# VKostoulas/Medical_Image_Generation

Measured on AMD Instinct MI355X. Metric: 3D DDPM U-Net train-step voxels/sec at 128^3 bf16, higher is better.
Workload: dtype bf16; 1 GPU; C4: DiffusionModelUNet num_channels=(32,64,128,256), attention at 16^3 (heads of 64), 128^3 x batch 1/GPU, eps-prediction, AdamW, clip 1.0; global_batch=1, parallelism=dp1, hipgraph=True

## Files before the change

### include/medimgen_hip.h

```cpp
#ifndef MEDIMGEN_HIP_H
#define MEDIMGEN_HIP_H

#include <hip/hip_runtime_api.h>
#include <stdint.h>

#ifdef __cplusplus
extern "C" {
#endif

#define MI_ERR_BAD_ARG 10001
#define MI_ERR_UNSUPPORTED 10002

int mi_abi_version(void);

int mi_ncdhw_f32_to_ndhwc_bf16(const float* src, void* dst, int N, int C, int64_t V, hipStream_t stream);
int mi_ndhwc_bf16_to_ncdhw_f32(const void* src, float* dst, int N, int C, int64_t V, hipStream_t stream);
int mi_cast_f32_to_bf16(const float* src, void* dst, int64_t n, hipStream_t stream);
int mi_cast_bf16_to_f32(const void* src, float* dst, int64_t n, int accumulate, hipStream_t stream);

int mi_add_bf16(const void* a, const void* b, void* out, int64_t n, hipStream_t stream);
int mi_copy_channels(const void* src, int Cs, int c0s, void* dst, int Cd, int c0d, int nC, int64_t nvox, hipStream_t stream);

int mi_upsample_nearest_fwd(const void* x, void* y, int N, int D, int H, int W, int C, int fd, int fh, int fw, hipStream_t stream);
int mi_upsample_nearest_bwd(const void* dy, void* dx, int N, int D, int H, int W, int C, int fd, int fh, int fw, hipStream_t stream);
int mi_space_to_depth(const void* in, int in_cstride, void* out, int N, int D, int H, int W, int C, int fd, int fh, int fw, hipStream_t stream);
int mi_depth_to_space(const void* in, void* out, int N, int D, int H, int W, int C, int fd, int fh, int fw, hipStream_t stream);

int64_t mi_gn_workspace_bytes(int N, int64_t V, int C);
int mi_gn_stats(const void* x, int x_cstride, int N, int64_t V, int C, int G, float eps, const float* gamma, const float* beta,
                float* scale_shift, float* mean_rstd, void* workspace, int64_t workspace_bytes, hipStream_t stream);
int mi_gn_stats_from_partial(const float* partial_a, int chunks_a, int Ca, const float* partial_b, int chunks_b, int Cb, int N, int64_t V,
                             int G, float eps, const float* gamma, const float* beta, float* scale_shift, float* mean_rstd,
                             hipStream_t stream);
int mi_gn_small_supported(int N, int64_t V, int C, int G);
int mi_gn_small_fwd(const void* x, int x_cstride, void* y, int y_cstride, int N, int64_t V, int C, int G, float eps, const float* gamma,
                    const float* beta, float* scale_shift, float* mean_rstd, int act, hipStream_t stream);
int mi_gn_apply(const void* x, int x_cstride, const float* scale_shift, void* y, int y_cstride, int N, int64_t V, int C, int silu,
                hipStream_t stream);
int mi_gn_bwd(const void* g, int g_cstride, const void* x, int x_cstride, int N, int64_t V, int C, int G, const float* gamma,
              const float* scale_shift, const float* mean_rstd, int silu, const void* add, int add_cstride, const void* add2, int add2_cstride,
              void* dx, int dx_cstride, float* dgamma, float* dbeta, float* coef, void* workspace, int64_t workspace_bytes, hipStream_t stream);

#define MI_GN_FUSED_REPLICAS 16
int mi_gn_bwd_fused(const void* g, int g_cstride, const void* x, int x_cstride, int N, int64_t V, int C, int G, const float* gamma,
                    const float* scale_shift, const float* mean_rstd, int silu, const void* add, int add_cstride, const void* add2,
                    int add2_cstride, void* dx, int dx_cstride, float* dgamma, float* dbeta, double* sums_zeroed, hipStream_t stream);

typedef struct mi_conv_plan mi_conv_plan;
int mi_conv_plan_create(mi_conv_plan** plan, int N, int Di, int Hi, int Wi, int Cin, int Cout, const int* kernel3, const int* stride3,
                        const int* padding3);
int mi_upconv_plan_create(mi_conv_plan** out, int N, int D, int H, int W, int Cin, int Cout);
int mi_conv_plan_destroy(mi_conv_plan* plan);
int mi_conv_plan_out_dims(const mi_conv_plan* plan, int* dims3);
int mi_conv_pack_weights(mi_conv_plan* plan, const float* weight, hipStream_t stream);
typedef struct mi_pack_batch mi_pack_batch;
int mi_conv_pack_batch_create(mi_pack_batch** out, mi_conv_plan* const* plans, const float* const* weights, int n);
int mi_conv_pack_batch_run(mi_pack_batch* batch, hipStream_t stream);
int mi_conv_pack_batch_destroy(mi_pack_batch* batch);

int mi_conv_fwd(mi_conv_plan* plan, const void* x, int x_cstride, const float* scale_shift, int silu, const float* addvec,
                int addvec_stride, const void* res, int res_cstride, void* y, int y_cstride, float* out_stats, hipStream_t stream);
int mi_conv_fwd_stats_chunks(const mi_conv_plan* plan);
int mi_conv_dgrad(mi_conv_plan* plan, const void* dy, int dy_cstride, void* dx, int dx_cstride, hipStream_t stream);
int mi_conv_wgrad(mi_conv_plan* plan, const void* x, int x_cstride, const float* scale_shift, int silu, const void* dy, int dy_cstride,
                  float* dweight, float* dy_colsum, int dy_colsum_stride, hipStream_t stream);
int mi_linear_wgrad_bf16(const void* x, int ldx, int in_features, const void* dy, int ldy, int out_features, int64_t rows, float* dw,
                         float* dbias, hipStream_t stream);

int mi_colsum_bf16(const void* x, float* out, int out_stride, int N, int64_t V, int C, int accumulate, hipStream_t stream);
int mi_add_f32_2d(const float* x, int ldx, float* y, int ldy, int rows, int cols, hipStream_t stream);
int mi_sum_rows_f32(const float* in, int ld, int rows, int cols, float* out, int accumulate, hipStream_t stream);
int mi_zero_f32_2d(float* x, int ld, int rows, int cols, hipStream_t stream);

int mi_gemm_nt_bf16(const void* A, int lda, int64_t sA1, int64_t sA2, const void* B, int ldb, int64_t sB1, int64_t sB2, void* C, int ldc,
                    int64_t sC1, int64_t sC2, const float* bias, const void* R, int ldr, int64_t sR1, int64_t sR2, int M, int N, int K,
                    int Z, int Z2, float alpha, int out_f32, int accumulate, hipStream_t stream);
int mi_transpose_bf16(const void* in, int ld_in, int64_t si1, int64_t si2, void* out, int ld_out, int64_t so1, int64_t so2, int R, int Cc,
                      int Z, int Z2, hipStream_t stream);
int mi_softmax_fwd(const float* scores, void* probs, int64_t rows, int cols, int ld_probs, hipStream_t stream);
int mi_softmax_bwd(const void* probs, const float* dprobs, void* dscores, int64_t rows, int cols, int ld_probs, float scale,
                   hipStream_t stream);

int mi_attn_supported(int C, int heads);
int64_t mi_attn_workspace_bytes(int C, int heads, int B, int S);
int mi_attn_fwd(const void* qkv, int ld, int C, int heads, int B, int S, float scale, const void* resid, void* y, float* lse, void* ws,
                int64_t ws_bytes, hipStream_t stream);
int mi_attn_bwd(const void* qkv, int ld, int C, int heads, int B, int S, float scale, const void* y, const void* resid, const void* dy,
                const float* lse, float* dsum, void* dqkv, void* ws, int64_t ws_bytes, hipStream_t stream);

int mi_timestep_embedding(const int64_t* timesteps, float* out, int B, int dim, float max_period, hipStream_t stream);
int mi_embedding_add(float* emb, const float* weight, const int64_t* labels, int B, int dim, hipStream_t stream);
int mi_embedding_bwd(const float* d_emb, const int64_t* labels, float* dweight, int B, int dim, hipStream_t stream);
int mi_silu_f32(const float* x, float* y, int64_t n, hipStream_t stream);
int mi_silu_bwd_f32(const float* x, const float* dy, float* dx, int64_t n, hipStream_t stream);

int mi_logvar_to_sigma_fwd(const void* logvar, void* sigma, int64_t n, hipStream_t stream);
int mi_logvar_to_sigma_bwd(const void* dsigma, const void* logvar, const void* sigma, void* dlogvar, int64_t n, hipStream_t stream);

int mi_layernorm_fwd(const void* x, int ldx, const float* gamma, const float* beta, void* y, int ldy, float* mean_rstd, int64_t M, int C,
                     float eps, hipStream_t stream);
int mi_layernorm_bwd(const void* dy, int lddy, const void* x, int ldx, const float* gamma, const float* mean_rstd, void* dx, int lddx,
                     float* dgamma, float* dbeta, int64_t M, int C, hipStream_t stream);
int mi_geglu_fwd(const void* h, void* y, int64_t M, int F, hipStream_t stream);
int mi_geglu_bwd(const void* h, const void* dy, void* dh, int64_t M, int F, hipStream_t stream);

int mi_avgpool_fwd(const void* x, void* y, int N, int D, int H, int W, int C, const int kernel[3], const int stride[3], hipStream_t stream);
int mi_avgpool_bwd(const void* dy, void* dx, int N, int D, int H, int W, int C, const int kernel[3], const int stride[3], hipStream_t stream);

int mi_crop_pad(const void* src, int src_is_f16, int C, int D, int H, int W, const int lo[3], float* out, int oD, int oH, int oW,
                float pad_value, int flip_mask, float scale, int clamp01, hipStream_t stream);

enum { MI_AUG_SCALE = 0, MI_AUG_CONTRAST = 1, MI_AUG_GAMMA = 2, MI_AUG_RESTORE_STATS = 3, MI_AUG_ADD_NOISE = 4, MI_AUG_CLAMP01 = 5 };
int64_t mi_aug_stats_workspace_bytes(void);
int mi_aug_plane_stats(const float* x, int64_t V, float* stats, float* workspace, hipStream_t stream);
int mi_aug_pointwise(float* x, int64_t V, int op, float p0, const float* stats_a, const float* stats_b, const float* aux, hipStream_t stream);
int mi_aug_blur_axis(const float* x, float* y, int D, int H, int W, int axis, const float* taps_host, int ntaps, hipStream_t stream);
int mi_aug_lowres(const float* x, float* y, int D, int H, int W, int lD, int lH, int lW, hipStream_t stream);
int mi_aug_affine_sample(const float* x, float* y, int D, int H, int W, int oD, int oH, int oW, const float* a_host, hipStream_t stream);

int mi_im2col3d(const void* x, int x_cstride, void* patches, int N, int D, int H, int W, int C, int k, int s, int p, hipStream_t stream);
int mi_col2im3d(const void* dpatches, void* dx, int dx_cstride, int N, int D, int H, int W, int C, int k, int s, int p, hipStream_t stream);
int mi_disc_pack_weights(const float* w, void* w2, void* w2t, int Cout, int Cout_padded, int Cin, int taps, hipStream_t stream);
int mi_disc_wgrad_unpack(const float* dw2, float* dw, int Cout, int Cin, int taps, hipStream_t stream);
int mi_leaky_relu_fwd(const void* x, void* y, int64_t n, float slope, hipStream_t stream);
int mi_leaky_relu_bwd(const void* x, const void* dy, void* dx, int64_t n, float slope, hipStream_t stream);
int mi_ls_gan_loss(const void* logits, int cs, int64_t nvox, float target, float act_slope, void* dlogits, float* loss, float weight,
                   hipStream_t stream);
int mi_bn_running_update(const float* mean_rstd, float* running_mean, float* running_var, int64_t* num_batches_tracked, int C, float eps,
                         float momentum, int64_t count, hipStream_t stream);

int mi_perc_gather(const void* x, int x_cstride, int C, int N, int D, int H, int W, int axis, const int* idx, int S, const float* shift,
                   const float* scale, void* out, hipStream_t stream);
int mi_perc_scatter_add(const void* dslices, int axis, const int* idx, int S, int N, int D, int H, int W, int C, const float* scale, void* dx,
                        int dx_cstride, hipStream_t stream);
int mi_pad_cin_f32(const float* w, float* out, int Cout, int Cin, int Cin_pad, int taps, hipStream_t stream);
int mi_relu_maxpool2_fwd(void* x, void* pooled, int N, int H, int W, int C, hipStream_t stream);
int mi_relu_maxpool2_bwd(const void* a, const void* dpooled, const void* dadd, void* dx, int N, int H, int W, int C, hipStream_t stream);
int mi_lpips_head(const void* f0, const void* f1, const float* w, int S, int64_t P, int C, float weight, float eps, float* loss, void* df0,
                  hipStream_t stream);

int mi_ssim_tiles(int D, int H, int W, int kD, int kH, int kW);
int mi_ssim_pairs(const float* x_base, const float* y_base, const int* pairs, int P, int C, int D, int H, int W, const float* taps, int kD,
                  int kH, int kW, float c1, float c2, double* partials, int part_stride, int part_off, hipStream_t stream);
int mi_ssim_pool2(const float* x, float* y, int64_t NC, int D, int H, int W, int pool_d, hipStream_t stream);
int mi_ssim_finalize(const double* partials, int P, int part_stride, int S, const int* host_tiles, const double* host_counts,
                     const double* host_weights, float* ms_out, float* ssim_out, hipStream_t stream);

int mi_qsample(const float* x0, const float* noise, const float* sqrt_alphas_cumprod, const float* sqrt_one_minus_alphas_cumprod,
               const int64_t* timesteps, const float* cond, int cond_channels, void* out, float* velocity, int N, int C, int64_t V,
               int num_train_timesteps, hipStream_t stream);
int mi_ddpm_step(float* x, const void* eps, const float* noise, const float* coef, const int64_t* t, void* x_cl, int x_cl_cs, int N,
                 int C, int64_t V, int clip, hipStream_t stream);
int mi_mse_fwd_bwd(const void* pred, const float* target, void* dpred, float* loss, int N, int C, int64_t V, float grad_scale,
                   hipStream_t stream);

int mi_l1_fwd_bwd(const void* pred, const float* target, void* dpred, float* loss, int N, int C, int64_t V, int accumulate, hipStream_t stream);
int mi_reparam_kl_fwd(const void* mu, const void* sigma, const float* eps, void* z, float* loss, int N, int C, int64_t V, float kl_weight,
                      hipStream_t stream);
int mi_reparam_kl_bwd(const void* mu, const void* sigma, const float* eps, const void* dz, void* dmu, void* dsigma, int N, int C, int64_t V,
                      float kl_weight, hipStream_t stream);

int mi_sumsq_f32(const float* x, int64_t n, float* out, int accumulate, hipStream_t stream);
int mi_clip_grad_by_norm(float* grad, int64_t n, const float* grad_sumsq, float max_norm, hipStream_t stream);
int mi_adam_step(float* param, const float* grad, float* exp_avg, float* exp_avg_sq, int64_t n, float lr, float beta1, float beta2,
                 float eps, float weight_decay, int decoupled_weight_decay, const float* grad_sumsq, float max_norm, float grad_scale,
                 float* step_counter, hipStream_t stream);
int mi_adam_step_dev(float* param, const float* grad, float* exp_avg, float* exp_avg_sq, int64_t n, const float* hparams,
                     int decoupled_weight_decay, const float* grad_sumsq, float grad_scale, float* step_counter, hipStream_t stream);
int mi_axpy_f32(float* y, const float* x, float alpha, int64_t n, hipStream_t stream);
int mi_scale_f32(float* x, float alpha, int64_t n, hipStream_t stream);

#define MI_METER_HEADER 4
#define MI_METER_PARTIALS 1024
int64_t mi_meter_bytes(void);
int mi_meter_reset(double* acc, hipStream_t stream);
int mi_mse_eval(const void* pred, const float* target, double* acc, int N, int C, int64_t V, hipStream_t stream);
int mi_l1_eval(const void* pred, const float* target, double* acc, int N, int C, int64_t V, hipStream_t stream);
int mi_kl_eval(const void* mu, const void* sigma, double* acc, int N, int C, int64_t V, hipStream_t stream);

#ifdef __cplusplus
}
#endif
#endif
```

### medical_image_generation_amd/_lib.py

```python
from __future__ import annotations

import ctypes as C
import os

import torch

_HERE = os.path.dirname(os.path.abspath(__file__))
LIB_PATH = os.environ.get("MI_LIB_PATH") or os.path.join(_HERE, "libmedimgen_hip.so")

_p, _i, _l, _f = C.c_void_p, C.c_int, C.c_int64, C.c_float

_SIGS = {
    "mi_abi_version": [],
    "mi_ncdhw_f32_to_ndhwc_bf16": [_p, _p, _i, _i, _l, _p],
    "mi_ndhwc_bf16_to_ncdhw_f32": [_p, _p, _i, _i, _l, _p],
    "mi_cast_f32_to_bf16": [_p, _p, _l, _p],
    "mi_cast_bf16_to_f32": [_p, _p, _l, _i, _p],
    "mi_add_bf16": [_p, _p, _p, _l, _p],
    "mi_copy_channels": [_p, _i, _i, _p, _i, _i, _i, _l, _p],
    "mi_upsample_nearest_fwd": [_p, _p, _i, _i, _i, _i, _i, _i, _i, _i, _p],
    "mi_upsample_nearest_bwd": [_p, _p, _i, _i, _i, _i, _i, _i, _i, _i, _p],
    "mi_space_to_depth": [_p, _i, _p, _i, _i, _i, _i, _i, _i, _i, _i, _p],
    "mi_depth_to_space": [_p, _p, _i, _i, _i, _i, _i, _i, _i, _i, _p],
    "mi_gn_workspace_bytes": [_i, _l, _i],
    "mi_gn_stats": [_p, _i, _i, _l, _i, _i, _f, _p, _p, _p, _p, _p, _l, _p],
    "mi_gn_stats_from_partial": [_p, _i, _i, _p, _i, _i, _i, _l, _i, _f, _p, _p, _p, _p, _p],
    "mi_gn_apply": [_p, _i, _p, _p, _i, _i, _l, _i, _i, _p],
    "mi_gn_bwd": [_p, _i, _p, _i, _i, _l, _i, _i, _p, _p, _p, _i, _p, _i, _p, _i, _p, _i, _p, _p, _p, _p, _l, _p],
    "mi_gn_bwd_fused": [_p, _i, _p, _i, _i, _l, _i, _i, _p, _p, _p, _i, _p, _i, _p, _i, _p, _i, _p, _p, _p, _p],
    "mi_conv_plan_create": [C.POINTER(_p), _i, _i, _i, _i, _i, _i, C.POINTER(_i), C.POINTER(_i), C.POINTER(_i)],
    "mi_upconv_plan_create": [C.POINTER(_p), _i, _i, _i, _i, _i, _i],
    "mi_conv_plan_destroy": [_p],
    "mi_conv_plan_out_dims": [_p, C.POINTER(_i)],
    "mi_conv_pack_weights": [_p, _p, _p],
    "mi_conv_pack_batch_create": [C.POINTER(_p), C.POINTER(_p), C.POINTER(_p), _i],
    "mi_conv_pack_batch_run": [_p, _p],
    "mi_conv_pack_batch_destroy": [_p],
    "mi_conv_fwd": [_p, _p, _i, _p, _i, _p, _i, _p, _i, _p, _i, _p, _p],
    "mi_conv_fwd_stats_chunks": [_p],
    "mi_conv_dgrad": [_p, _p, _i, _p, _i, _p],
    "mi_conv_wgrad": [_p, _p, _i, _p, _i, _p, _i, _p, _p, _i, _p],
    "mi_linear_wgrad_bf16": [_p, _i, _i, _p, _i, _i, _l, _p, _p, _p],
    "mi_colsum_bf16": [_p, _p, _i, _i, _l, _i, _i, _p],
    "mi_add_f32_2d": [_p, _i, _p, _i, _i, _i, _p],
    "mi_sum_rows_f32": [_p, _i, _i, _i, _p, _i, _p],
    "mi_zero_f32_2d": [_p, _i, _i, _i, _p],
    "mi_gemm_nt_bf16": [_p, _i, _l, _l, _p, _i, _l, _l, _p, _i, _l, _l, _p, _p, _i, _l, _l, _i, _i, _i, _i, _i, _f, _i, _i, _p],
    "mi_transpose_bf16": [_p, _i, _l, _l, _p, _i, _l, _l, _i, _i, _i, _i, _p],
    "mi_softmax_fwd": [_p, _p, _l, _i, _i, _p],
    "mi_softmax_bwd": [_p, _p, _p, _l, _i, _i, _f, _p],
    "mi_attn_supported": [_i, _i],
    "mi_attn_workspace_bytes": [_i, _i, _i, _i],
    "mi_attn_fwd": [_p, _i, _i, _i, _i, _i, _f, _p, _p, _p, _p, _l, _p],
    "mi_attn_bwd": [_p, _i, _i, _i, _i, _i, _f, _p, _p, _p, _p, _p, _p, _p, _l, _p],
    "mi_timestep_embedding": [_p, _p, _i, _i, _f, _p],
    "mi_silu_f32": [_p, _p, _l, _p],
    "mi_silu_bwd_f32": [_p, _p, _p, _l, _p],
    "mi_logvar_to_sigma_fwd": [_p, _p, _l, _p],
    "mi_logvar_to_sigma_bwd": [_p, _p, _p, _p, _l, _p],
    "mi_embedding_add": [_p, _p, _p, _i, _i, _p],
    "mi_embedding_bwd": [_p, _p, _p, _i, _i, _p],
    "mi_layernorm_fwd": [_p, _i, _p, _p, _p, _i, _p, _l, _i, _f, _p],
    "mi_layernorm_bwd": [_p, _i, _p, _i, _p, _p, _p, _i, _p, _p, _l, _i, _p],
    "mi_geglu_fwd": [_p, _p, _l, _i, _p],
    "mi_geglu_bwd": [_p, _p, _p, _l, _i, _p],
    "mi_avgpool_fwd": [_p, _p, _i, _i, _i, _i, _i, _p, _p, _p],
    "mi_avgpool_bwd": [_p, _p, _i, _i, _i, _i, _i, _p, _p, _p],
    "mi_crop_pad": [_p, _i, _i, _i, _i, _i, _p, _p, _i, _i, _i, _f, _i, _f, _i, _p],
    "mi_gn_small_supported": [_i, _l, _i, _i],
    "mi_gn_small_fwd": [_p, _i, _p, _i, _i, _l, _i, _i, _f, _p, _p, _p, _p, _i, _p],
    "mi_aug_stats_workspace_bytes": [],
    "mi_aug_plane_stats": [_p, _l, _p, _p, _p],
    "mi_aug_pointwise": [_p, _l, _i, _f, _p, _p, _p, _p],
    "mi_aug_blur_axis": [_p, _p, _i, _i, _i, _i, _p, _i, _p],
    "mi_aug_lowres": [_p, _p, _i, _i, _i, _i, _i, _i, _p],
    "mi_aug_affine_sample": [_p, _p, _i, _i, _i, _i, _i, _i, _p, _p],
    "mi_im2col3d": [_p, _i, _p, _i, _i, _i, _i, _i, _i, _i, _i, _p],
    "mi_col2im3d": [_p, _p, _i, _i, _i, _i, _i, _i, _i, _i, _i, _p],
    "mi_disc_pack_weights": [_p, _p, _p, _i, _i, _i, _i, _p],
    "mi_disc_wgrad_unpack": [_p, _p, _i, _i, _i, _p],
    "mi_perc_gather": [_p, _i, _i, _i, _i, _i, _i, _i, _p, _i, _p, _p, _p, _p],
    "mi_perc_scatter_add": [_p, _i, _p, _i, _i, _i, _i, _i, _i, _p, _p, _i, _p],
    "mi_pad_cin_f32": [_p, _p, _i, _i, _i, _i, _p],
    "mi_relu_maxpool2_fwd": [_p, _p, _i, _i, _i, _i, _p],
    "mi_relu_maxpool2_bwd": [_p, _p, _p, _p, _i, _i, _i, _i, _p],
    "mi_lpips_head": [_p, _p, _p, _i, _l, _i, _f, _f, _p, _p, _p],
    "mi_ssim_tiles": [_i, _i, _i, _i, _i, _i],
    "mi_ssim_pairs": [_p, _p, _p, _i, _i, _i, _i, _i, _p, _i, _i, _i, _f, _f, _p, _i, _i, _p],
    "mi_ssim_pool2": [_p, _p, _l, _i, _i, _i, _i, _p],
    "mi_ssim_finalize": [_p, _i, _i, _i, _p, _p, _p, _p, _p, _p],
    "mi_leaky_relu_fwd": [_p, _p, _l, _f, _p],
    "mi_leaky_relu_bwd": [_p, _p, _p, _l, _f, _p],
    "mi_ls_gan_loss": [_p, _i, _l, _f, _f, _p, _p, _f, _p],
    "mi_bn_running_update": [_p, _p, _p, _p, _i, _f, _f, _l, _p],
    "mi_qsample": [_p, _p, _p, _p, _p, _p, _i, _p, _p, _i, _i, _l, _i, _p],
    "mi_ddpm_step": [_p, _p, _p, _p, _p, _p, _i, _i, _i, _l, _i, _p],
    "mi_mse_fwd_bwd": [_p, _p, _p, _p, _i, _i, _l, _f, _p],
    "mi_l1_fwd_bwd": [_p, _p, _p, _p, _i, _i, _l, _i, _p],
    "mi_reparam_kl_fwd": [_p, _p, _p, _p, _p, _i, _i, _l, _f, _p],
    "mi_reparam_kl_bwd": [_p, _p, _p, _p, _p, _p, _i, _i, _l, _f, _p],
    "mi_sumsq_f32": [_p, _l, _p, _i, _p],
    "mi_clip_grad_by_norm": [_p, _l, _p, _f, _p],
    "mi_adam_step": [_p, _p, _p, _p, _l, _f, _f, _f, _f, _f, _i, _p, _f, _f, _p, _p],
    "mi_adam_step_dev": [_p, _p, _p, _p, _l, _p, _i, _p, _f, _p, _p],
    "mi_axpy_f32": [_p, _p, _f, _l, _p],
    "mi_scale_f32": [_p, _f, _l, _p],
    "mi_meter_bytes": [],
    "mi_meter_reset": [_p, _p],
    "mi_mse_eval": [_p, _p, _p, _i, _i, _l, _p],
    "mi_l1_eval": [_p, _p, _p, _i, _i, _l, _p],
    "mi_kl_eval": [_p, _p, _p, _i, _i, _l, _p],
}
_RET = {"mi_gn_workspace_bytes": _l, "mi_attn_workspace_bytes": _l, "mi_aug_stats_workspace_bytes": _l, "mi_meter_bytes": _l}
_NOCHECK = {"mi_abi_version", "mi_meter_bytes", "mi_ssim_tiles", "mi_gn_small_supported", "mi_gn_workspace_bytes", "mi_aug_stats_workspace_bytes", "mi_attn_supported", "mi_attn_workspace_bytes", "mi_conv_fwd_stats_chunks"}

_lib = None
ABI_VERSION = 12


def exported_symbols() -> list[str]:
    return sorted(_SIGS)


def load():
    global _lib
    if _lib is None:
        if not os.path.exists(LIB_PATH):
            raise RuntimeError(
                f"{LIB_PATH} is missing: build it with `python -c 'import __graft_entry__ as g; g.build()'` "
                "(there is no CPU / PyTorch fallback for the HIP path)")
        lib = C.CDLL(LIB_PATH)
        try:
            lib.mi_abi_version.restype = _i
            have = int(lib.mi_abi_version())
        except AttributeError:
            have = None
        if have != ABI_VERSION:
            raise RuntimeError(f"{LIB_PATH} is a stale library (C ABI {have}, this binding needs {ABI_VERSION}): rebuild it with "
                               "`python -c 'import __graft_entry__ as g; g.build()'`")
        for name, args in _SIGS.items():
            fn = getattr(lib, name)
            fn.argtypes = args
            fn.restype = _RET.get(name, _i)
        _lib = lib
    return _lib


def stream_ptr() -> int:
    return torch.cuda.current_stream().cuda_stream


class HipError(RuntimeError):
    pass


_ERRS = {10001: "MI_ERR_BAD_ARG (host-side shape/alignment check failed)", 10002: "MI_ERR_UNSUPPORTED"}


def ptr(t):
    if t is None:
        return None
    assert t.is_cuda, "medimgen HIP ops take device tensors only"
    return t.data_ptr()


_profile = None


class profile_calls:

    def __enter__(self):
        global _profile
        self.records = []
        _profile = self
        return self

    def __exit__(self, *exc):
        global _profile
        _profile = None
        return False

    def summary(self):
        torch.cuda.synchronize()
        out = {}
        for name, e0, e1 in self.records:
            out[name] = out.get(name, 0.0) + e0.elapsed_time(e1)
        return out


def call(name: str, *args):
    fn = getattr(load(), name)
    prof = _profile
    if prof is not None:
        st = torch.cuda.current_stream()
        e0, e1 = torch.cuda.Event(enable_timing=True), torch.cuda.Event(enable_timing=True)
        e0.record(st)
    rc = fn(*args, stream_ptr())
    if prof is not None:
        e1.record(st)
        prof.records.append((name, e0, e1))
    if rc != 0:
        raise HipError(f"{name} failed: {_ERRS.get(rc, f'hipError_t {rc}')}")


def call_raw(name: str, *args):
    fn = getattr(load(), name)
    rc = fn(*args)
    if name not in _NOCHECK and rc != 0:
        raise HipError(f"{name} failed: {_ERRS.get(rc, f'hipError_t {rc}')}")
    return rc
```

### medical_image_generation_amd/csrc/api.hip

```cpp
#include "common.h"
#include "medimgen_hip.h"
extern "C" int mi_abi_version(void) { return 12; }
```

### medical_image_generation_amd/csrc/conv.hip

```cpp
#include <stdlib.h>
#include <string.h>

#include <algorithm>
#include <unordered_map>
#include <vector>

#include "conv_common.h"
#include "medimgen_hip.h"

namespace {

template <int NP>
struct Stage {
  int pk[NP];
  u32x4 pre[NP];
  unsigned valid;
};

template <int NP, int NT = 256>
__device__ __forceinline__ void stage_init(Stage<NP>& s, const Geom& g) {
  const int HVOX = g.HD * g.HH * g.HW;
#pragma unroll
  for (int i = 0; i < NP; ++i) {
    int v = (threadIdx.x + NT * i) >> 2;
// ... 2046 lines not shown
  const int64_t xb = (int64_t)N * id * ih * iw * x_cs * 2, yb = (int64_t)N * od * oh * ow * y_cs * 2;
  if (xb >= (1ll << 32) || yb >= (1ll << 32) || (int64_t)ps.nfrags * 1024 >= (1ll << 32)) return MI_ERR_UNSUPPORTED;
  ConvArgs a;
  memset(&a, 0, sizeof(a));
  a.x = (const bf16*)x; a.x_cs = x_cs; a.N = N; a.Di = id; a.Hi = ih; a.Wi = iw; a.Cin = ps.Ki;
  a.y = (bf16*)y; a.y_cs = y_cs; a.Cout = ps.Ko; a.Do = od; a.Ho = oh; a.Wo = ow;
  a.ogpq = ps.ny; a.outc_q = ps.Ko;
  a.wpk = ps.d_w; a.wpk_bytes = (unsigned)ps.nfrags * 1024u; a.nchunks = ps.nchunks;
  a.addvec = addvec; a.addvec_stride = addvec_stride;
  a.x_bytes = (unsigned)xb; a.y_bytes = (unsigned)yb;
  a.perm16 = 1;
  a.g = ps.g;
  const int ntiles = N * a.g.tilesD * a.g.tilesH * a.g.tilesW;
  return mi_launch_convph(a, ps.ncb, ps.mode, ntiles, ps.ny, st);
}

int upconv_wgrad_tables(mi_conv_plan* P) {
  const int halo[3] = {1, 1, 1};
  P->g_wg = make_geom(2, P->Di, P->Hi, P->Wi, halo, P->N, 64);
  const Geom& g = P->g_wg;
  if (g.TD != 4 || g.TH != 8 || g.TW != 8 || g.row != WG3_XROW || g.slice != WG3_XSLICE) return MI_ERR_UNSUPPORTED;
  const int ny = (P->Cout + 31) / 32, nch = (P->Cin + 31) / 32;
  P->up_nch = nch;
  P->wg.ny = ny; P->wg.nchunks = nch;
  const int npairs = ny * nch * 2;
  P->wg_split_stride = (int64_t)ny * nch * 64 * 1024;
  const int ntiles = P->N * g.tilesD * g.tilesH * g.tilesW;
  int nsplit = 1;
  {
    int64_t best = -1;
    for (int ns = 1; ns <= 256 && ns <= ntiles; ++ns) {
      const int per_xcd = ns >= 8 ? npairs * ((ns + 7) / 8) : (npairs * ns + 7) / 8;
      const int64_t rounds = (per_xcd + 31) / 32, cost = rounds * ((ntiles + ns - 1) / ns + 2);
      if (best < 0 || cost < best) { best = cost; nsplit = ns; }
    }
  }
  static const int ns_env = env_int("MI_WGU_NSPLIT", 0);
  if (ns_env > 0 && ns_env <= ntiles) nsplit = ns_env;
  while (nsplit > 1 && (int64_t)nsplit * P->wg_split_stride * 4 > (256ll << 20)) nsplit /= 2;
  P->wg_nsplit = nsplit;
  if (hipMalloc((void**)&P->d_part, (size_t)nsplit * P->wg_split_stride * 4) != hipSuccess) return (int)hipErrorOutOfMemory;
  if (hipMalloc((void**)&P->d_cspart, (size_t)nsplit * 8 * P->N * P->Cout * 4) != hipSuccess) return (int)hipErrorOutOfMemory;
  return 0;
}

int upconv_wgrad(mi_conv_plan* P, const void* x, int x_cs, const void* dy, int dy_cs, float* dw, float* dy_colsum, int dy_colsum_stride, hipStream_t st) {
  if (dy_colsum && dy_colsum_stride != 0 && dy_colsum_stride < P->Cout) return MI_ERR_BAD_ARG;
  WgradArgs w;
  memset(&w, 0, sizeof(w));
  ConvArgs& a = w.c;
  a.x = (const bf16*)x; a.x_cs = x_cs; a.N = P->N; a.Di = P->Di; a.Hi = P->Hi; a.Wi = P->Wi; a.Cin = P->Cin;
  a.Cout = P->Cout; a.Do = P->Do; a.Ho = P->Ho; a.Wo = P->Wo;
  a.nchunks = P->up_nch;
  a.g = P->g_wg;
  const int64_t xb = (int64_t)P->N * P->Di * P->Hi * P->Wi * x_cs * 2, dyb = (int64_t)P->N * P->Do * P->Ho * P->Wo * dy_cs * 2;
  if (xb >= (1ll << 32) || dyb >= (1ll << 32)) return MI_ERR_UNSUPPORTED;
  a.x_bytes = (unsigned)xb;
  w.dy = (const bf16*)dy; w.dy_cs = dy_cs; w.dy_bytes = (unsigned)dyb;
  w.sx = 1; w.sy = 2; w.cs_chunks = 1;
  w.part = P->d_part; w.split_stride = P->wg_split_stride;
  w.ntiles = P->N * a.g.tilesD * a.g.tilesH * a.g.tilesW;
  w.nsplit = P->wg_nsplit;
  static const int contig_env = env_int("MI_WGRAD_CONTIG", 1);
  w.contig = contig_env && (w.ntiles % 8 == 0) && (w.nsplit % 8 == 0) && w.nsplit <= w.ntiles;
  w.colsum = dy_colsum; w.colsum_stride = dy_colsum_stride;
  w.cs_part = dy_colsum ? P->d_cspart : nullptr;
  w.npairs = P->wg.ny * P->up_nch * 2;
  const size_t lds = 2 * WGU_XSLOT + WGU_NBY * WGU_YSLOT + 64;
  static bool attr = false;
  if (!attr) {
    hipError_t e = hipFuncSetAttribute((const void*)k_wgrad_up, hipFuncAttributeMaxDynamicSharedMemorySize, 160 * 1024);
    if (e != hipSuccess) return (int)e;
    attr = true;
  }
  dim3 grid(w.nsplit >= 8 ? w.npairs * ((w.nsplit + 7) / 8) * 8 : w.npairs * w.nsplit);
  hipLaunchKernelGGL(k_wgrad_up, grid, dim3(768), lds, st, w);
  CsReduce cs{w.cs_part, P->wg_nsplit * 8, P->N, P->Cout, dy_colsum, dy_colsum_stride, 0};
  cs.nbx = (cs.Cout + 31) / 32;
  const int extra = cs.part ? cs.nbx * cs.N : 0, nmain = P->wg.ny * P->up_nch * 32;
  hipLaunchKernelGGL(k_wgrad_reduce_up, dim3(nmain + extra), dim3(256), 0, st, P->d_part, P->wg_split_stride, P->wg_nsplit, P->up_nch, dw, P->Cout,
                     P->Cin, cs, nmain);
  MI_CHECK_LAUNCH();
  return 0;
}

}

extern "C" {

int mi_conv_plan_create(mi_conv_plan** out, int N, int Di, int Hi, int Wi, int Cin, int Cout, const int* k, const int* s, const int* p) {
  if (!out || N <= 0 || Di <= 0 || Hi <= 0 || Wi <= 0 || Cin <= 0 || Cout <= 0) return MI_ERR_BAD_ARG;
  mi_conv_plan* P = new mi_conv_plan();
  P->N = N; P->Di = Di; P->Hi = Hi; P->Wi = Wi; P->Cin = Cin; P->Cout = Cout;
  std::vector<AxisCombo> cf[3], cdg[3];
  int dims[3] = {Di, Hi, Wi}, od[3], halo_f[3] = {0, 0, 0}, halo_d[3] = {0, 0, 0};
  for (int a = 0; a < 3; ++a) {
    P->k[a] = k[a]; P->s[a] = s[a]; P->p[a] = p[a];
    if (!axis_combos_fwd(k[a], s[a], p[a], cf[a], P->f[a]) || !axis_combos_dgrad(k[a], s[a], p[a], cdg[a])) {
      delete P;
      return MI_ERR_UNSUPPORTED;
    }
    od[a] = (dims[a] + 2 * p[a] - k[a]) / s[a] + 1;
    for (auto& c : cf[a]) if (c.delta != 0) halo_f[a] = 1;
    for (auto& c : cdg[a]) if (c.delta != 0) halo_d[a] = 1;
  }
  P->Do = od[0]; P->Ho = od[1]; P->Wo = od[2];
  P->Q = P->f[0] * P->f[1] * P->f[2];
  P->strided = P->Q > 1;
  P->Dp = (Di + P->f[0] - 1) / P->f[0]; P->Hp = (Hi + P->f[1] - 1) / P->f[1]; P->Wp = (Wi + P->f[2] - 1) / P->f[2];
  P->KT = k[0] * k[1] * k[2];
  P->full27 = true;
  for (int a = 0; a < 3; ++a) P->full27 = P->full27 && k[a] == 3 && s[a] == 1 && p[a] == 1;
  if (P->strided && (Cin % 8) != 0) { delete P; return MI_ERR_UNSUPPORTED; }
  P->ncb_fwd = Cout > 32 && Cout != 96 ? 2 : 1;
  {
    static const int ncb1_max = env_int("MI_NCB1_FWD_MAXC", 32);
    if (Cout <= ncb1_max && (Cout % 32) == 0) P->ncb_fwd = 1;
  }
  P->ncb_dg = Cin > 32 && Cin != 96 ? 2 : 1;
  {
    const int64_t tiles = (int64_t)N * ((od[0] + 3) / 4) * ((od[1] + 7) / 8) * ((od[2] + 7) / 8);
    if (od[0] > 1 && tiles * ((Cout + 63) / 64) <= 128) P->ncb_fwd = 1;
    if (od[0] > 1 && tiles * ((Cin + 63) / 64) <= 128) P->ncb_dg = 1;
  }
  P->g_fwd = make_geom(2, P->Do, P->Ho, P->Wo, halo_f, N);
  static const int use27 = env_int("MI_CONV27", 1);
  {
    static const int use_c1 = env_int("MI_CONV_C1", 1);
    auto c_ok = [](int c) { return c >= 8 && c <= 64 && (c & 7) == 0; };
    P->c1_in = use_c1 && P->full27 && Cin == 1 && c_ok(Cout);
    P->c1_out = use_c1 && P->full27 && Cout == 1 && c_ok(Cin);
    if (P->c1_in || P->c1_out) {
      const int C = P->c1_in ? Cout : Cin;
      if (hipMalloc((void**)&P->d_c1w, (size_t)27 * C * 4) != hipSuccess) { mi_conv_plan_destroy(P); return (int)hipErrorOutOfMemory; }
      if (hipMalloc((void**)&P->d_c1part, (size_t)mi_c1_wgrad_scratch_floats(C) * 4) != hipSuccess) { mi_conv_plan_destroy(P); return (int)hipErrorOutOfMemory; }
    }
  }
  const bool geo27 = P->full27 && P->g_fwd.TD == 4 && P->g_fwd.TH == 8 && P->g_fwd.TW == 8;
  P->v27_fwd = use27 && geo27 && (Cin % 8) == 0 && (Cout % 8) == 0;
  P->v27_dg = use27 && geo27 && (Cout % 8) == 0 && (Cin % 8) == 0;
  {
    static const int use11 = env_int("MI_CONV1X1", 1);
    const bool k1 = P->KT == 1 && !P->strided;
    auto chunks_ok = [](int c) { int n = (c + 31) / 32; return n == 1 || n == 2 || n == 3 || n == 4 || n == 6; };
    P->v11_fwd = use11 && k1 && (Cin % 8) == 0 && chunks_ok(Cin) && ((Cout + 31) / 32) * ((Cin + 31) / 32) * 2 <= 96;
    P->v11_dg = use11 && k1 && (Cout % 8) == 0 && chunks_ok(Cout) && ((Cout + 31) / 32) * ((Cin + 31) / 32) * 2 <= 96;
    static const int use_g11 = env_int("MI_CONV1X1_GEMM", 1);
    P->g11 = use_g11 && k1 && (!P->v11_fwd || !P->v11_dg) && (Cin % 8) == 0 && (Cout % 8) == 0;
    if (P->g11 && (hipMalloc((void**)&P->d_w11, (size_t)Cin * Cout * 2) != hipSuccess || hipMalloc((void**)&P->d_w11t, (size_t)Cin * Cout * 2) != hipSuccess)) {
      mi_conv_plan_destroy(P);
      return (int)hipErrorOutOfMemory;
    }
  }
  build_tables(P->fwd, P->g_fwd, P->ncb_fwd, cf, P->f, P->k, true, Cin, Cout, false, P->v27_fwd || P->v11_fwd);
  P->g_dg = make_geom(2, P->Dp, P->Hp, P->Wp, halo_d, N);
  build_tables(P->dg, P->g_dg, P->ncb_dg, cdg, P->f, P->k, false, Cout, Cin, true, P->v27_dg || P->v11_dg);
  P->g_wg = make_geom(2, P->Do, P->Ho, P->Wo, halo_f, N, 64);
  build_tables(P->wg, P->g_wg, 1, cf, P->f, P->k, true, Cin, Cout, false);
  int e;
  if ((e = upload_tables(P->fwd, true)) || (e = upload_tables(P->dg, true)) || (e = upload_tables(P->wg, false))) { mi_conv_plan_destroy(P); return e; }
  int npairs = P->wg.ny * P->wg.nchunks;
  int64_t off = 0;
  P->wg_pair_off.resize(npairs);
  for (int pr = 0; pr < npairs; ++pr) {
    P->wg_pair_off[pr] = (int)off;
    int nt = P->wg.hdr[(size_t)pr * 4 + 1];
    int frag0 = P->wg.hdr[(size_t)pr * 4 + 3];
    for (int t = 0; t < nt; ++t) {
      const int* it = &P->wg.frag_items[(size_t)(frag0 + t * 2) * 4];
      P->wg_uitems.push_back(it[0]); P->wg_uitems.push_back(it[1]); P->wg_uitems.push_back(it[2]); P->wg_uitems.push_back(0);
    }
    off += (int64_t)nt * 1024;
  }
  P->wg_split_stride = off;
  P->wg_nitems = (int)(off / 1024);
  int ntiles = N * P->g_wg.tilesD * P->g_wg.tilesH * P->g_wg.tilesW;
  int nsplit = 1;
  {
    int64_t best = -1;
    for (int ns = 1; ns <= 256 && ns <= ntiles; ++ns) {
      const int per_xcd = ns >= 8 ? npairs * ((ns + 7) / 8) : (npairs * ns + 7) / 8;
      static const int slab_cost = env_int("MI_WGRAD_SLAB_COST", 0);
      const int64_t rounds = (per_xcd + 31) / 32;
      const int64_t cost = 100 * rounds * ((ntiles + ns - 1) / ns + 6) + (int64_t)slab_cost * ns * (off * 4 / (1 << 20));
      if (best < 0 || cost < best) { best = cost; nsplit = ns; }
    }
  }
  static const int old_split = env_int("MI_WGRAD_SPLIT_OLD", 0);
  if (old_split) nsplit = (256 + npairs - 1) / npairs;
  static const int force_split = env_int("MI_WGRAD_NSPLIT", 0);
  if (force_split && ntiles <= 64) nsplit = force_split;
  if (nsplit > ntiles) nsplit = ntiles;
  while (nsplit > 1 && (int64_t)nsplit * off * 4 > (256ll << 20)) nsplit /= 2;
  if (nsplit < 1) nsplit = 1;
  P->wg_nsplit = nsplit;
  if ((e = upload(P->wg_pair_off, &P->d_pair_off)) || (e = upload(P->wg_uitems, &P->d_uitems))) { mi_conv_plan_destroy(P); return e; }
  if (hipMalloc((void**)&P->d_part, (size_t)nsplit * off * 4) != hipSuccess) { mi_conv_plan_destroy(P); return (int)hipErrorOutOfMemory; }
  if (hipMalloc((void**)&P->d_cspart, (size_t)nsplit * N * Cout * 4) != hipSuccess) { mi_conv_plan_destroy(P); return (int)hipErrorOutOfMemory; }
  {
    static const int use_ph = env_int("MI_CONVPH", 1);
    bool s2all = Di > 1;
    for (int a = 0; a < 3; ++a) s2all = s2all && k[a] == 3 && s[a] == 2 && p[a] == 1;
    if (use_ph && s2all && (Cin % 8) == 0 && (Cout % 8) == 0) {
      int e1 = phase_side_create(P->ph_fwd, S2_FWD, 2, 0, Cout, Cin, P->Do, P->Ho, P->Wo, N);
      int e2 = e1 ? e1 : phase_side_create(P->ph_dg, S2_DG, 1, 1, Cin, Cout, P->Do, P->Ho, P->Wo, N);
      if (e1 || e2) { phase_side_free(P->ph_fwd); phase_side_free(P->ph_dg); if ((e1 ? e1 : e2) != MI_ERR_UNSUPPORTED) { mi_conv_plan_destroy(P); return e1 ? e1 : e2; } }
      if (P->ph_fwd.mode && (Cin % 32) == 0) {
        std::vector<int> h2 = P->wg.hdr;
        const int cpq = Cin / 32;
        for (int pr = 0; pr < P->wg.ny * P->wg.nchunks; ++pr) {
          const int ch = pr % P->wg.nchunks, q = ch / cpq;
          h2[(size_t)pr * 4 + 2] = (ch % cpq) * 32;
          h2[(size_t)pr * 4 + 3] = q;
        }
        if ((e = upload(h2, &P->d_hdr2))) { mi_conv_plan_destroy(P); return e; }
        P->s2_wg_direct = true;
      }
    }
  }
  if (P->strided) {
    size_t nb = (size_t)N * P->Dp * P->Hp * P->Wp * P->Q * Cin * 2;
    if (hipMalloc((void**)&P->d_xs, nb) != hipSuccess || hipMalloc((void**)&P->d_dxs, nb) != hipSuccess) { mi_conv_plan_destroy(P); return (int)hipErrorOutOfMemory; }
  }
  *out = P;
  return 0;
}

int mi_conv_plan_destroy(mi_conv_plan* P) {
  if (!P) return 0;
  phase_side_free(P->ph_fwd); phase_side_free(P->ph_dg);
  if (P->d_hdr2) (void)hipFree(P->d_hdr2);
  if (P->up_inner) mi_conv_plan_destroy(P->up_inner);
  if (P->d_xup) (void)hipFree(P->d_xup);
  free_tables(P->fwd); free_tables(P->dg); free_tables(P->wg);
  if (P->d_pair_off) (void)hipFree(P->d_pair_off);
  if (P->d_uitems) (void)hipFree(P->d_uitems);
  if (P->d_part) (void)hipFree(P->d_part);
  if (P->d_cspart) (void)hipFree(P->d_cspart);
  if (P->d_c1w) (void)hipFree(P->d_c1w);
  if (P->d_w11) (void)hipFree(P->d_w11);
  if (P->d_w11t) (void)hipFree(P->d_w11t);
  if (P->d_g11job) (void)hipFree(P->d_g11job);
  if (P->d_c1part) (void)hipFree(P->d_c1part);
  if (P->d_xs) (void)hipFree(P->d_xs);
  if (P->d_dxs) (void)hipFree(P->d_dxs);
  delete P;
  return 0;
}

int mi_upconv_plan_create(mi_conv_plan** out, int N, int D, int H, int W, int Cin, int Cout) {
  if (!out || N <= 0 || D <= 0 || H <= 0 || W <= 0 || Cin <= 0 || Cout <= 0) return MI_ERR_BAD_ARG;
  if (D == 1) return MI_ERR_UNSUPPORTED;
  mi_conv_plan* P = new mi_conv_plan();
  P->up = true;
  P->N = N; P->Di = D; P->Hi = H; P->Wi = W; P->Cin = Cin; P->Cout = Cout;
  P->Do = 2 * D; P->Ho = 2 * H; P->Wo = 2 * W;
  for (int a = 0; a < 3; ++a) { P->k[a] = 3; P->s[a] = 1; P->p[a] = 1; P->f[a] = 1; }
  P->Q = 1; P->KT = 27; P->Dp = D; P->Hp = H; P->Wp = W;
  const int k3[3] = {3, 3, 3}, s1[3] = {1, 1, 1}, p1[3] = {1, 1, 1};
  int e = mi_conv_plan_create(&P->up_inner, N, 2 * D, 2 * H, 2 * W, Cin, Cout, k3, s1, p1);
  if (e) { P->up_inner = nullptr; mi_conv_plan_destroy(P); return e; }
  if (hipMalloc((void**)&P->d_xup, (size_t)N * 8 * D * H * W * Cin * 2) != hipSuccess) { mi_conv_plan_destroy(P); return (int)hipErrorOutOfMemory; }
  static const int use_ph = env_int("MI_CONVPH", 1);
  if (use_ph && (Cin % 8) == 0 && (Cout % 8) == 0) {
    int e1 = phase_side_create(P->ph_fwd, UC_FWD, 1, 0, Cout, Cin, D, H, W, N);
    int e2 = e1 ? e1 : phase_side_create(P->ph_dg, UC_DG, 2, 1, Cin, Cout, D, H, W, N);
    if (e1 || e2) { phase_side_free(P->ph_fwd); phase_side_free(P->ph_dg); if ((e1 ? e1 : e2) != MI_ERR_UNSUPPORTED) { mi_conv_plan_destroy(P); return e1 ? e1 : e2; } }
    if (P->ph_fwd.mode) {
      const int ew = upconv_wgrad_tables(P);
      if (ew && ew != MI_ERR_UNSUPPORTED) { mi_conv_plan_destroy(P); return ew; }
      P->up_wg = ew == 0;
    }
  }
  *out = P;
  return 0;
}

int mi_conv_plan_out_dims(const mi_conv_plan* P, int* dims3) {
  if (!P || !dims3) return MI_ERR_BAD_ARG;
  dims3[0] = P->Do; dims3[1] = P->Ho; dims3[2] = P->Wo;
  return 0;
}

}

struct G11Job { const float* w; bf16* o; bf16* ot; int Co, Ci, block0, bx; };
namespace {
__global__ void __launch_bounds__(256) k_pack_gemm11(const G11Job* __restrict__ jobs, int njobs) {
  __shared__ float t[32][33];
  int j = 0;
  while (j + 1 < njobs && (int)blockIdx.x >= jobs[j + 1].block0) ++j;
  const G11Job g = jobs[j];
  const int b = blockIdx.x - g.block0, bi = b % g.bx, bo = b / g.bx;
  const int tx = threadIdx.x & 31, ty = threadIdx.x >> 5;
  for (int r = ty; r < 32; r += 8) {
    const int co = bo * 32 + r, ci = bi * 32 + tx;
    const float v = (co < g.Co && ci < g.Ci) ? g.w[(int64_t)co * g.Ci + ci] : 0.f;
    t[r][tx] = v;
    if (co < g.Co && ci < g.Ci) g.o[(int64_t)co * g.Ci + ci] = f2bf(v);
  }
  __syncthreads();
  for (int r = ty; r < 32; r += 8) {
    const int ci = bi * 32 + r, co = bo * 32 + tx;
    if (co < g.Co && ci < g.Ci) g.ot[(int64_t)ci * g.Co + co] = f2bf(t[tx][r]);
  }
}
G11Job g11_job(const mi_conv_plan* P, const float* w, int block0) {
  G11Job g;
  g.w = w; g.o = P->d_w11; g.ot = P->d_w11t; g.Co = P->Cout; g.Ci = P->Cin; g.block0 = block0; g.bx = (P->Cin + 31) / 32;
  return g;
}
int g11_blocks(const mi_conv_plan* P) { return ((P->Cin + 31) / 32) * ((P->Cout + 31) / 32); }
}

extern "C" {

int mi_conv_pack_weights(mi_conv_plan* P, const float* w, hipStream_t st) {
  if (!P || !w) return MI_ERR_BAD_ARG;
  {
    int e = phase_side_pack(P->ph_fwd, w, P->Cout, P->Cin, st);
    if (!e) e = phase_side_pack(P->ph_dg, w, P->Cout, P->Cin, st);
    if (e) return e;
    if (P->up) return mi_conv_pack_weights(P->up_inner, w, st);
  }
  hipLaunchKernelGGL(k_pack_weights, dim3(((P->fwd.nfrags + P->dg.nfrags) * 64 + 255) / 256), dim3(256), 0, st, w, P->fwd.d_wpk,
                     P->fwd.d_items, P->fwd.nfrags, P->dg.d_wpk, P->dg.d_items, P->dg.nfrags, P->Cout, P->Cin, P->KT, P->d_c1w,
                     P->d_c1w ? 27 * P->Cin * P->Cout : 0);
  if (P->g11) {
    if (!P->d_g11job || P->g11job_w != w) {
      if (!P->d_g11job && hipMalloc(&P->d_g11job, sizeof(G11Job)) != hipSuccess) return (int)hipErrorOutOfMemory;
      const G11Job h = g11_job(P, w, 0);
      if (hipMemcpy(P->d_g11job, &h, sizeof(h), hipMemcpyHostToDevice) != hipSuccess) return (int)hipErrorUnknown;
      P->g11job_w = w;
    }
    hipLaunchKernelGGL(k_pack_gemm11, dim3(g11_blocks(P)), dim3(256), 0, st, (const G11Job*)P->d_g11job, 1);
  }
  P->c1_packed = true;
  MI_CHECK_LAUNCH();
  return 0;
}

struct mi_pack_batch {
  PackSuper* d_supers = nullptr;
  int nsupers = 0;
  size_t lds_super = 0;
  G11Job* d_g11 = nullptr;
  int ng11 = 0, g11_blocks = 0;
  PackGroup* d_groups = nullptr;
  int2* d_gtaps = nullptr;
  int ngroups = 0;
  size_t lds = 0;
  PhasePackJob* d_phase = nullptr;
  int nphase = 0, phase_blocks = 0;
};
namespace {
void add_groups(std::vector<PackGroup>& groups, std::vector<int2>& gtaps, const Tables& T, const float* w, const mi_conv_plan* P) {
  std::unordered_map<int64_t, int> index;
  const size_t g0 = groups.size();
  std::vector<std::vector<int2>> taps;
  for (int f = 0; f < T.nfrags; ++f) {
    const int* it = &T.frag_items[(size_t)f * 4];
    const int64_t key = ((int64_t)it[1] << 32) | (unsigned)it[2];
    auto found = index.find(key);
    int gi = found == index.end() ? -1 : found->second;
    if (gi < 0) {
      gi = (int)taps.size();
      index.emplace(key, gi);
      taps.emplace_back();
      PackGroup g;
      memset(&g, 0, sizeof(g));
      g.w = w; g.out = T.d_wpk;
      g.tr = it[3] & 1; g.perm = (it[3] >> 1) & 1;
      g.o0 = g.tr ? it[2] : it[1];
      g.i0 = g.tr ? it[1] : it[2];
      g.Co_t = P->Cout; g.Ci_t = P->Cin; g.KT = P->KT;
      groups.push_back(g);
    }
    taps[(size_t)gi].push_back(int2{it[0], f});
  }
  for (size_t k = 0; k < taps.size(); ++k) {
    groups[g0 + k].ntaps = (int)taps[k].size();
    groups[g0 + k].tap_off = (int)gtaps.size();
    gtaps.insert(gtaps.end(), taps[k].begin(), taps[k].end());
  }
}
}
int mi_conv_pack_batch_create(mi_pack_batch** out, mi_conv_plan* const* plans, const float* const* weights, int n) {
  if (!out || !plans || !weights || n <= 0) return MI_ERR_BAD_ARG;
  std::vector<PackGroup> groups;
  std::vector<int2> gtaps;
  size_t lds = 0;
  std::vector<PhasePackJob> phase;
  int phase_blocks = 0;
  std::vector<G11Job> g11;
  int g11_nblocks = 0;
  std::vector<PackSuper> supers;
  size_t lds_super = 0;
  static const int use_super = env_int("MI_PACK_SUPER", 1);
  bool super_ok = use_super != 0;
  for (int i = 0; i < n; ++i) {
    mi_conv_plan* P = plans[i];
    if (!P || !weights[i]) return MI_ERR_BAD_ARG;
    for (PhaseSide* ps : {&P->ph_fwd, &P->ph_dg})
      if (ps->mode) {
        phase.push_back(phase_job(*ps, weights[i], P->Cout, P->Cin, phase_blocks));
        phase_blocks += mi_pack_phase_blocks(ps->nfrags, ps->ncb, ps->nchunks);
      }
    if (P->g11) {
      g11.push_back(g11_job(P, weights[i], g11_nblocks));
      g11_nblocks += g11_blocks(P);
    }
    if (P->up) P = P->up_inner;
    P->c1_packed = true;
    const size_t g0 = groups.size();
    add_groups(groups, gtaps, P->fwd, weights[i], P);
    add_groups(groups, gtaps, P->dg, weights[i], P);
    if (P->d_c1w && groups.size() > g0) { groups[g0].c1w = P->d_c1w; groups[g0].c1n = 27 * P->Cin * P->Cout; }
    {
      std::unordered_map<int64_t, int> at;
      for (size_t gi = g0; gi < groups.size(); ++gi) {
        const PackGroup& g = groups[gi];
        const int O0 = g.o0 & ~31, I0 = g.i0 & ~31;
        const int64_t key = ((int64_t)O0 << 32) | (unsigned)I0;
        auto f = at.find(key);
        if (f == at.end()) {
          PackSuper su;
          memset(&su, 0, sizeof(su));
          su.w = weights[i]; su.O0 = O0; su.I0 = I0; su.Co_t = P->Cout; su.Ci_t = P->Cin; su.KT = P->KT;
          at.emplace(key, (int)supers.size());
          supers.push_back(su);
          f = at.find(key);
        }
        PackSuper& su = supers[(size_t)f->second];
        if (su.ng < 4) su.g[su.ng++] = (int)gi;
        else super_ok = false;
      }
      const size_t need_su = sizeof(unsigned short) * 32 * (size_t)(32 * P->KT + 4);
      if (need_su > lds_super) lds_super = need_su;
    }
    const size_t need = sizeof(float) * 32 * (size_t)(16 * P->KT + 1) > sizeof(float) * 16 * (size_t)(32 * P->KT + 1)
                            ? sizeof(float) * 32 * (size_t)(16 * P->KT + 1) : sizeof(float) * 16 * (size_t)(32 * P->KT + 1);
    if (need > lds) lds = need;
  }
  if (lds > 64 * 1024) return MI_ERR_UNSUPPORTED;
  mi_pack_batch* B = new mi_pack_batch();
  B->ngroups = (int)groups.size(); B->lds = lds;
  B->nphase = (int)phase.size(); B->phase_blocks = phase_blocks;
  B->ng11 = (int)g11.size(); B->g11_blocks = g11_nblocks;
  if (use_super > 1) fprintf(stderr, "[pack batch] %d plans, %zu groups, %zu super-groups, paired: %d, LDS %zu B\n", n, groups.size(), supers.size(), (int)super_ok, lds_super);
  if (super_ok && !supers.empty() && lds_super <= 150 * 1024) {
    if (hipMalloc((void**)&B->d_supers, sizeof(PackSuper) * supers.size()) != hipSuccess ||
        hipMemcpy(B->d_supers, supers.data(), sizeof(PackSuper) * supers.size(), hipMemcpyHostToDevice) != hipSuccess ||
        hipFuncSetAttribute((const void*)k_pack_super, hipFuncAttributeMaxDynamicSharedMemorySize, 160 * 1024) != hipSuccess) {
      mi_conv_pack_batch_destroy(B);
      return (int)hipErrorOutOfMemory;
    }
    B->nsupers = (int)supers.size(); B->lds_super = lds_super;
  }
  if (B->ng11) {
    if (hipMalloc((void**)&B->d_g11, sizeof(G11Job) * g11.size()) != hipSuccess ||
        hipMemcpy(B->d_g11, g11.data(), sizeof(G11Job) * g11.size(), hipMemcpyHostToDevice) != hipSuccess) {
      mi_conv_pack_batch_destroy(B);
      return (int)hipErrorOutOfMemory;
    }
  }
  if (B->nphase) {
    if (hipMalloc((void**)&B->d_phase, sizeof(PhasePackJob) * phase.size()) != hipSuccess ||
        hipMemcpy(B->d_phase, phase.data(), sizeof(PhasePackJob) * phase.size(), hipMemcpyHostToDevice) != hipSuccess) {
      mi_conv_pack_batch_destroy(B);
      return (int)hipErrorOutOfMemory;
    }
  }
  if (hipMalloc((void**)&B->d_groups, sizeof(PackGroup) * (groups.size() ? groups.size() : 1)) != hipSuccess ||
      hipMalloc((void**)&B->d_gtaps, sizeof(int2) * (gtaps.size() ? gtaps.size() : 1)) != hipSuccess) {
    mi_conv_pack_batch_destroy(B);
    return (int)hipErrorOutOfMemory;
  }
  hipError_t e = hipMemcpy(B->d_groups, groups.data(), sizeof(PackGroup) * groups.size(), hipMemcpyHostToDevice);
  if (e == hipSuccess) e = hipMemcpy(B->d_gtaps, gtaps.data(), sizeof(int2) * gtaps.size(), hipMemcpyHostToDevice);
  if (e != hipSuccess) { mi_conv_pack_batch_destroy(B); return (int)e; }
  *out = B;
  return 0;
}
int mi_conv_pack_batch_run(mi_pack_batch* B, hipStream_t st) {
  if (!B) return MI_ERR_BAD_ARG;
  if (B->nsupers) hipLaunchKernelGGL(k_pack_super, dim3(B->nsupers), dim3(kPackSuperT), B->lds_super, st, B->d_supers, B->d_groups, B->d_gtaps);
  else if (B->ngroups) hipLaunchKernelGGL(k_pack_groups, dim3(B->ngroups), dim3(256), B->lds, st, B->d_groups, B->d_gtaps);
  MI_CHECK_LAUNCH();
  if (B->ng11) hipLaunchKernelGGL(k_pack_gemm11, dim3(B->g11_blocks), dim3(256), 0, st, (const G11Job*)B->d_g11, B->ng11);
  MI_CHECK_LAUNCH();
  if (B->nphase) return mi_launch_pack_phase(B->d_phase, B->nphase, B->phase_blocks, st);
  return 0;
}
int mi_conv_pack_batch_destroy(mi_pack_batch* B) {
  if (!B) return 0;
  if (B->d_groups) (void)hipFree(B->d_groups);
  if (B->d_gtaps) (void)hipFree(B->d_gtaps);
  if (B->d_phase) (void)hipFree(B->d_phase);
  if (B->d_g11) (void)hipFree(B->d_g11);
  if (B->d_supers) (void)hipFree(B->d_supers);
  delete B;
  return 0;
}

int mi_conv_fwd_stats_chunks(const mi_conv_plan* P) {
  if (P && !P->up && P->c1_in) return mi_c1_expand_stats_chunks(P->N, P->Di, P->Hi, P->Wi, P->Cout);
  if (!P || P->up || !P->v27_fwd || P->N > 16 || P->ncb_fwd != 1) return 0;
  return 4 * mi_conv27_grid_x(P->N * P->g_fwd.tilesD * P->g_fwd.tilesH * P->g_fwd.tilesW, P->fwd.ny);
}

int mi_conv_fwd(mi_conv_plan* P, const void* x, int x_cs, const float* scale_shift, int silu, const float* addvec, int addvec_stride,
                const void* res, int res_cs, void* y, int y_cs, float* out_stats, hipStream_t st) {
  if (!P || !x || !y || x_cs < P->Cin || y_cs < P->Cout) return MI_ERR_BAD_ARG;
  if (out_stats && (!mi_conv_fwd_stats_chunks(P) || scale_shift || ((x_cs & 7) && !P->c1_in))) return MI_ERR_UNSUPPORTED;
  if (P->ph_fwd.mode && !scale_shift && !res) {
    const int e = phase_side_run(P->ph_fwd, x, x_cs, P->Di, P->Hi, P->Wi, y, y_cs, P->Do, P->Ho, P->Wo, P->N, addvec, addvec_stride, st);
    if (e != MI_ERR_UNSUPPORTED) return e;
  }
  if (P->up) {
    if (x_cs != P->Cin) return MI_ERR_UNSUPPORTED;
    int e = mi_upsample_nearest_fwd(x, P->d_xup, P->N, P->Di, P->Hi, P->Wi, P->Cin, 2, 2, 2, st);
    if (e) return e;
    return mi_conv_fwd(P->up_inner, P->d_xup, P->Cin, scale_shift, silu, addvec, addvec_stride, res, res_cs, y, y_cs, nullptr, st);
  }
  if ((P->c1_in || P->c1_out) && P->c1_packed && !scale_shift && !res) {
    if (out_stats && !P->c1_in) return MI_ERR_UNSUPPORTED;
    int e = P->c1_in ? mi_launch_c1_expand(x, x_cs, P->d_c1w, addvec, addvec_stride, y, y_cs, P->N, P->Di, P->Hi, P->Wi, P->Cout, 0, st, out_stats)
                     : mi_launch_c1_reduce(x, x_cs, P->d_c1w, addvec, addvec_stride, y, y_cs, P->N, P->Di, P->Hi, P->Wi, P->Cin, st);
    if (e != MI_ERR_UNSUPPORTED) return e;
  }
  if (out_stats && P->c1_in) return MI_ERR_UNSUPPORTED;
  ConvArgs a;
  memset(&a, 0, sizeof(a));
  const bf16* src = (const bf16*)x;
  int src_cs = x_cs;
  if (P->strided) {
    int e = mi_space_to_depth(x, x_cs, P->d_xs, P->N, P->Di, P->Hi, P->Wi, P->Cin, P->f[0], P->f[1], P->f[2], st);
    if (e) return e;
    src = P->d_xs;
    src_cs = P->Q * P->Cin;
  }
  a.x = src; a.x_cs = src_cs; a.N = P->N; a.Di = P->Dp; a.Hi = P->Hp; a.Wi = P->Wp; a.Cin = P->strided ? P->Q * P->Cin : P->Cin;
  if (!P->strided) { a.Di = P->Di; a.Hi = P->Hi; a.Wi = P->Wi; }
  a.y = (bf16*)y; a.y_cs = y_cs; a.Cout = P->Cout; a.Do = P->Do; a.Ho = P->Ho; a.Wo = P->Wo;
  a.ogpq = P->fwd.ny; a.outc_q = P->Cout;
  a.wpk = P->fwd.d_wpk; a.hdr = P->fwd.d_hdr; a.taps = P->fwd.d_taps; a.nchunks = P->fwd.nchunks;
  a.ss = scale_shift; a.ss_C = P->Cin; a.pro_silu = silu;
  a.addvec = addvec; a.addvec_stride = addvec_stride;
  a.res = (const bf16*)res; a.res_cs = res_cs;
  a.g = P->g_fwd;
  int ntiles = P->N * a.g.tilesD * a.g.tilesH * a.g.tilesW;
  a.wpk_bytes = (unsigned)P->fwd.nfrags * 1024u;
  {
    int64_t xb = (int64_t)a.N * a.Di * a.Hi * a.Wi * a.x_cs * 2;
    if (xb >= (1ll << 32)) return MI_ERR_UNSUPPORTED;
    a.x_bytes = (unsigned)xb;
  }
  a.perm16 = P->v27_fwd || P->v11_fwd;
  if (P->g11 && !P->v11_fwd && !scale_shift && !res && (x_cs & 7) == 0 && (y_cs & 7) == 0 && addvec_stride == 0 && !out_stats &&
      ((uintptr_t)x & 15) == 0 && (int64_t)P->N * P->Do * P->Ho * P->Wo < (1ll << 31))
    return mi_gemm_nt_bf16(x, x_cs, 0, 0, P->d_w11, P->Cin, 0, 0, y, y_cs, 0, 0, addvec, nullptr, 0, 0, 0, P->N * P->Do * P->Ho * P->Wo, P->Cout, P->Cin, 1, 1,
                           1.0f, 0, 0, st);
  if (P->v11_fwd && !scale_shift && !res && (x_cs & 7) == 0) {
    const int64_t yb = (int64_t)P->N * P->Do * P->Ho * P->Wo * y_cs * 2;
    a.y_bytes = yb < (1ll << 32) ? (unsigned)yb : 0u;
    return mi_launch_conv1x1(a, P->ncb_fwd, P->fwd.ny, st);
  }
  if (P->v27_fwd && !scale_shift) {
    if (x_cs & 7) return MI_ERR_UNSUPPORTED;
    const int64_t rb = res ? (int64_t)P->N * P->Do * P->Ho * P->Wo * res_cs * 2 : 0;
    a.res_bytes = rb < (1ll << 32) ? (unsigned)rb : 0u;
    const int64_t yb = (int64_t)P->N * P->Do * P->Ho * P->Wo * y_cs * 2;
    a.y_bytes = yb < (1ll << 32) ? (unsigned)yb : 0u;
    a.stats = out_stats; a.stats_chunks = out_stats ? mi_conv_fwd_stats_chunks(P) : 0;
    const int e27 = mi_launch_conv27(a, P->ncb_fwd, 0, ntiles, P->fwd.ny, st);
    if (e27 != MI_ERR_UNSUPPORTED || out_stats) return e27;
    a.stats = nullptr;
  }
  return launch_igemm_any(a, P->ncb_fwd, P->full27 ? 1 : 0, ntiles, P->fwd.ny, st);
}

int mi_conv_dgrad(mi_conv_plan* P, const void* dy, int dy_cs, void* dx, int dx_cs, hipStream_t st) {
  if (!P || !dy || !dx || dy_cs < P->Cout || dx_cs < P->Cin) return MI_ERR_BAD_ARG;
  if (P->ph_dg.mode) {
    const int e = phase_side_run(P->ph_dg, dy, dy_cs, P->Do, P->Ho, P->Wo, dx, dx_cs, P->Di, P->Hi, P->Wi, P->N, nullptr, 0, st);
    if (e != MI_ERR_UNSUPPORTED) return e;
  }
  if (P->up) {
    if (dx_cs != P->Cin) return MI_ERR_UNSUPPORTED;
    int e = mi_conv_dgrad(P->up_inner, dy, dy_cs, P->d_xup, P->Cin, st);
    if (e) return e;
    return mi_upsample_nearest_bwd(P->d_xup, dx, P->N, P->Di, P->Hi, P->Wi, P->Cin, 2, 2, 2, st);
  }
  if (P->c1_out && P->c1_packed) {
    int e = mi_launch_c1_expand(dy, dy_cs, P->d_c1w, nullptr, 0, dx, dx_cs, P->N, P->Di, P->Hi, P->Wi, P->Cin, 1, st);
    if (e != MI_ERR_UNSUPPORTED) return e;
  }
  ConvArgs a;
  memset(&a, 0, sizeof(a));
  a.x = (const bf16*)dy; a.x_cs = dy_cs; a.N = P->N; a.Di = P->Do; a.Hi = P->Ho; a.Wi = P->Wo; a.Cin = P->Cout;
  a.Do = P->Dp; a.Ho = P->Hp; a.Wo = P->Wp;
  a.Cout = P->Q * P->Cin;
  a.ogpq = P->dg.ny / P->Q; a.outc_q = P->Cin;
  if (P->strided) {
    if (dx_cs != P->Cin) return MI_ERR_UNSUPPORTED;
    a.y = P->d_dxs; a.y_cs = P->Q * P->Cin;
  } else {
    a.y = (bf16*)dx; a.y_cs = dx_cs;
  }
  a.wpk = P->dg.d_wpk; a.hdr = P->dg.d_hdr; a.taps = P->dg.d_taps; a.nchunks = P->dg.nchunks;
  a.g = P->g_dg;
  int ntiles = P->N * a.g.tilesD * a.g.tilesH * a.g.tilesW;
  a.wpk_bytes = (unsigned)P->dg.nfrags * 1024u;
  {
    int64_t xb = (int64_t)a.N * a.Di * a.Hi * a.Wi * a.x_cs * 2;
    if (xb >= (1ll << 32)) return MI_ERR_UNSUPPORTED;
    a.x_bytes = (unsigned)xb;
  }
  a.perm16 = P->v27_dg || P->v11_dg;
  if (P->g11 && !P->v11_dg && (dy_cs & 7) == 0 && (dx_cs & 7) == 0 && ((uintptr_t)dy & 15) == 0 &&
      (int64_t)P->N * P->Do * P->Ho * P->Wo < (1ll << 31))
    return mi_gemm_nt_bf16(dy, dy_cs, 0, 0, P->d_w11t, P->Cout, 0, 0, dx, dx_cs, 0, 0, nullptr, nullptr, 0, 0, 0, P->N * P->Do * P->Ho * P->Wo, P->Cin, P->Cout, 1,
                           1, 1.0f, 0, 0, st);
  if (P->v11_dg && (dy_cs & 7) == 0) {
    const int64_t yb = (int64_t)P->N * a.Do * a.Ho * a.Wo * a.y_cs * 2;
    a.y_bytes = yb < (1ll << 32) ? (unsigned)yb : 0u;
    return mi_launch_conv1x1(a, P->ncb_dg, P->dg.ny, st);
  }
  if (P->v27_dg) {
    if (dy_cs & 7) return MI_ERR_UNSUPPORTED;
    const int64_t yb = (int64_t)P->N * a.Do * a.Ho * a.Wo * a.y_cs * 2;
    a.y_bytes = yb < (1ll << 32) ? (unsigned)yb : 0u;
    const int e27 = mi_launch_conv27(a, P->ncb_dg, 1, ntiles, P->dg.ny, st);
    if (e27 != MI_ERR_UNSUPPORTED) return e27;
  }
  int e = launch_igemm_any(a, P->ncb_dg, P->full27 ? 2 : 0, ntiles, P->dg.ny, st);
  if (e) return e;
  if (P->strided) return mi_depth_to_space(P->d_dxs, dx, P->N, P->Di, P->Hi, P->Wi, P->Cin, P->f[0], P->f[1], P->f[2], st);
  return 0;
}

int mi_conv_wgrad(mi_conv_plan* P, const void* x, int x_cs, const float* scale_shift, int silu, const void* dy, int dy_cs, float* dw,
                  float* dy_colsum, int dy_colsum_stride, hipStream_t st) {
  if (!P || !x || !dy || !dw || x_cs < P->Cin || dy_cs < P->Cout) return MI_ERR_BAD_ARG;
  if (P->up && P->up_wg && !scale_shift && (x_cs & 7) == 0 && (dy_cs & 7) == 0) {
    const int e = upconv_wgrad(P, x, x_cs, dy, dy_cs, dw, dy_colsum, dy_colsum_stride, st);
    if (e != MI_ERR_UNSUPPORTED) return e;
  }
  if (P->up) {
    if (x_cs != P->Cin || scale_shift) return MI_ERR_UNSUPPORTED;
    int e = mi_upsample_nearest_fwd(x, P->d_xup, P->N, P->Di, P->Hi, P->Wi, P->Cin, 2, 2, 2, st);
    if (e) return e;
    return mi_conv_wgrad(P->up_inner, P->d_xup, P->Cin, nullptr, 0, dy, dy_cs, dw, dy_colsum, dy_colsum_stride, st);
  }
  static const int use_w11 = env_int("MI_WGRAD1X1", 1);
  if (use_w11 && P->KT == 1 && !P->strided && !scale_shift && !(dy_colsum && dy_colsum_stride != 0 && dy_colsum_stride < P->Cout)) {
    int e = mi_launch_wgrad1x1(x, x_cs, P->Cin, dy, dy_cs, P->Cout, P->N, (int64_t)P->Di * P->Hi * P->Wi, dw, dy_colsum, dy_colsum_stride, st);
    if (e != MI_ERR_UNSUPPORTED) return e;
  }
  static const int use_c1w = env_int("MI_C1_WGRAD", 1);
  if (use_c1w && (P->c1_in || P->c1_out) && P->d_c1part && !scale_shift && !(dy_colsum && dy_colsum_stride != 0)) {
    int e = P->c1_in ? mi_launch_c1_wgrad(dy, dy_cs, x, x_cs, dw, dy_colsum, nullptr, P->d_c1part, P->N, P->Di, P->Hi, P->Wi, P->Cout, 0, st)
                     : mi_launch_c1_wgrad(x, x_cs, dy, dy_cs, dw, nullptr, dy_colsum, P->d_c1part, P->N, P->Di, P->Hi, P->Wi, P->Cin, 1, st);
    if (e != MI_ERR_UNSUPPORTED) return e;
  }
  WgradArgs w;
  memset(&w, 0, sizeof(w));
  w.sx = w.sy = 1; w.cs_chunks = 1;
  ConvArgs& a = w.c;
  const bf16* src = (const bf16*)x;
  int src_cs = x_cs;
  static const int use_w2 = env_int("MI_WGRAD2", 1);
  bool direct = false;
  if (P->s2_wg_direct && use_w2 && !scale_shift && (x_cs & 7) == 0 && (dy_cs & 7) == 0 && (P->Cout & 7) == 0 && P->g_wg.vox == 64) {
    const int px = (P->g_wg.lds_bytes + 1023) / 1024, py = (P->g_wg.TD * P->g_wg.TH * P->g_wg.TW * 64 + 1023) / 1024;
    const int64_t dyb = (int64_t)P->N * P->Do * P->Ho * P->Wo * dy_cs * 2, xb = (int64_t)P->N * P->Di * P->Hi * P->Wi * x_cs * 2;
    direct = px <= 40 && py <= 16 && dyb < (1ll << 32) && xb < (1ll << 32);
  }
  if (P->strided && !direct) {
    int e = mi_space_to_depth(x, x_cs, P->d_xs, P->N, P->Di, P->Hi, P->Wi, P->Cin, P->f[0], P->f[1], P->f[2], st);
    if (e) return e;
    src = P->d_xs;
    src_cs = P->Q * P->Cin;
  }
  const bool s2d = P->strided && !direct;
  a.x = src; a.x_cs = src_cs; a.N = P->N;
  a.Di = s2d ? P->Dp : P->Di; a.Hi = s2d ? P->Hp : P->Hi; a.Wi = s2d ? P->Wp : P->Wi;
  a.Cin = s2d ? P->Q * P->Cin : P->Cin;
  a.Cout = P->Cout; a.Do = P->Do; a.Ho = P->Ho; a.Wo = P->Wo;
  a.hdr = direct ? P->d_hdr2 : P->wg.d_hdr; a.taps = P->wg.d_taps; a.nchunks = P->wg.nchunks;
  if (direct) w.sx = 2;
  a.ss = scale_shift; a.ss_C = P->Cin; a.pro_silu = silu;
  {
    int64_t xb = (int64_t)a.N * a.Di * a.Hi * a.Wi * a.x_cs * 2;
    if (xb >= (1ll << 32)) return MI_ERR_UNSUPPORTED;
    a.x_bytes = (unsigned)xb;
  }
  a.g = P->g_wg;
  w.dy = (const bf16*)dy; w.dy_cs = dy_cs;
  w.part = P->d_part; w.pair_off = P->d_pair_off; w.split_stride = P->wg_split_stride;
  w.ntiles = P->N * a.g.tilesD * a.g.tilesH * a.g.tilesW;
  w.nsplit = P->wg_nsplit;
  static const int contig_env = env_int("MI_WGRAD_CONTIG", 1);
  w.contig = contig_env && (w.ntiles % 8 == 0) && (w.nsplit % 8 == 0) && w.nsplit <= w.ntiles;
  static const int dbg = mi_diag_knob("MI_WGRAD_DBG");
  w.dbg = dbg;
  w.colsum = dy_colsum; w.colsum_stride = dy_colsum_stride;
  static const int cs_slab = env_int("MI_CS_SLAB", 1);
  bool cs_pairs_multi_tap = true;
  for (int yy = 0; yy < P->wg.ny; ++yy) cs_pairs_multi_tap = cs_pairs_multi_tap && P->wg.hdr[((size_t)yy * P->wg.nchunks) * 4 + 1] > 1;
  w.cs_part = (cs_slab && dy_colsum && cs_pairs_multi_tap) ? P->d_cspart : nullptr;  if (dy_colsum && dy_colsum_stride != 0 && dy_colsum_stride < P->Cout) return MI_ERR_BAD_ARG;
  const int hv = a.g.HD * a.g.HH * a.g.HW;
  const int np = (hv * 4 + 255) / 256;
  const int nvox = a.g.TD * a.g.TH * a.g.TW;
  const int npy = (nvox * 4 + 255) / 256;
  size_t lds = (size_t)a.g.lds_bytes + (size_t)nvox * a.g.vox;
  w.npairs = P->wg.ny * P->wg.nchunks;
  dim3 grid(w.nsplit >= 8 ? w.npairs * ((w.nsplit + 7) / 8) * 8 : w.npairs * w.nsplit), blk(512);
  if ((a.g.TD * (a.g.TH / 2) * (a.g.TW / 8)) % 2) return MI_ERR_BAD_ARG;
  if (npy > 4 || np > 16) return MI_ERR_BAD_ARG;
  int max_taps = 0;
  for (size_t i = 1; i < P->wg.hdr.size(); i += 4) max_taps = P->wg.hdr[i] > max_taps ? P->wg.hdr[i] : max_taps;
  if (max_taps >= 32) return MI_ERR_UNSUPPORTED;
#define MI_LAUNCH_WG(NPV) MI_LAUNCH_WG_G(NPV, false)
#define MI_LAUNCH_WG_G(NPV, G3)                                                                                    \
  do {                                                                                                             \
    auto kern = k_conv_wgrad<NPV, 2, G3>;                                                                          \
    static int lds_ok = 0;                                                                                         \
    if ((int)lds > lds_ok) {                                                                                       \
      hipError_t e = hipFuncSetAttribute((const void*)kern, hipFuncAttributeMaxDynamicSharedMemorySize, 160 * 1024); \
      if (e != hipSuccess) return (int)e;                                                                          \
      lds_ok = 160 * 1024;                                                                                         \
    }                                                                                                              \
    hipLaunchKernelGGL(kern, grid, blk, lds, st, w);                                                               \
  } while (0)
  {
    const int px = (a.g.lds_bytes + 1023) / 1024, py = (nvox * 64 + 1023) / 1024;
    const int64_t dyb = (int64_t)P->N * P->Do * P->Ho * P->Wo * dy_cs * 2;
    if (use_w2 && !scale_shift && a.g.vox == 64 && (a.x_cs & 7) == 0 && (a.Cin & 7) == 0 && (dy_cs & 7) == 0 && (P->Cout & 7) == 0 && px <= 40 &&
        py <= 16 && dyb < (1ll << 32)) {
      w.dy_bytes = (unsigned)dyb;
      w.nbuf = (P->KT == 1 && px == 16 && py == 16) ? 4 : 2;
      static const int use_flags = env_int("MI_WGRAD_FLAGS", 1);
      w.flags = use_flags;
      const size_t lds2 = (size_t)(w.nbuf * (px + py)) * 1024 + 64;
      const bool geo3 = P->full27 && a.g.row == WG3_XROW && a.g.slice == WG3_XSLICE && a.g.TD == 4 && a.g.TH == 8 && a.g.TW == 8;
      static bool attr3 = false, attrg = false;
      bool& done = geo3 ? attr3 : attrg;
      if (!done) {
        hipError_t e = geo3 ? hipFuncSetAttribute((const void*)k_conv_wgrad2<true>, hipFuncAttributeMaxDynamicSharedMemorySize, 160 * 1024)
                            : hipFuncSetAttribute((const void*)k_conv_wgrad2<false>, hipFuncAttributeMaxDynamicSharedMemorySize, 160 * 1024);
        if (e != hipSuccess) return (int)e;
        done = true;
      }
      static const int use_roll = env_int("MI_WGRAD_ROLL", 1);
      const bool roll = use_roll && geo3 && !direct && w.sx == 1 && w.sy == 1 && w.nbuf == 2 && w.flags && P->wg.hdr[1] == 27 && w.nsplit <= w.ntiles &&
                        a.g.tilesD >= 2 && (use_roll > 1 || (int64_t)w.ntiles <= 2ll * a.g.tilesD * w.nsplit);
      if (roll) {
        static bool attr_r = false;
        if (!attr_r) {
          hipError_t e = hipFuncSetAttribute((const void*)k_conv_wgrad3, hipFuncAttributeMaxDynamicSharedMemorySize, 160 * 1024);
          if (e != hipSuccess) return (int)e;
          attr_r = true;
        }
#ifdef MI_WG3_DIAG_CLK
        {
          unsigned long long h0[16] = {0, 0, 0, 0, 0, 0, 0, 0, 0, 0, 0, 0, 0, 0, ~0ull, 0};
          (void)hipDeviceSynchronize();
          (void)hipMemcpyToSymbol(HIP_SYMBOL(g_wg3_clk), h0, sizeof(h0));
          static unsigned long long z[6][1024];
          (void)hipMemcpyToSymbol(HIP_SYMBOL(g_wg3_span), z, sizeof(z));
        }
#endif
        hipLaunchKernelGGL(k_conv_wgrad3, grid, dim3(768), (size_t)WR_LDS, st, w);
#ifdef MI_WG3_DIAG_CLK
        {
          unsigned long long h[16];
          (void)hipDeviceSynchronize();
          (void)hipMemcpyFromSymbol(h, HIP_SYMBOL(g_wg3_clk), sizeof(h));
          auto us = [&](int a, int b) { return (double)((long long)h[b] - (long long)h[a]) / 100.0; };
          fprintf(stderr, "[wgrad3 %d->%d ntiles %d nsplit %d] all workgroups: first entry -> last exit %.2f us | workgroup 0 (from the first entry): entry %.2f, "
                  "compute wave 0: setup %.2f, prologue barrier %.2f, tiles %.2f, final barrier %.2f, stores issued %.2f, stores landed %.2f | loader wave: "
                  "descriptors %.2f, prologue issue %.2f, landed %.2f us\n", P->Cin, P->Cout, w.ntiles, w.nsplit, us(14, 15), us(14, 0), us(0, 1), us(1, 2), us(2, 3), us(3, 4),
                  us(4, 5), us(5, 6), us(8, 9), us(9, 10), us(10, 11));
// ... 55 lines not shown
```

### medical_image_generation_amd/engine.py

```python
from __future__ import annotations

import math
import weakref

import torch

from . import _lib
from . import hipops as ops
from ._lib import call, ptr

BF16, F32 = torch.bfloat16, torch.float32

import os as _os
FLASH_ATTENTION = _os.environ.get("MI_FLASH_ATTENTION", "1") == "1"
FUSE_GN_STATS = ops.FUSE_GN_STATS


class ParamArena:

    def __init__(self, entries, device, late=()):
        self.offsets, self.shapes = {}, {}
        late = set(late)
        off = 0
        self.n_late = 0
        for trainable_pass in (True, False):
            for name, shape, trainable in entries:
                if trainable != trainable_pass:
                    continue
                n = math.prod(shape)
                self.offsets[name], self.shapes[name] = off, tuple(shape)
                off += n
                if not trainable_pass or n % 4:
                    off = (off + 3) // 4 * 4
                if trainable_pass and name in late:
                    assert self.n_late == self.offsets[name], f"late tensors must form a prefix of the arena ({name})"
                    self.n_late = off
            if trainable_pass:
                off = (off + 3) // 4 * 4
                self.n_trainable = off
        self.numel = max(off, 4)
        self.data = torch.zeros(self.numel, dtype=F32, device=device)
        self.grad = torch.zeros(self.numel, dtype=F32, device=device)

    def view(self, name, flat=None):
        flat = self.data if flat is None else flat
        o, s = self.offsets[name], self.shapes[name]
        return flat[o:o + math.prod(s)].view(s)

    def gview(self, name):
        return self.view(name, self.grad)

    def span(self, names, flat=None):
        flat = self.data if flat is None else flat
        o = self.offsets[names[0]]
        end = o
        for nme in names:
            assert self.offsets[nme] == end, f"{nme} is not adjacent in the arena"
            end += math.prod(self.shapes[nme])
        return flat[o:end]


def CUT():
    """Tape marker (a no-op when called): recorded by a model at the forward position behind which -- in backward order: before
    which -- every gradient of the arena's early segment is final.  trainer._ArenaTrainer splits the backward there."""


class Tape:
    def __init__(self):
        self.fns = []
        self.grads = {}
        self.keep = []

    def record(self, fn):
        self.fns.append(fn)

    def take(self, t):
        g = self.grads.pop(id(t), None)
        return ops.add(g[0], g[1]) if isinstance(g, tuple) else g

    def take2(self, t):
        g = self.grads.pop(id(t), None)
        return g if isinstance(g, tuple) else (g, None)

    def put(self, t, g):
        cur = self.grads.get(id(t))
        if cur is None:
            self.grads[id(t)] = g
        elif isinstance(cur, tuple):
            self.grads[id(t)] = ops.add(ops.add(cur[0], cur[1]), g)
        else:
            self.grads[id(t)] = (cur, g)
        self.keep.append(t)

    def move(self, t, other: "Tape"):
        g = self.grads.pop(id(t), None)
        if g is not None:
            other.grads[id(t)] = g
            other.keep.append(t)

    def backward(self, out, dout):
        self.put(out, dout)
        for fn in reversed(self.fns):
            fn()
        self.fns.clear()


class Ctx:

    def __init__(self, arena: ParamArena, plans: dict, grad_enabled=True, prepacked=()):
        self.arena, self.plans = arena, plans
        self.tape = Tape() if grad_enabled else None
        self.packed = set(prepacked)
        self.flops_fwd = 0
        self.flops_bwd = 0
        self.sums = {}
        self.cat_parts = {}

    def sums_of(self, x):
        ent = self.sums.get(id(x))
        return ent[0] if ent is not None and ent[1]() is x else None

    def parts_of(self, x):
        ent = self.cat_parts.get(id(x))
        return ent[:2] if ent is not None and ent[2]() is x else None

    def count(self, fwd_flops, dgrad=True, wgrad=True):
        self.flops_fwd += fwd_flops
        if self.tape is not None:
            self.flops_bwd += fwd_flops * (int(dgrad) + int(wgrad))

    def p(self, name):
        return self.arena.view(name)

    def g(self, name):
        return self.arena.gview(name)


class PackBatch:

    def __init__(self, arena: ParamArena, plans: dict):
        import ctypes as C
        self.keys = tuple(plans)
        n = len(self.keys)
        plan_arr = (C.c_void_p * n)(*[plans[k].handle for k in self.keys])
        w_arr = (C.c_void_p * n)(*[arena.view(k[0] + ".weight").data_ptr() for k in self.keys])
        h = C.c_void_p()
        _lib.call_raw("mi_conv_pack_batch_create", C.byref(h), plan_arr, w_arr, n)
        self.handle = h

    def run(self):
        call("mi_conv_pack_batch_run", self.handle)
        return self.keys

    def __del__(self):
        try:
            if getattr(self, "handle", None):
                _lib.call_raw("mi_conv_pack_batch_destroy", self.handle)
                self.handle = None
        except Exception:
            pass


def gn(ctx: Ctx, x, name, groups, eps):
    gamma, beta = ctx.p(name + ".weight"), ctx.p(name + ".bias")
    st = None
    if FUSE_GN_STATS:
        n, v = x.shape[0], x.shape[1] * x.shape[2] * x.shape[3]
        ent, parts = ctx.sums_of(x), ctx.parts_of(x)
        if ent is not None:
            st = ops.gn_stats_from_sums(ent, None, n, v, groups, eps, gamma, beta)
        elif parts is not None:
            ea, eb = ctx.sums_of(parts[0]), ctx.sums_of(parts[1])
            if ea is not None and eb is not None:
                st = ops.gn_stats_from_sums(ea, eb, n, v, groups, eps, gamma, beta)
    if st is None:
        st = ops.gn_stats(x, groups, eps, gamma, beta)
    st.name = name
    return st


UPCONV = _os.environ.get("MI_UPCONV", "1") == "1"


def upsample_conv(ctx: Ctx, x, name, factors, kernel, padding, out=None):
    n, d, h, w, cin = x.shape
    fused = UPCONV and tuple(factors) == (2, 2, 2) and tuple(kernel) == (3, 3, 3) and tuple(padding) == (1, 1, 1) and d > 1 and \
        cin % 8 == 0 and ctx.p(name + ".weight").shape[0] % 8 == 0 and x.is_contiguous()
    if not fused:
        return conv(ctx, upsample(ctx, x, factors), name, kernel, (1, 1, 1), padding, out=out)
    return conv(ctx, x, name, kernel, (1, 1, 1), padding, out=out, upconv=True)


def conv_transpose(ctx: Ctx, x, name, kernel, stride, padding):
    n, d, h, w, cin = x.shape
    wt = ctx.p(name + ".weight")
    cout = wt.shape[1]
    k, s_, p_ = tuple(kernel), tuple(stride), tuple(padding)
    if d <= 1 or k != (3, 3, 3) or p_ != (1, 1, 1) or s_ not in ((1, 1, 1), (2, 2, 2)) or cin % 8 or cout % 8:
        raise NotImplementedError(f"use_convtranspose: kernel {k} stride {s_} padding {p_} ({cin}->{cout}) is not on the HIP path "
                                  "(3-D, kernel 3, padding 1, stride 1 or 2 on all axes, channels in multiples of 8)")
    fine = tuple(v * s_[0] for v in (d, h, w))
    key = (name, n, d, h, w)
    plan = ctx.plans.get(key)
    if plan is None:
        plan = ctx.plans[key] = ops.ConvPlan(n, fine, cout, cin, k, s_, p_)
    if key not in ctx.packed:
        plan.pack(wt)
        ctx.packed.add(key)
    y0 = plan.dgrad(x)
    bias = ctx.p(name + ".bias")
    ss = torch.stack([torch.ones_like(bias), bias], dim=1).unsqueeze(0).expand(n, cout, 2).contiguous()
    y = ops.gn_apply(y0, ops.GNStats(ss, None, 1), False)
    del y0
    ctx.count(2 * y.numel() * cin * 27 // (s_[0] ** 3), dgrad=True)
    if ctx.tape is not None:
        tape = ctx.tape

        def bwd():
            dy = tape.take(y)
            if dy is None:
                return
            plan.wgrad(dy, x, ctx.g(name + ".weight"))
            ops.colsum(dy.contiguous(), out=ctx.g(name + ".bias"), accumulate=True, merge_batch=True)
            tape.put(x, plan.fwd(dy))

        tape.record(bwd)
    return y


def conv(ctx: Ctx, x, name, kernel, stride, padding, norm=None, silu=False, addvec=None, res=None, d_addvec=None,
         need_dx=True, bias_grad_like=None, out=None, upconv=False):
    n, d, h, w, cin = x.shape
    wt = ctx.p(name + ".weight")
    cout = wt.shape[0]
    key = (name, n, d, h, w)
    plan = ctx.plans.get(key)
    if plan is None:
        plan = ctx.plans[key] = ops.UpConvPlan(n, (d, h, w), cin, cout) if upconv else ops.ConvPlan(n, (d, h, w), cin, cout, kernel, stride, padding)
    if key not in ctx.packed:
        plan.pack(wt)
        ctx.packed.add(key)
    av = addvec if addvec is not None else ctx.p(name + ".bias")
    xin = ops.gn_apply(x, norm, silu) if norm is not None else x
    y, sums = plan.fwd(xin, addvec=av, res=res, out=out, want_sums=True)
    if sums is not None:
        ctx.sums[id(y)] = (sums, weakref.ref(y))
    ctx.count(2 * y.numel() * cin * math.prod(kernel), dgrad=need_dx)
    if ctx.tape is not None:
        tape = ctx.tape

        def bwd():
            dy = tape.take(y)
            if dy is None:
                return
            gw = ctx.g(name + ".weight")
            if bias_grad_like is not None:
                plan.wgrad(xin, dy, gw)
                ops.add_f32_(ctx.g(name + ".bias"), ctx.g(bias_grad_like + ".bias"))
            else:
                plan.wgrad(xin, dy, gw, colsum=d_addvec if d_addvec is not None else ctx.g(name + ".bias"))
            if res is not None:
                tape.put(res, dy)
            if need_dx:
                g = plan.dgrad(dy)
                if norm is not None:
                    other, other2 = tape.take2(x)
                    dx = ops.gn_bwd(g, x, norm, ctx.p(norm.name + ".weight"), silu, ctx.g(norm.name + ".weight"),
                                    ctx.g(norm.name + ".bias"), add=other, add2=other2)
                    tape.grads[id(x)] = dx
                    tape.keep.append(x)
                else:
                    tape.put(x, g)

        tape.record(bwd)
    return y


def upsample(ctx: Ctx, x, factors):
    y = ops.upsample_nearest(x, factors)
    if ctx.tape is not None:
        tape = ctx.tape

        def bwd():
            dy = tape.take(y)
            if dy is not None:
                tape.put(x, ops.upsample_nearest_bwd(ops.dense(dy), factors))

        tape.record(bwd)
    return y


def checkpoint(ctx: Ctx, fn, x):
    if ctx.tape is None:
        return fn(ctx, x)
    sub = Ctx(ctx.arena, ctx.plans, grad_enabled=False)
    sub.packed, sub.sums, sub.cat_parts = ctx.packed, ctx.sums, ctx.cat_parts
    y = fn(sub, x)
    ctx.flops_fwd += sub.flops_fwd
    ctx.flops_bwd += 2 * sub.flops_fwd
    tape = ctx.tape

    def bwd():
        dy = tape.take(y)
        if dy is None:
            return
        inner = Ctx(ctx.arena, ctx.plans, grad_enabled=True)
        inner.packed, inner.sums, inner.cat_parts = ctx.packed, ctx.sums, ctx.cat_parts
        y2 = fn(inner, x)
        it = inner.tape
        tape.move(x, it)
        it.backward(y2, dy)
        g = it.take(x)
        if g is not None:
            tape.grads[id(x)] = g
            tape.keep.append(x)
        it.grads.clear(), it.keep.clear()

    tape.record(bwd)
    return y


def avg_pool(ctx: Ctx, x, kernel, stride):
    y = ops.avg_pool(x, kernel, stride)
    if ctx.tape is not None:
        tape = ctx.tape
        dims = tuple(x.shape[1:4])

        def bwd():
            dy = tape.take(y)
            if dy is not None:
                tape.put(x, ops.avg_pool_bwd(ops.dense(dy), dims, kernel, stride))

        tape.record(bwd)
    return y


def gn_act(ctx: Ctx, x, st, silu):
    y = ops.gn_apply(x, st, silu)
    if ctx.tape is not None:
        tape = ctx.tape

        def bwd():
            g = tape.take(y)
            if g is None:
                return
            other, other2 = tape.take2(x)
            dx = ops.gn_bwd(g, x, st, ctx.p(st.name + ".weight"), silu, ctx.g(st.name + ".weight"), ctx.g(st.name + ".bias"),
                            add=other, add2=other2)
            tape.grads[id(x)] = dx
            tape.keep.append(x)

        tape.record(bwd)
    return y


def add(ctx: Ctx, a, b, b_needs_grad=True):
    y = ops.add(a, b)
    if ctx.tape is not None:
        tape = ctx.tape

        def bwd():
            dy = tape.take(y)
            if dy is not None:
                tape.put(a, dy)
                if b_needs_grad:
                    tape.put(b, dy)

        tape.record(bwd)
    return y


def resnet(ctx: Ctx, x, name, sd, groups, eps, addvec, d_addvec, mode=None, stride=None, kernel=None, out=None):
    k3, s1, p1 = (1,) * (3 - sd) + (3,) * sd, (1, 1, 1), (0,) * (3 - sd) + (1,) * sd
    name = name + "." if name else ""
    n1 = gn(ctx, x, name + "norm1", groups, eps)
    if mode is None:
        h = conv(ctx, x, name + "conv1.conv", k3, s1, p1, norm=n1, silu=True, addvec=addvec, d_addvec=d_addvec)
    else:
        h = gn_act(ctx, x, n1, True)
        if mode == "up":
            x, h = upsample(ctx, x, stride), upsample(ctx, h, stride)
        else:
            x, h = avg_pool(ctx, x, kernel, stride), avg_pool(ctx, h, kernel, stride)
        h = conv(ctx, h, name + "conv1.conv", k3, s1, p1, addvec=addvec, d_addvec=d_addvec)
    n2 = gn(ctx, h, name + "norm2", groups, eps)
    if name + "skip_connection.conv.weight" in ctx.arena.offsets:
        xs = conv(ctx, x, name + "skip_connection.conv", (1, 1, 1), s1, (0, 0, 0), bias_grad_like=name + "conv2.conv")
    else:
        xs = x
    return conv(ctx, h, name + "conv2.conv", k3, s1, p1, norm=n2, silu=True, res=xs, out=out)


def concat_buffer(a_shape, ca, cb, device):
    buf = torch.empty(tuple(a_shape[:-1]) + (ca + cb,), dtype=BF16, device=device)
    return buf, buf[..., :ca]


def concat(ctx: Ctx, a, b, buf=None):
    ca, cb = a.shape[-1], b.shape[-1]
    a_in = buf is not None and a.data_ptr() == buf.data_ptr() and ops._cs(a) == ca + cb
    b_in = buf is not None and b.data_ptr() == buf.data_ptr() + 2 * ca and ops._cs(b) == ca + cb
    if a_in or b_in:
        n, v = a.shape[0], a.shape[1] * a.shape[2] * a.shape[3]
        if not a_in:
            call("mi_copy_channels", ptr(a), ops._cs(a), 0, ptr(buf), ca + cb, 0, ca, n * v)
        if not b_in:
            call("mi_copy_channels", ptr(b), ops._cs(b), 0, ptr(buf), ca + cb, ca, cb, n * v)
        y = buf
    else:
        y = ops.concat_channels(a, b)
    ctx.cat_parts[id(y)] = (a, b, weakref.ref(y))
    if ctx.tape is not None:
        tape = ctx.tape

        def bwd():
            dy = tape.take(y)
            if dy is None:
                return
            for t, lo, n_c, in_place in ((a, 0, ca, a_in), (b, ca, cb, b_in)):
                if in_place and id(t) not in tape.grads:
                    tape.grads[id(t)] = dy[..., lo:lo + n_c]
                    tape.keep.append(t)
                    tape.keep.append(dy)
                else:
                    tape.put(t, ops.slice_channels(dy, lo, n_c))

        tape.record(bwd)
    return y


def _gemm(a, lda, sa1, sa2, b, ldb, sb1, sb2, c, ldc, sc1, sc2, m, n, k, z, z2, alpha=1.0, bias=None, res=None, ldr=0, sr1=0,
          sr2=0, accumulate=False):

    def addr(t):
        if t is None:
            return None
        if isinstance(t, tuple):
            return t[0].data_ptr() + t[1] * t[0].element_size()
        return t.data_ptr()

    ct = c[0] if isinstance(c, tuple) else c
    call("mi_gemm_nt_bf16", addr(a), lda, sa1, sa2, addr(b), ldb, sb1, sb2, addr(c), ldc, sc1, sc2, ptr(bias), addr(res), ldr, sr1, sr2,
         m, n, k, z, z2, float(alpha), int(ct.dtype == F32), int(accumulate))


def _transpose(src, ld_in, si1, si2, rows, cols, z, z2, device):
    out = torch.empty((z, cols, rows), dtype=BF16, device=device)
    a = src[0].data_ptr() + src[1] * 2 if isinstance(src, tuple) else src.data_ptr()
    call("mi_transpose_bf16", a, ld_in, si1, si2, ptr(out), rows, z2 * cols * rows, cols * rows, rows, cols, z, z2)
    return out


def _attention_flash(ctx, x, name, st, xn, wqkv, qkv, b, s, c, heads, scale):
    dev = x.device
    d_, h_, w_ = x.shape[1:4]
    y = torch.empty_like(x)
    lse = torch.empty((b * heads, s), dtype=F32, device=dev)
    nws = _lib.call_raw("mi_attn_workspace_bytes", c, heads, b, s)
    ws = torch.empty(max(nws, 16), dtype=torch.uint8, device=dev)
    call("mi_attn_fwd", ptr(qkv), 3 * c, c, heads, b, s, float(scale), ptr(x), ptr(y), ptr(lse), ptr(ws), nws)
    del ws
    ctx.count(2 * b * s * c * 3 * c)
    ctx.count(4 * b * s * s * c)
    if ctx.tape is not None:
        tape = ctx.tape

        def bwd():
            dy = tape.take(y)
            if dy is None:
                return
            dqkv = torch.empty((b * s, 3 * c), dtype=BF16, device=dev)
            dsum = torch.empty((b * heads, s), dtype=F32, device=dev)
            ws = torch.empty(max(nws, 16), dtype=torch.uint8, device=dev)
            call("mi_attn_bwd", ptr(qkv), 3 * c, c, heads, b, s, float(scale), ptr(y), ptr(x), ptr(dy), ptr(lse), ptr(dsum), ptr(dqkv),
                 ptr(ws), nws)
            _attention_param_and_input_grads(ctx, tape, x, name, st, xn, wqkv, dqkv, dy, b, s, c)

        tape.record(bwd)
    return y


def _attention_param_and_input_grads(ctx, tape, x, name, st, xn, wqkv, dqkv, dy, b, s, c):
    dev = x.device
    pre = name + "." if name else ""
    gw = ctx.arena.span([f"{pre}to_{t}.weight" for t in "qkv"], ctx.arena.grad)
    gb = ctx.arena.span([f"{pre}to_{t}.bias" for t in "qkv"], ctx.arena.grad)
    call("mi_linear_wgrad_bf16", ptr(xn), c, c, ptr(dqkv), 3 * c, 3 * c, b * s, ptr(gw), ptr(gb))
    wqkv_t = _transpose(wqkv, c, 0, 0, 3 * c, c, 1, 1, dev)[0]
    dxn = torch.empty(x.shape, dtype=BF16, device=dev)
    _gemm(dqkv, 3 * c, 0, 0, wqkv_t, 3 * c, 0, 0, dxn, c, 0, 0, b * s, c, 3 * c, 1, 1)
    other = tape.take(x)
    dx = ops.gn_bwd(dxn, x, st, ctx.p(pre + "norm.weight"), False, ctx.g(pre + "norm.weight"), ctx.g(pre + "norm.bias"), add=dy, add2=other)
    tape.grads[id(x)] = dx
    tape.keep.append(x)


def attention(ctx: Ctx, x, name, groups, eps, heads):
    b, d_, h_, w_, c = x.shape
    s = d_ * h_ * w_
    hd = c // heads
    scale = 1.0 / math.sqrt(c / heads)
    dev = x.device
    pre = name + "." if name else ""
    st = gn(ctx, x, pre + "norm", groups, eps)
    xn = ops.gn_apply(x, st, False)
    wqkv = ops.cast_bf16(ctx.arena.span([f"{pre}to_{t}.weight" for t in "qkv"]).view(3 * c, c))
    bqkv = ctx.arena.span([f"{pre}to_{t}.bias" for t in "qkv"])
    qkv = torch.empty((b * s, 3 * c), dtype=BF16, device=dev)
    _gemm(xn, c, 0, 0, wqkv, c, 0, 0, qkv, 3 * c, 0, 0, b * s, 3 * c, c, 1, 1, bias=bqkv)
    z = b * heads
    sq = s * 3 * c
    if FLASH_ATTENTION and _lib.call_raw("mi_attn_supported", c, heads):
        return _attention_flash(ctx, x, name, st, xn, wqkv, qkv, b, s, c, heads, scale)
    sp = (s + 7) // 8 * 8
    scores = torch.empty((z, s, s), dtype=F32, device=dev)
    _gemm((qkv, 0), 3 * c, sq, hd, (qkv, c), 3 * c, sq, hd, scores, s, heads * s * s, s * s, s, s, hd, z, heads, alpha=scale)
    probs = ops.softmax_fwd(scores, pad8=True)
    del scores

    def tr_tokens(src, ld_in, si1, si2, cols):
        out = torch.empty((z, cols, sp), dtype=BF16, device=dev)
        a = src[0].data_ptr() + src[1] * 2 if isinstance(src, tuple) else src.data_ptr()
        call("mi_transpose_bf16", a, ld_in, si1, si2, ptr(out), sp, heads * cols * sp, cols * sp, s, cols, z, heads)
        return out

    vt = tr_tokens((qkv, 2 * c), 3 * c, sq, hd, hd)
    y = torch.empty_like(x)
    _gemm(probs, sp, heads * s * sp, s * sp, vt, sp, heads * hd * sp, hd * sp, (y, 0), c, s * c, hd, s, hd, sp, z, heads,
          res=(x, 0), ldr=c, sr1=s * c, sr2=hd)
    ctx.count(2 * b * s * c * 3 * c)
    ctx.count(4 * b * s * s * c)
    if ctx.tape is not None:
        tape = ctx.tape

        def bwd():
            dy = tape.take(y)
            if dy is None:
                return
            dp = torch.empty((z, s, s), dtype=F32, device=dev)
            _gemm((dy, 0), c, s * c, hd, (qkv, 2 * c), 3 * c, sq, hd, dp, s, heads * s * s, s * s, s, s, hd, z, heads)
            ds = ops.softmax_bwd(probs, dp, scale)
            del dp
            dqkv = torch.empty((b * s, 3 * c), dtype=BF16, device=dev)
            kt = tr_tokens((qkv, c), 3 * c, sq, hd, hd)
            _gemm(ds, sp, heads * s * sp, s * sp, kt, sp, heads * hd * sp, hd * sp, (dqkv, 0), 3 * c, sq, hd, s, hd, sp, z, heads)
            qt = tr_tokens((qkv, 0), 3 * c, sq, hd, hd)
            dst = tr_tokens(ds, sp, heads * s * sp, s * sp, s)
            _gemm(dst, sp, heads * s * sp, s * sp, qt, sp, heads * hd * sp, hd * sp, (dqkv, c), 3 * c, sq, hd, s, hd, sp, z, heads)
            del dst, ds
            pt = tr_tokens(probs, sp, heads * s * sp, s * sp, s)
            dot = tr_tokens((dy, 0), c, s * c, hd, hd)
            _gemm(pt, sp, heads * s * sp, s * sp, dot, sp, heads * hd * sp, hd * sp, (dqkv, 2 * c), 3 * c, sq, hd, s, hd, sp, z, heads)
            del pt
            _attention_param_and_input_grads(ctx, tape, x, name, st, xn, wqkv, dqkv, dy, b, s, c)

        tape.record(bwd)
    return y


def linear_f32(x_f32, w, b, gw, gb):
    out_f, in_f = w.shape
    xb, wb = ops.cast_bf16(x_f32), ops.cast_bf16(w)
    m = x_f32.shape[0]
    y = torch.empty((m, out_f), dtype=F32, device=x_f32.device)
    _gemm(xb, in_f, 0, 0, wb, in_f, 0, 0, y, out_f, 0, 0, m, out_f, in_f, 1, 1, bias=b)

    def bwd(dy_f32, need_dx=True):
        dyb = ops.cast_bf16(dy_f32)
        ops.sum_rows_f32(dy_f32, gb, accumulate=True)
        mp = (m + 7) // 8 * 8
        dy_t = torch.empty((out_f, mp), dtype=BF16, device=dy_f32.device)
        x_t = torch.empty((in_f, mp), dtype=BF16, device=dy_f32.device)
        call("mi_transpose_bf16", ptr(dyb), out_f, 0, 0, ptr(dy_t), mp, 0, 0, m, out_f, 1, 1)
        call("mi_transpose_bf16", ptr(xb), in_f, 0, 0, ptr(x_t), mp, 0, 0, m, in_f, 1, 1)
        _gemm(dy_t, mp, 0, 0, x_t, mp, 0, 0, gw, in_f, 0, 0, out_f, in_f, mp, 1, 1, accumulate=True)
        if not need_dx:
            return None
        w_t = _transpose(wb, in_f, 0, 0, out_f, in_f, 1, 1, dy_f32.device)[0]
        dx = torch.empty((m, in_f), dtype=F32, device=dy_f32.device)
        _gemm(dyb, out_f, 0, 0, w_t, out_f, 0, 0, dx, in_f, 0, 0, m, in_f, out_f, 1, 1)
        return dx

    return y, bwd


def _reshape(ctx: Ctx, x, shape):
    y = x.view(shape)
    if ctx.tape is not None:
        tape = ctx.tape

        def bwd():
            g = tape.take(y)
            if g is not None:
                tape.put(x, ops.dense(g).view(x.shape))

        tape.record(bwd)
    return y


def layernorm(ctx: Ctx, x, name, eps=1e-5):
    m, c = x.shape
    gamma, beta = ctx.p(name + ".weight"), ctx.p(name + ".bias")
    y = torch.empty_like(x)
    mr = torch.empty((m, 2), dtype=F32, device=x.device)
    call("mi_layernorm_fwd", ptr(x), c, ptr(gamma), ptr(beta), ptr(y), c, ptr(mr), m, c, float(eps))
    if ctx.tape is not None:
        tape = ctx.tape

        def bwd():
            dy = tape.take(y)
            if dy is None:
                return
            dx = torch.empty_like(x)
            call("mi_layernorm_bwd", ptr(dy), c, ptr(x), c, ptr(gamma), ptr(mr), ptr(dx), c, ptr(ctx.g(name + ".weight")),
                 ptr(ctx.g(name + ".bias")), m, c)
            tape.put(x, dx)

        tape.record(bwd)
    return y


def linear(ctx: Ctx, x, name, bias=True, res=None, need_dx=True):
    m, k = x.shape
    w = ctx.p(name + ".weight")
    n = w.shape[0]
    if k % 8 or n % 8:
        raise ValueError(f"{name}: feature counts must be multiples of 8 on the HIP path (got {k} -> {n})")
    wb = ops.cast_bf16(w)
    y = torch.empty((m, n), dtype=BF16, device=x.device)
    _gemm(x, k, 0, 0, wb, k, 0, 0, y, n, 0, 0, m, n, k, 1, 1, bias=ctx.p(name + ".bias") if bias else None, res=res, ldr=n)
    ctx.count(2 * m * n * k, dgrad=need_dx)
    if ctx.tape is not None:
        tape = ctx.tape

        def bwd():
            dy = tape.take(y)
            if dy is None:
                return
            call("mi_linear_wgrad_bf16", ptr(x), k, k, ptr(dy), n, n, m, ptr(ctx.g(name + ".weight")), ptr(ctx.g(name + ".bias")) if bias else None)
            if res is not None:
                tape.put(res, dy)
            if need_dx:
                wt = _transpose(wb, k, 0, 0, n, k, 1, 1, x.device)[0]
                dx = torch.empty((m, k), dtype=BF16, device=x.device)
                _gemm(dy, n, 0, 0, wt, n, 0, 0, dx, k, 0, 0, m, k, n, 1, 1)
                tape.put(x, dx)

        tape.record(bwd)
    return y


def geglu(ctx: Ctx, h):
    m, f2 = h.shape
    f = f2 // 2
    y = torch.empty((m, f), dtype=BF16, device=h.device)
    call("mi_geglu_fwd", ptr(h), ptr(y), m, f)
    if ctx.tape is not None:
        tape = ctx.tape

        def bwd():
            dy = tape.take(y)
            if dy is not None:
                dh = torch.empty_like(h)
                call("mi_geglu_bwd", ptr(h), ptr(dy), ptr(dh), m, f)
                tape.put(h, dh)

        tape.record(bwd)
    return y


def mha(ctx: Ctx, q, k, v, b, sq, skv, heads):
    c = q.shape[1]
    hd = c // heads
    if hd % 8:
        raise ValueError("head width must be a multiple of 8 on the HIP path")
    scale = 1.0 / math.sqrt(hd)
    z, dev = b * heads, q.device
    kp, qp = (skv + 7) // 8 * 8, (sq + 7) // 8 * 8

    def tr(src, rows, pad):
        out = torch.empty((z, hd, pad), dtype=BF16, device=dev)
        call("mi_transpose_bf16", ptr(src), c, rows * c, hd, ptr(out), pad, heads * hd * pad, hd * pad, rows, hd, z, heads)
        return out

    scores = torch.empty((z, sq, skv), dtype=F32, device=dev)
    _gemm(q, c, sq * c, hd, k, c, skv * c, hd, scores, skv, heads * sq * skv, sq * skv, sq, skv, hd, z, heads, alpha=scale)
    probs = ops.softmax_fwd(scores, pad8=True)
    del scores
    vt = tr(v, skv, kp)
    o = torch.empty((b * sq, c), dtype=BF16, device=dev)
    _gemm(probs, kp, heads * sq * kp, sq * kp, vt, kp, heads * hd * kp, hd * kp, o, c, sq * c, hd, sq, hd, kp, z, heads)
    ctx.count(4 * b * sq * skv * c)
    if ctx.tape is not None:
        tape = ctx.tape

        def bwd():
            do = tape.take(o)
            if do is None:
                return
            dp = torch.empty((z, sq, skv), dtype=F32, device=dev)
            _gemm(do, c, sq * c, hd, v, c, skv * c, hd, dp, skv, heads * sq * skv, sq * skv, sq, skv, hd, z, heads)
            ds = ops.softmax_bwd(probs, dp, scale)
            del dp
            kt = tr(k, skv, kp)
            dq = torch.empty((b * sq, c), dtype=BF16, device=dev)
            _gemm(ds, kp, heads * sq * kp, sq * kp, kt, kp, heads * hd * kp, hd * kp, dq, c, sq * c, hd, sq, hd, kp, z, heads)
            tape.put(q, dq)

            def tr_ss(src):
                out = torch.empty((z, skv, qp), dtype=BF16, device=dev)
                call("mi_transpose_bf16", ptr(src), kp, heads * sq * kp, sq * kp, ptr(out), qp, heads * skv * qp, skv * qp, sq, skv, z, heads)
                return out

            dst, qt = tr_ss(ds), tr(q, sq, qp)
            dk = torch.empty((b * skv, c), dtype=BF16, device=dev)
            _gemm(dst, qp, heads * skv * qp, skv * qp, qt, qp, heads * hd * qp, hd * qp, dk, c, skv * c, hd, skv, hd, qp, z, heads)
            pt, dot = tr_ss(probs), tr(do, sq, qp)
            dv = torch.empty((b * skv, c), dtype=BF16, device=dev)
            _gemm(pt, qp, heads * skv * qp, skv * qp, dot, qp, heads * hd * qp, hd * qp, dv, c, skv * c, hd, skv, hd, qp, z, heads)
            tape.put(k, dk), tape.put(v, dv)

        tape.record(bwd)
    return o


def spatial_transformer(ctx: Ctx, x, name, context, groups, eps, heads, layers):
    b, d_, h_, w_, c = x.shape
    s = d_ * h_ * w_
    pre = name + "." if name else ""
    st = gn(ctx, x, pre + "norm", groups, eps)
    xn = gn_act(ctx, x, st, False)
    one, zero = (1, 1, 1), (0, 0, 0)
    t = _reshape(ctx, conv(ctx, xn, pre + "proj_in.conv", one, one, zero), (b * s, c))
    sc = context.shape[0] // b if context is not None else s
    for li in range(layers):
        blk = f"{pre}transformer_blocks.{li}"
        n1 = layernorm(ctx, t, blk + ".norm1")
        a1 = blk + ".attn1"
        o = mha(ctx, linear(ctx, n1, a1 + ".to_q", bias=False), linear(ctx, n1, a1 + ".to_k", bias=False),
                linear(ctx, n1, a1 + ".to_v", bias=False), b, s, s, heads)
        t = linear(ctx, o, a1 + ".to_out.0", res=t)
        n2 = layernorm(ctx, t, blk + ".norm2")
        a2 = blk + ".attn2"
        kv_src, kv_grad = (context, False) if context is not None else (n2, True)
        o = mha(ctx, linear(ctx, n2, a2 + ".to_q", bias=False), linear(ctx, kv_src, a2 + ".to_k", bias=False, need_dx=kv_grad),
                linear(ctx, kv_src, a2 + ".to_v", bias=False, need_dx=kv_grad), b, s, sc, heads)
        t = linear(ctx, o, a2 + ".to_out.0", res=t)
        n3 = layernorm(ctx, t, blk + ".norm3")
        t = linear(ctx, geglu(ctx, linear(ctx, n3, blk + ".ff.linear1")), blk + ".ff.linear2", res=t)
    return conv(ctx, _reshape(ctx, t, (b, d_, h_, w_, c)), pre + "proj_out.conv", one, one, zero, res=x)
```

### medical_image_generation_amd/hipops.py

```python
from __future__ import annotations

import ctypes as C
import os

import torch

from . import _lib
from ._lib import call, ptr

BF16, F32 = torch.bfloat16, torch.float32
import os as _os
FUSE_GN_STATS = _os.environ.get("MI_FUSE_GN_STATS", "1") == "1"


def _vox(t):
    n, d, h, w, c = t.shape
    return n, d * h * w, c


def _cs(t):
    assert t.dim() == 5
    if t.is_contiguous():
        return t.shape[-1]
    assert t.stride(-1) == 1
# ... 59 lines not shown

def upsample_nearest_bwd(dy, f):
    n, d, h, w, c = dy.shape
    out = torch.empty((n, d // f[0], h // f[1], w // f[2], c), dtype=BF16, device=dy.device)
    call("mi_upsample_nearest_bwd", ptr(dy), ptr(out), n, d // f[0], h // f[1], w // f[2], c, f[0], f[1], f[2])
    return out


def _pool_out(dims, kernel, stride):
    return tuple((d - k) // s + 1 for d, k, s in zip(dims, kernel, stride))


def avg_pool(x, kernel, stride):
    x = dense(x)
    n, d, h, w, c = x.shape
    od, oh, ow = _pool_out((d, h, w), kernel, stride)
    out = torch.empty((n, od, oh, ow, c), dtype=BF16, device=x.device)
    arr = lambda v: (C.c_int * 3)(*v)
    call("mi_avgpool_fwd", ptr(x), ptr(out), n, d, h, w, c, arr(kernel), arr(stride))
    return out


def avg_pool_bwd(dy, in_dims, kernel, stride):
    n, c = dy.shape[0], dy.shape[-1]
    assert dy.is_contiguous() and tuple(dy.shape[1:4]) == _pool_out(in_dims, kernel, stride)
    dx = torch.empty((n,) + tuple(in_dims) + (c,), dtype=BF16, device=dy.device)
    arr = lambda v: (C.c_int * 3)(*v)
    call("mi_avgpool_bwd", ptr(dy), ptr(dx), n, in_dims[0], in_dims[1], in_dims[2], c, arr(kernel), arr(stride))
    return dx


_ws_cache: dict = {}


def _workspace(nbytes, device):
    key = (device.index, "gn")
    ws = _ws_cache.get(key)
    if ws is None or ws.numel() < nbytes:
        ws = torch.empty(max(nbytes, 1 << 20), dtype=torch.uint8, device=device)
        _ws_cache[key] = ws
    return ws


class GNStats:
    __slots__ = ("_ss", "_mr", "groups", "name", "_pending")

    def __init__(self, scale_shift, mean_rstd, groups, pending=None):
        self._ss, self._mr, self.groups, self._pending = scale_shift, mean_rstd, groups, pending

    def _force(self):
        if self._pending is not None:
            x, eps, gamma, beta = self._pending
            self._pending = None
            st = gn_stats(x, self.groups, eps, gamma, beta, allow_small=False)
            self._ss, self._mr = st._ss, st._mr

    @property
    def scale_shift(self):
        self._force()
        return self._ss

    @property
    def mean_rstd(self):
        self._force()
        return self._mr


GN_SMALL = os.environ.get("MI_GN_SMALL", "0") == "1"


def gn_stats(x, groups, eps, gamma, beta, allow_small=True) -> GNStats:
    n, v, c = _vox(x)
    if allow_small and GN_SMALL and c % groups == 0 and _lib.call_raw("mi_gn_small_supported", n, v, c, groups):
        return GNStats(None, None, groups, pending=(x, float(eps), gamma, beta))
    ss = torch.empty((n, c, 2), dtype=F32, device=x.device)
    mr = torch.empty((n, groups, 2), dtype=F32, device=x.device)
    nb = _lib.call_raw("mi_gn_workspace_bytes", n, v, c)
    ws = _workspace(nb, x.device)
    call("mi_gn_stats", ptr(x), _cs(x), n, v, c, groups, float(eps), ptr(gamma), ptr(beta), ptr(ss), ptr(mr), ptr(ws), ws.numel())
    return GNStats(ss, mr, groups)


class ChannelSums:
    __slots__ = ("partial", "chunks", "channels")

    def __init__(self, partial, chunks, channels):
        self.partial, self.chunks, self.channels = partial, chunks, channels


def gn_stats_from_sums(a: ChannelSums, b: ChannelSums | None, n, v, groups, eps, gamma, beta) -> GNStats | None:
    c = a.channels + (b.channels if b is not None else 0)
    dev = a.partial.device
    ss = torch.empty((n, c, 2), dtype=F32, device=dev)
    mr = torch.empty((n, groups, 2), dtype=F32, device=dev)
    call("mi_gn_stats_from_partial", ptr(a.partial), a.chunks, a.channels, ptr(b.partial) if b is not None else None,
         b.chunks if b is not None else 0, b.channels if b is not None else 0, n, v, groups, float(eps), ptr(gamma), ptr(beta), ptr(ss), ptr(mr))
    return GNStats(ss, mr, groups)


def gn_apply(x, st: GNStats, silu: bool):
    n, v, c = _vox(x)
    y = torch.empty(x.shape, dtype=BF16, device=x.device)
    if st._pending is not None and st._pending[0] is x:
        _, eps, gamma, beta = st._pending
        st._pending = None
        st._ss = torch.empty((n, c, 2), dtype=F32, device=x.device)
        st._mr = torch.empty((n, st.groups, 2), dtype=F32, device=x.device)
        call("mi_gn_small_fwd", ptr(x), _cs(x), ptr(y), c, n, v, c, st.groups, eps, ptr(gamma), ptr(beta), ptr(st._ss), ptr(st._mr), int(silu))
        return y
    call("mi_gn_apply", ptr(x), _cs(x), ptr(st.scale_shift), ptr(y), c, n, v, c, int(silu))
    return y


GN_FUSED_REPLICAS = 16


def gn_bwd(g, x, st: GNStats, gamma, silu: bool, dgamma, dbeta, add=None, add2=None, sums=None):
    if add is None and add2 is not None:
        add, add2 = add2, None
    n, v, c = _vox(x)
    dx = torch.empty(x.shape, dtype=BF16, device=x.device)
    if sums is not None:
        assert sums.dtype == torch.float64 and sums.numel() >= GN_FUSED_REPLICAS * n * c * 2
        call("mi_gn_bwd_fused", ptr(g), _cs(g), ptr(x), _cs(x), n, v, c, st.groups, ptr(gamma), ptr(st.scale_shift), ptr(st.mean_rstd),
             int(silu), ptr(add), _cs(add) if add is not None else 0, ptr(add2), _cs(add2) if add2 is not None else 0, ptr(dx), c,
             ptr(dgamma), ptr(dbeta), ptr(sums))
        return dx
    coef = torch.empty((n, c, 3), dtype=F32, device=x.device)
    nb = _lib.call_raw("mi_gn_workspace_bytes", n, v, c)
    ws = _workspace(nb, x.device)
    call("mi_gn_bwd", ptr(g), _cs(g), ptr(x), _cs(x), n, v, c, st.groups, ptr(gamma), ptr(st.scale_shift), ptr(st.mean_rstd),
         int(silu), ptr(add), _cs(add) if add is not None else 0, ptr(add2), _cs(add2) if add2 is not None else 0, ptr(dx), c, ptr(dgamma),
         ptr(dbeta), ptr(coef), ptr(ws), ws.numel())
    return dx


class ConvPlan:

    def __init__(self, n, dims, cin, cout, kernel, stride, padding):
        self.n, self.dims, self.cin, self.cout = n, tuple(dims), cin, cout
        self.kernel, self.stride, self.padding = tuple(kernel), tuple(stride), tuple(padding)
        h = C.c_void_p()
        arr = lambda v: (C.c_int * 3)(*v)
        _lib.call_raw("mi_conv_plan_create", C.byref(h), n, dims[0], dims[1], dims[2], cin, cout, arr(kernel), arr(stride), arr(padding))
        self.handle = h
        od = (C.c_int * 3)()
        _lib.call_raw("mi_conv_plan_out_dims", self.handle, od)
        self.out_dims = tuple(od)
        self.stats_chunks = int(_lib.call_raw("mi_conv_fwd_stats_chunks", self.handle))

    def __del__(self):
        try:
            if getattr(self, "handle", None):
                _lib.call_raw("mi_conv_plan_destroy", self.handle)
                self.handle = None
        except Exception:
            pass

    def pack(self, weight_f32):
        assert weight_f32.dtype == F32 and weight_f32.is_contiguous()
        call("mi_conv_pack_weights", self.handle, ptr(weight_f32))

    def fwd(self, x, st: GNStats | None = None, silu=False, addvec=None, res=None, out=None, want_sums=False):
        n, d, h, w, c = x.shape
        assert (n, (d, h, w), c) == (self.n, self.dims, self.cin), f"plan/input mismatch {x.shape} vs {self.n, self.dims, self.cin}"
        if out is None:
            y = torch.empty((n,) + self.out_dims + (self.cout,), dtype=BF16, device=x.device)
        else:
            assert out.shape == (n,) + self.out_dims + (self.cout,) and out.dtype == BF16
            y = out
        av_stride = 0
        if addvec is not None and addvec.dim() == 2:
            assert addvec.shape == (n, self.cout) and addvec.stride(1) == 1
            av_stride = addvec.stride(0)
        sums = None
        if want_sums and FUSE_GN_STATS and st is None and self.stats_chunks > 0 and (_cs(x) % 8 == 0 or (self.cin == 1 and res is None)):
            sums = ChannelSums(torch.empty((n, self.cout, self.stats_chunks, 2), dtype=F32, device=x.device), self.stats_chunks, self.cout)
        call("mi_conv_fwd", self.handle, ptr(x), _cs(x), ptr(st.scale_shift) if st is not None else None, int(silu), ptr(addvec), av_stride,
             ptr(res), _cs(res) if res is not None else 0, ptr(y), _cs(y), ptr(sums.partial) if sums is not None else None)
        return (y, sums) if want_sums else y

    def dgrad(self, dy):
        assert dy.shape == (self.n,) + self.out_dims + (self.cout,)
        dx = torch.empty((self.n,) + self.dims + (self.cin,), dtype=BF16, device=dy.device)
        call("mi_conv_dgrad", self.handle, ptr(dy), _cs(dy), ptr(dx), self.cin)
        return dx

    def wgrad(self, x, dy, dweight_f32, st: GNStats | None = None, silu=False, colsum=None):
        assert dweight_f32.dtype == F32 and dweight_f32.is_contiguous()
        cs_stride = 0
        if colsum is not None:
            assert colsum.dtype == F32 and colsum.stride(-1) == 1
            if colsum.dim() == 2:
                assert colsum.shape == (self.n, self.cout)
                cs_stride = colsum.stride(0)
            else:
                assert colsum.shape == (self.cout,)
        call("mi_conv_wgrad", self.handle, ptr(x), _cs(x), ptr(st.scale_shift) if st is not None else None, int(silu), ptr(dy), _cs(dy),
             ptr(dweight_f32), ptr(colsum), cs_stride)


class UpConvPlan(ConvPlan):

    def __init__(self, n, dims, cin, cout):
        self.n, self.dims, self.cin, self.cout = n, tuple(dims), cin, cout
        self.kernel, self.stride, self.padding = (3, 3, 3), (1, 1, 1), (1, 1, 1)
        h = C.c_void_p()
        _lib.call_raw("mi_upconv_plan_create", C.byref(h), n, dims[0], dims[1], dims[2], cin, cout)
        self.handle = h
        self.out_dims = tuple(2 * d for d in dims)
        self.stats_chunks = 0


def colsum(x, out=None, accumulate=False, merge_batch=False):
    n, v, c = _vox(x)
    assert x.is_contiguous()
    if merge_batch:
        n, v = 1, n * v
    if out is None:
        out = torch.empty((n, c), dtype=F32, device=x.device)
    stride = out.stride(0) if out.dim() == 2 else c
    call("mi_colsum_bf16", ptr(x), ptr(out), stride, n, v, c, int(accumulate))
    return out


def add_f32_(y, x):
    y2 = y if y.dim() == 2 else y.unsqueeze(0)
    if x.dim() == 1:
        assert x.shape[0] == y2.shape[1] and x.stride(0) == 1
        ldx, xp = 0, x
    else:
        assert x.shape == y2.shape and x.stride(1) == 1
        ldx, xp = x.stride(0), x
    assert y2.stride(1) == 1
    call("mi_add_f32_2d", ptr(xp), ldx, ptr(y2), y2.stride(0), y2.shape[0], y2.shape[1])
    return y


def zero_f32_2d_(x):
    assert x.dim() == 2 and x.stride(1) == 1
    call("mi_zero_f32_2d", ptr(x), x.stride(0), x.shape[0], x.shape[1])
    return x


def sum_rows_f32(x, out, accumulate=True):
    assert x.dim() == 2 and x.stride(1) == 1 and out.is_contiguous()
    call("mi_sum_rows_f32", ptr(x), x.stride(0), x.shape[0], x.shape[1], ptr(out), int(accumulate))
    return out


def gemm_nt(a, b, *, bias=None, res=None, alpha=1.0, out=None, out_f32=False, accumulate=False):
    a3, b3 = (a if a.dim() == 3 else a.unsqueeze(0)), (b if b.dim() == 3 else b.unsqueeze(0))
    z, m, k = a3.shape
    n = b3.shape[1]
    assert b3.shape[2] == k and a3.stride(2) == 1 and b3.stride(2) == 1
    zb = b3.shape[0]
    assert zb in (1, z)
    if out is None:
        out = torch.empty((z, m, n), dtype=F32 if out_f32 else BF16, device=a.device)
        out_v = out
    else:
        out_v = out if out.dim() == 3 else out.unsqueeze(0)
    r3 = None
    if res is not None:
        r3 = res if res.dim() == 3 else res.unsqueeze(0)
        assert r3.stride(2) == 1
    call("mi_gemm_nt_bf16", ptr(a3), a3.stride(1), a3.stride(0), 0, ptr(b3), b3.stride(1), b3.stride(0) if zb == z else 0, 0,
         ptr(out_v), out_v.stride(1), out_v.stride(0), 0, ptr(bias), ptr(r3), r3.stride(1) if r3 is not None else 0,
         r3.stride(0) if r3 is not None else 0, 0, m, n, k, z, 1, float(alpha), int(out_v.dtype == F32), int(accumulate))
    return out if a.dim() == 3 or out.dim() == 2 else out[0]


def transpose(x):
    x3 = x if x.dim() == 3 else x.unsqueeze(0)
    z, r, c = x3.shape
    out = torch.empty((z, c, r), dtype=BF16, device=x.device)
    call("mi_transpose_bf16", ptr(x3), x3.stride(1), x3.stride(0), 0, ptr(out), r, c * r, 0, r, c, z, 1)
    return out if x.dim() == 3 else out[0]


def softmax_fwd(scores_f32, pad8=False):
    s = scores_f32.contiguous()
    cols = s.shape[-1]
    ld = (cols + 7) // 8 * 8 if pad8 else cols
    out = torch.empty(s.shape[:-1] + (ld,), dtype=BF16, device=s.device)
    call("mi_softmax_fwd", ptr(s), ptr(out), s.numel() // cols, cols, ld)
    return out[..., :cols]


def softmax_bwd(probs, dprobs_f32, scale):
    cols, ld = probs.shape[-1], probs.stride(-2)
    assert probs.stride(-1) == 1 and dprobs_f32.is_contiguous()
    out = torch.empty(probs.shape[:-1] + (ld,), dtype=BF16, device=probs.device)
    call("mi_softmax_bwd", ptr(probs), ptr(dprobs_f32), ptr(out), probs.numel() // cols, cols, ld, float(scale))
    return out[..., :cols]


def timestep_embedding(t_i64, dim, max_period=10000.0):
    out = torch.empty((t_i64.shape[0], dim), dtype=F32, device=t_i64.device)
    call("mi_timestep_embedding", ptr(t_i64), ptr(out), t_i64.shape[0], dim, float(max_period))
    return out


def silu_f32(x):
    y = torch.empty_like(x)
    call("mi_silu_f32", ptr(x), ptr(y), x.numel())
    return y


def silu_bwd_f32(x, dy):
    dx = torch.empty_like(x)
    call("mi_silu_bwd_f32", ptr(x), ptr(dy), ptr(dx), x.numel())
    return dx


def cast_bf16(x_f32):
    assert x_f32.is_contiguous() and x_f32.dtype == F32
    out = torch.empty(x_f32.shape, dtype=BF16, device=x_f32.device)
    call("mi_cast_f32_to_bf16", ptr(x_f32), ptr(out), x_f32.numel())
    return out


def cast_f32(x_bf16, out=None, accumulate=False):
    if out is None:
        out = torch.empty(x_bf16.shape, dtype=F32, device=x_bf16.device)
    call("mi_cast_bf16_to_f32", ptr(x_bf16), ptr(out), x_bf16.numel(), int(accumulate))
    return out
```

### medical_image_generation_amd/unet.py

```python
from __future__ import annotations

import math
from typing import Sequence

import torch
from torch import nn

from . import engine as E
from . import hipops as ops
from ._lib import call, ptr

F32 = torch.float32
import os as _os
SKIP_SLOTS = _os.environ.get("MI_SKIP_SLOTS", "1") == "1"


class _Tree(nn.Module):
    """Anonymous container: gives parameters the reference's dotted state_dict names."""


def _attach(root, dotted, tensor):
    mod = root
    parts = dotted.split(".")
    for part in parts[:-1]:
        if part not in mod._modules:
            mod.add_module(part, _Tree())
        mod = mod._modules[part]
    mod.register_parameter(parts[-1], nn.Parameter(tensor))


def _tuple_rep(v, n):
    if isinstance(v, (list, tuple)):
        if len(v) != n:
            raise ValueError(f"Sequence must have length {n}, got {len(v)}.")
        return tuple(v)
    return (v,) * n


def _axis3(v, sd, fill):
    t = _tuple_rep(v, sd)
    return (fill,) * (3 - sd) + tuple(int(a) for a in t)


class ParamSpec:

    def __init__(self, root, sd):
        self.root, self.sd = root, sd
        self.order = []

    def _add(self, name, t, trainable=True):
        _attach(self.root, name, t)
        self.order.append((name, tuple(t.shape), trainable))

    def conv(self, name, cin, cout, k, zero=False):
        k = _tuple_rep(k, self.sd)
        w, b = torch.empty(cout, cin, *k), torch.empty(cout)
        if zero:
            w.zero_(), b.zero_()
        else:
            nn.init.kaiming_uniform_(w, a=math.sqrt(5))
            bound = 1 / math.sqrt(cin * math.prod(k))
            nn.init.uniform_(b, -bound, bound)
        self._add(name + ".weight", w)
        self._add(name + ".bias", b)

    def linear(self, name, cin, cout, trainable=True, bias=True):
        w = torch.empty(cout, cin)
        nn.init.kaiming_uniform_(w, a=math.sqrt(5))
        bound = 1 / math.sqrt(cin)
        self._add(name + ".weight", w, trainable)
        if bias:
            self._add(name + ".bias", torch.empty(cout).uniform_(-bound, bound), trainable)

    def transformer(self, name, c, cdim, layers):
        name = name + "." if name else ""
        self.norm(name + "norm", c)
        self.conv(name + "proj_in.conv", c, c, 1)
        for k in range(layers):
            blk = f"{name}transformer_blocks.{k}"
            for attn, kv in (("attn1", c), ("attn2", cdim)):
                self.linear(f"{blk}.{attn}.to_q", c, c, bias=False)
                self.linear(f"{blk}.{attn}.to_k", kv, c, bias=False)
                self.linear(f"{blk}.{attn}.to_v", kv, c, bias=False)
                self.linear(f"{blk}.{attn}.to_out.0", c, c)
            self.linear(f"{blk}.ff.linear1", c, 8 * c)
            self.linear(f"{blk}.ff.linear2", 4 * c, c)
            for n in ("norm1", "norm2", "norm3"):
                self.norm(f"{blk}.{n}", c)
        self.conv(name + "proj_out.conv", c, c, 1, zero=True)

    def norm(self, name, c):
        self._add(name + ".weight", torch.ones(c))
        self._add(name + ".bias", torch.zeros(c))

    def attention(self, name, c):
        pre = name + "." if name else ""
        self.norm(pre + "norm", c)
        for n in ("to_q", "to_k", "to_v"):
            self.linear(pre + n, c, c)
        self.linear(pre + "proj_attn", c, c, trainable=False)


def arena_order(entries, groups, late=()):
    grouped = {n for g in groups for n in g}
    by_name = {e[0]: e for e in entries}
    out = []
    for g in groups:
        out.extend(by_name[n] for n in g)
    out.extend(e for e in entries if e[0] not in grouped)
    late = set(late)
    for g in groups:
        assert len({n in late for n in g}) <= 1, f"group straddles the late / early split: {g[0]} ..."
    return [e for e in out if e[0] in late and e[2]] + [e for e in out if not (e[0] in late and e[2])]


class HipModule(nn.Module):

    def _init_plumbing(self, spec: ParamSpec, groups, late=()):
        self._late = tuple(n for n in late)
        self._entries = arena_order(spec.order, groups, self._late)
        self._arena = None
        self._plans = {}
        self._packb = None

    def arena(self, device) -> E.ParamArena:
        device = torch.device(device)
        if device.type == "cuda" and device.index is None:
            device = torch.device("cuda", torch.cuda.current_device())
        params = dict(self.named_parameters())
        a = self._arena
        first = self._entries[0][0]
        if a is None or a.data.device != device or params[first].data_ptr() != a.view(first).data_ptr():
            a = E.ParamArena(self._entries, device, late=self._late)
            for name, _, _ in self._entries:
                v = a.view(name)
                v.copy_(params[name].data)
                params[name].data = v
            self._arena = a
            self._plans = {}
            self._packb = None
        return a

    def pack_all(self):
        if not self._plans or self._arena is None:
            return ()
        pb = getattr(self, "_packb", None)
        if pb is None or len(pb.keys) != len(self._plans):
            if torch.cuda.is_current_stream_capturing():
                return () if pb is None else pb.run()
            pb = self._packb = E.PackBatch(self._arena, self._plans)
        return pb.run()

    def _apply(self, fn, *args, **kwargs):
        self._arena = None
        self._packb = None
        return super()._apply(fn, *args, **kwargs)


class _NetFn(torch.autograd.Function):

    @staticmethod
    def forward(ctx, module, runner, nouts, grad_enabled, x, emb, *params):
        dev = x.device
        ctx.set_materialize_grads(False)
        arena = module.arena(dev)
        c = E.Ctx(arena, module._plans, grad_enabled=grad_enabled, prepacked=module.pack_all())
        need_dx = bool(grad_enabled and ctx.needs_input_grad[4])
        outs_cl, extra = runner(c, x, need_dx) if emb is None else runner(c, x, need_dx, emb)
        ctx.c, ctx.module, ctx.outs_cl, ctx.need_dx, ctx.extra = c, module, outs_cl, need_dx, extra
        ctx.need_demb = bool(emb is not None and grad_enabled and ctx.needs_input_grad[5])
        ctx.sd = module.spatial_dims
        ctx.names = [n for n, _ in module.named_parameters()]
        outs = tuple(ops.to_channels_first(o, ctx.sd) for o in outs_cl)
        return outs if nouts > 1 else outs[0]

    @staticmethod
    def backward(ctx, *douts):
        c = ctx.c
        arena = c.arena
        arena.grad.zero_()
        tape = c.tape
        for o, do in zip(ctx.outs_cl, douts):
            if do is not None:
                tape.put(o, ops.to_channels_last(do.contiguous().float()))
        for fn in reversed(tape.fns):
            fn()
        tape.fns.clear()
        dx = None
        if ctx.need_dx:
            g = tape.take(ctx.extra["x_cl"])
            dx = ops.to_channels_first(ops.dense(g), ctx.sd) if g is not None else None
        demb = ctx.extra["d_emb"]() if ctx.need_demb else None
        trainable = {n for n, _, t in ctx.module._entries if t}
        grads = tuple(arena.gview(n).clone() if n in trainable else None for n in ctx.names)
        tape.grads.clear(), tape.keep.clear()
        return (None, None, None, None, dx, demb) + grads


class DiffusionModelUNet(HipModule):
    def __init__(
        self,
        spatial_dims: int,
        in_channels: int,
        out_channels: int,
        num_res_blocks: Sequence[int] | int = (2, 2, 2, 2),
        num_channels: Sequence[int] = (32, 64, 64, 64),
        attention_levels: Sequence[bool] = (False, False, True, True),
        norm_num_groups: int = 32,
        norm_eps: float = 1e-6,
        resblock_updown: bool = False,
        num_head_channels: int | Sequence[int] = 8,
        with_conditioning: bool = False,
        transformer_num_layers: int = 1,
        cross_attention_dim: int | None = None,
        num_class_embeds: int | None = None,
        upcast_attention: bool = False,
        use_flash_attention: bool = False,
        dropout_cattn: float = 0.0,
        strides=((2, 2, 2), (2, 2, 2), (2, 2, 2)),
        kernel_sizes=((4, 4, 4), (4, 4, 4), (4, 4, 4)),
        paddings=(1, 1, 1),
    ) -> None:
        super().__init__()
        if with_conditioning is True and cross_attention_dim is None:
            raise ValueError("DiffusionModelUNet expects dimension of the cross-attention conditioning (cross_attention_dim) "
                             "when using with_conditioning.")
        if cross_attention_dim is not None and with_conditioning is False:
            raise ValueError("DiffusionModelUNet expects with_conditioning=True when specifying the cross_attention_dim.")
        if dropout_cattn > 1.0 or dropout_cattn < 0.0:
            raise ValueError("Dropout cannot be negative or >1.0!")
        if any((c % norm_num_groups) != 0 for c in num_channels):
            raise ValueError("DiffusionModelUNet expects all num_channels being multiple of norm_num_groups")
        if len(num_channels) != len(attention_levels):
            raise ValueError("DiffusionModelUNet expects num_channels being same size of attention_levels")
        if isinstance(num_head_channels, int):
            num_head_channels = _tuple_rep(num_head_channels, len(attention_levels))
        if len(num_head_channels) != len(attention_levels):
            raise ValueError("num_head_channels should have the same length as attention_levels.")
        if isinstance(num_res_blocks, int):
            num_res_blocks = _tuple_rep(num_res_blocks, len(num_channels))
        if len(num_res_blocks) != len(num_channels):
            raise ValueError("`num_res_blocks` should be a single integer or a tuple of integers with the same length as "
                             "`num_channels`.")
        if use_flash_attention:
            raise ValueError("use_flash_attention is True but xformers is not installed.")
        if with_conditioning and dropout_cattn > 0.0:
            raise NotImplementedError("dropout_cattn > 0 is not on the HIP path (the reference's default is 0.0)")
        if with_conditioning and (cross_attention_dim % 8 or any(a and n % 8 for a, n in zip(attention_levels, num_head_channels))):
            raise ValueError("cross_attention_dim and num_head_channels must be multiples of 8 on the HIP path")
        if spatial_dims not in (2, 3):
            raise ValueError("spatial_dims must be 2 or 3")

        sd = self.spatial_dims = spatial_dims
        self.in_channels, self.out_channels = in_channels, out_channels
        self.block_out_channels = ch = tuple(num_channels)
        self.num_res_blocks = nrb = tuple(num_res_blocks)
        self.attention_levels = att = tuple(attention_levels)
        self.num_head_channels = nhc = tuple(num_head_channels)
        self.with_conditioning = bool(with_conditioning)
        self.cross_attention_dim, self.transformer_num_layers = cross_attention_dim, transformer_num_layers
        self.num_class_embeds = num_class_embeds
        self.resblock_updown = bool(resblock_updown)
        self.use_checkpointing = False
        self.groups, self.eps = norm_num_groups, norm_eps
        L = len(ch)
        self._k = [_axis3(kernel_sizes[i], sd, 1) for i in range(L)]
        self._s = [_axis3(strides[i], sd, 1) for i in range(L)]
        self._p = [_axis3(paddings[i], sd, 0) for i in range(L)]
        temb = self.temb_dim = ch[0] * 4

        spec = ParamSpec(self, sd)
        self._resnets: list[tuple[str, int, int]] = []
        self._attns: list[str] = []

        def resnet(name, cin, cout):
            spec.norm(name + ".norm1", cin)
            spec.conv(name + ".conv1.conv", cin, cout, 3)
            spec.linear(name + ".time_emb_proj", temb, cout)
            spec.norm(name + ".norm2", cout)
            spec.conv(name + ".conv2.conv", cout, cout, 3, zero=True)
            if cin != cout:
                spec.conv(name + ".skip_connection.conv", cin, cout, 1)
            self._resnets.append((name, cin, cout))

        def attn(name, c):
            if with_conditioning:
                spec.transformer(name, c, cross_attention_dim, transformer_num_layers)
            else:
                spec.attention(name, c)
                self._attns.append(name)

        spec.conv("conv_in.conv", in_channels, ch[0], kernel_sizes[0])
        spec.linear("time_embed.0", ch[0], temb)
        spec.linear("time_embed.2", temb, temb)
        out_c = ch[0]
        for i in range(L):
            in_c, out_c = out_c, ch[i]
            for j in range(nrb[i]):
                resnet(f"down_blocks.{i}.resnets.{j}", in_c if j == 0 else out_c, out_c)
                if att[i]:
                    attn(f"down_blocks.{i}.attentions.{j}", out_c)
            if i != L - 1:
                if resblock_updown:
                    resnet(f"down_blocks.{i}.downsampler", out_c, out_c)
                else:
                    spec.conv(f"down_blocks.{i}.downsampler.op.conv", out_c, out_c, kernel_sizes[i + 1])
        resnet("middle_block.resnet_1", ch[-1], ch[-1])
        attn("middle_block.attention", ch[-1])
        resnet("middle_block.resnet_2", ch[-1], ch[-1])
        rch, rnrb, ratt = list(reversed(ch)), list(reversed(nrb)), list(reversed(att))
        out_c = rch[0]
        for i in range(L):
            prev, out_c = out_c, rch[i]
            in_c = rch[min(i + 1, L - 1)]
            n = rnrb[i] + 1
            for j in range(n):
                skip_c = in_c if j == n - 1 else out_c
                resnet(f"up_blocks.{i}.resnets.{j}", (prev if j == 0 else out_c) + skip_c, out_c)
                if ratt[i]:
                    attn(f"up_blocks.{i}.attentions.{j}", out_c)
            if i != L - 1:
                if resblock_updown:
                    resnet(f"up_blocks.{i}.upsampler", out_c, out_c)
                else:
                    spec.conv(f"up_blocks.{i}.upsampler.conv.conv", out_c, out_c, 3)
        spec.norm("out.0", ch[0])
        spec.conv("out.2.conv", ch[0], out_channels, 3, zero=True)
        if num_class_embeds is not None:
            spec._add("class_embedding.weight", torch.randn(num_class_embeds, temb))

        groups = [[r[0] + ".time_emb_proj.weight" for r in self._resnets], [r[0] + ".time_emb_proj.bias" for r in self._resnets],
                  [r[0] + ".conv1.conv.bias" for r in self._resnets]]
        for a in self._attns:
            groups.append([f"{a}.to_{t}.weight" for t in "qkv"])
            groups.append([f"{a}.to_{t}.bias" for t in "qkv"])
        self._cut_level = max(0, L // 2 - 1)
        late_pre = tuple(f"down_blocks.{i}." for i in range(self._cut_level + 1)) + ("conv_in.", "time_embed.", "class_embedding.")
        late = [n for n, _, _ in spec.order if n.startswith(late_pre) or ".time_emb_proj." in n or n.endswith(".conv1.conv.bias")]
        self._init_plumbing(spec, groups, late)
        rch_, rnrb_ = list(reversed(ch)), list(reversed(nrb))
        pops = []
        for i in range(L):
            for j in range(rnrb_[i] + 1):
                pops.append((rch_[i - 1] if i > 0 else rch_[0]) if j == 0 else rch_[i])
        self._skip_ca = list(reversed(pops))
        self._temb_off = {}
        off = 0
        for name, _, cout in self._resnets:
            self._temb_off[name] = off
            off += cout
        self._temb_total = off

    def _resnet(self, c, x, name, temb_all, d_temb_all, out=None, mode=None, stride=None, kernel=None):
        cout = c.p(name + ".conv1.conv.weight").shape[0]
        off = self._temb_off[name]

        def run(cc, xx):
            return E.resnet(cc, xx, name, self.spatial_dims, self.groups, self.eps, temb_all[:, off:off + cout],
                            d_temb_all[:, off:off + cout] if d_temb_all is not None else None, mode=mode, stride=stride, kernel=kernel,
                            out=out if cc is c or cc.tape is None else None)

        return E.checkpoint(c, run, x) if self.use_checkpointing else run(c, x)

    def _attention(self, c, x, name, heads):
        if self.with_conditioning:
            run = lambda cc, xx: E.spatial_transformer(cc, xx, name, self._context, self.groups, self.eps, heads, self.transformer_num_layers)
        else:
            run = lambda cc, xx: E.attention(cc, xx, name, self.groups, self.eps, heads)
        return E.checkpoint(c, run, x) if self.use_checkpointing else run(c, x)

    def _heads(self, ch, nhc):
        return ch // nhc if nhc is not None else 1

    def _run(self, c: E.Ctx, x_cl, timesteps, need_dx, class_labels=None, down_res=None, mid_res=None, context=None):
        ch, L, sd = self.block_out_channels, len(self.block_out_channels), self.spatial_dims
        self._context = context
        a = c.arena
        dev = x_cl.device
        grad = c.tape is not None
        t0 = ops.timestep_embedding(timesteps, ch[0])
        e1, bwd1 = E.linear_f32(t0, c.p("time_embed.0.weight"), c.p("time_embed.0.bias"), c.g("time_embed.0.weight"), c.g("time_embed.0.bias"))
        s1v = ops.silu_f32(e1)
        emb, bwd2 = E.linear_f32(s1v, c.p("time_embed.2.weight"), c.p("time_embed.2.bias"), c.g("time_embed.2.weight"), c.g("time_embed.2.bias"))
        if self.num_class_embeds is not None:
            call("mi_embedding_add", ptr(emb), ptr(c.p("class_embedding.weight")), ptr(class_labels), emb.shape[0], emb.shape[1])
        se = ops.silu_f32(emb)
        wn = [r[0] + ".time_emb_proj.weight" for r in self._resnets]
        bn = [r[0] + ".time_emb_proj.bias" for r in self._resnets]
        T = self._temb_total
        temb_all, bwd3 = E.linear_f32(se, a.span(wn).view(T, self.temb_dim), a.span(bn), a.span(wn, a.grad).view(T, self.temb_dim),
                                      a.span(bn, a.grad))
        ops.add_f32_(temb_all, a.span([r[0] + ".conv1.conv.bias" for r in self._resnets]))
        d_temb_all = ops.zero_f32_2d_(torch.empty_like(temb_all)) if grad else None
        if grad:
            def bwd_emb():
                ops.sum_rows_f32(d_temb_all, a.span([r[0] + ".conv1.conv.bias" for r in self._resnets], a.grad), accumulate=True)
                d_se = bwd3(d_temb_all)
                d_emb = ops.silu_bwd_f32(emb, d_se)
                if self.num_class_embeds is not None:
                    call("mi_embedding_bwd", ptr(d_emb), ptr(class_labels), ptr(c.g("class_embedding.weight")), d_emb.shape[0], d_emb.shape[1])
                d_s1 = bwd2(d_emb)
                bwd1(ops.silu_bwd_f32(e1, d_s1), need_dx=False)

            c.tape.record(bwd_emb)

        k3 = (1,) * (3 - sd) + (3,) * sd
        slots = down_res is None and SKIP_SLOTS
        skips = []

        def slot(dims, cb):
            if not slots:
                return None, None
            ca = self._skip_ca[len(skips)]
            buf = torch.empty((x_cl.shape[0],) + tuple(dims) + (ca + cb,), dtype=torch.bfloat16, device=dev)
            return buf, buf[..., ca:]

        def conv_dims(dims, k, s, p):
            return tuple((d + 2 * pp - kk) // ss + 1 for d, kk, ss, pp in zip(dims, k, s, p))

        buf, view = slot(conv_dims(x_cl.shape[1:4], self._k[0], self._s[0], self._p[0]), ch[0])
        h = E.conv(c, x_cl, "conv_in.conv", self._k[0], self._s[0], self._p[0], need_dx=need_dx, out=view)
        skips.append((h, buf))
        for i in range(L):
            for j in range(self.num_res_blocks[i]):
                att = self.attention_levels[i]
                buf, view = (None, None) if att else slot(h.shape[1:4], ch[i])
                h = self._resnet(c, h, f"down_blocks.{i}.resnets.{j}", temb_all, d_temb_all, out=view)
                if att:
                    h = self._attention(c, h, f"down_blocks.{i}.attentions.{j}", self._heads(ch[i], self.num_head_channels[i]))
                skips.append((h, buf))
            if i != L - 1:
                if self.resblock_updown:
                    h = self._resnet(c, h, f"down_blocks.{i}.downsampler", temb_all, d_temb_all, mode="down", stride=self._s[i + 1],
                                     kernel=self._k[i + 1])
                    skips.append((h, None))
                else:
                    buf, view = slot(conv_dims(h.shape[1:4], self._k[i + 1], self._s[i + 1], self._p[i + 1]), ch[i])
                    h = E.conv(c, h, f"down_blocks.{i}.downsampler.op.conv", self._k[i + 1], self._s[i + 1], self._p[i + 1], out=view)
                    skips.append((h, buf))
            if i == self._cut_level and grad:
                c.tape.record(E.CUT)
        if down_res is not None:
            if len(down_res) != len(skips):
                raise ValueError(f"down_block_additional_residuals must hold {len(skips)} tensors, got {len(down_res)}")
            skips = [(E.add(c, sk, r, b_needs_grad=False), None) for (sk, _), r in zip(skips, down_res)]
        h = self._resnet(c, h, "middle_block.resnet_1", temb_all, d_temb_all)
        h = self._attention(c, h, "middle_block.attention", self._heads(ch[-1], self.num_head_channels[-1]))

        def cat_buffer(ca):
            sk, sbuf = skips[-1]
            if sbuf is not None and sbuf.shape[-1] == ca + sk.shape[-1]:
                return sbuf, sbuf[..., :ca]
            return E.concat_buffer(sk.shape, ca, sk.shape[-1], dev)

        pending, view = cat_buffer(ch[-1])
        h = self._resnet(c, h, "middle_block.resnet_2", temb_all, d_temb_all, out=None if mid_res is not None else view)
        if mid_res is not None:
            h = E.add(c, h, mid_res, b_needs_grad=False)
        rch, rnrb = list(reversed(ch)), list(reversed(self.num_res_blocks))
        ratt, rnhc = list(reversed(self.attention_levels)), list(reversed(self.num_head_channels))
        rs, rp = list(reversed(self._s)), list(reversed(self._p))
        for i in range(L):
            n_res = rnrb[i] + 1
            for j in range(n_res):
                sk, sbuf = skips.pop()
                if pending is None or (sbuf is not None and pending is not sbuf):
                    pending = sbuf if sbuf is not None and sbuf.shape[-1] == h.shape[-1] + sk.shape[-1] else pending
                h = E.concat(c, h, sk, buf=pending)
                pending, view = (None, None)
                if j < n_res - 1 and not ratt[i]:
                    pending, view = cat_buffer(rch[i])
                h = self._resnet(c, h, f"up_blocks.{i}.resnets.{j}", temb_all, d_temb_all, out=view)
                if ratt[i]:
                    h = self._attention(c, h, f"up_blocks.{i}.attentions.{j}", self._heads(rch[i], rnhc[i]))
            if i != L - 1 and self.resblock_updown:
                pending, view = cat_buffer(rch[i])
                h = self._resnet(c, h, f"up_blocks.{i}.upsampler", temb_all, d_temb_all, out=view, mode="up", stride=rs[i])
            elif i != L - 1:
                pending, view = cat_buffer(rch[i])
                h = E.upsample_conv(c, h, f"up_blocks.{i}.upsampler.conv.conv", rs[i], k3, rp[i], out=view)
        no = E.gn(c, h, "out.0", self.groups, self.eps)
        p1 = (0,) * (3 - sd) + (1,) * sd
        return E.conv(c, h, "out.2.conv", k3, (1, 1, 1), p1, norm=no, silu=True)

    def forward(self, x, timesteps, context=None, class_labels=None, down_block_additional_residuals=None,
                mid_block_additional_residual=None):
        if context is not None and not self.with_conditioning:
            raise ValueError("model should have with_conditioning = True if context is provided")
        if timesteps.ndim != 1:
            raise ValueError("Timesteps should be a 1d-array")
        if x.shape[1] != self.in_channels:
            raise ValueError(f"Input number of channels ({x.shape[1]}) is not equal to expected number of channels ({self.in_channels})")
        if not x.is_cuda:
            raise RuntimeError("medical_image_generation_amd runs on MI355X only: move the module and inputs to 'cuda' "
                               "(there is no CPU fallback; the CPU restatement lives in oracle/ for tests)")
        timesteps = timesteps.to(device=x.device, dtype=torch.int64)
        if self.num_class_embeds is not None:
            if class_labels is None:
                raise ValueError("class_labels should be provided when num_class_embeds > 0")
            class_labels = class_labels.to(device=x.device, dtype=torch.int64).contiguous()
            if class_labels.shape != timesteps.shape or int(class_labels.min()) < 0 or int(class_labels.max()) >= self.num_class_embeds:
                raise IndexError("class_labels must hold one index in [0, num_class_embeds) per sample")

        to_cl = lambda r: ops.to_channels_last(r.detach().to(x.device).contiguous().float())
        down_res = [to_cl(r) for r in down_block_additional_residuals] if down_block_additional_residuals is not None else None
        mid_res = to_cl(mid_block_additional_residual) if mid_block_additional_residual is not None else None

        ctx_tokens = None
        if context is not None:
            if context.dim() != 3 or context.shape[0] != x.shape[0] or context.shape[2] != self.cross_attention_dim:
                raise ValueError(f"context must be [batch, tokens, {self.cross_attention_dim}], got {tuple(context.shape)}")
            ctx_tokens = ops.cast_bf16(context.detach().to(x.device).contiguous().float().reshape(-1, context.shape[2]))

        def runner(c, xin, need_dx):
            x_cl = ops.to_channels_last(xin.contiguous().float())
            y = self._run(c, x_cl, timesteps, need_dx, class_labels, down_res, mid_res, ctx_tokens)
            return (y,), {"x_cl": x_cl}

        grad_enabled = torch.is_grad_enabled() and (x.requires_grad or any(p.requires_grad for p in self.parameters()))
        return _NetFn.apply(self, runner, 1, grad_enabled, x, None, *self.parameters())
```

Baseline: 98.95 million voxels/s.

## Fuse timestep-embedding MLP into custom kernels and prepack attention QKV weights

Replaces the chain of small timestep-embedding ops (sinusoid, two linears, SiLU, projection to all resnet biases, zeroing of the gradient buffer) with two fused forward kernels and a fused backward kernel. It also extends the weight-pack batch to produce the bf16 QKV weights and their transposes once per step, so attention no longer casts and transposes them on every call. The goal is fewer tiny launches and less per-op overhead in a launch-bound graph. In exchange it adds a lot of new kernel code, and the bf16 rounding and accumulation order differ from the previous path.

```diff
diff --git a/include/medimgen_hip.h b/include/medimgen_hip.h
--- a/include/medimgen_hip.h
+++ b/include/medimgen_hip.h
@@ -55,6 +55,8 @@
 int mi_conv_pack_weights(mi_conv_plan* plan, const float* weight, hipStream_t stream);
 typedef struct mi_pack_batch mi_pack_batch;
 int mi_conv_pack_batch_create(mi_pack_batch** out, mi_conv_plan* const* plans, const float* const* weights, int n);
+int mi_conv_pack_batch_add_params(mi_pack_batch* batch, const float* const* weights, void* const* copies, void* const* transposes,
+                                  const int* rows, const int* cols, int n);
 int mi_conv_pack_batch_run(mi_pack_batch* batch, hipStream_t stream);
 int mi_conv_pack_batch_destroy(mi_pack_batch* batch);
 
@@ -92,6 +94,15 @@
 int mi_embedding_add(float* emb, const float* weight, const int64_t* labels, int B, int dim, hipStream_t stream);
 int mi_embedding_bwd(const float* d_emb, const int64_t* labels, float* dweight, int B, int dim, hipStream_t stream);
 int mi_silu_f32(const float* x, float* y, int64_t n, hipStream_t stream);
+int mi_embed_mlp_fwd(const int64_t* timesteps, int N, int C, int E, int T, float max_period, const float* w0, const float* b0,
+                     const float* w2, const float* b2, const float* class_weight, const int64_t* labels, const float* w_proj,
+                     const float* b_proj, const float* b_conv1, float* t0, float* e1, float* emb, float* temb_all, float* d_temb_all,
+                     hipStream_t stream);
+int64_t mi_embed_mlp_ws_floats(int N, int C, int E, int T);
+int mi_embed_mlp_bwd(const float* d_temb_all, int N, int C, int E, int T, const float* t0, const float* e1, const float* emb,
+                     const float* w0, const float* w2, const float* w_proj, float* gw0, float* gb0, float* gw2, float* gb2, float* gw_proj,
+                     float* gb_proj, float* gb_conv1, const int64_t* labels, float* g_class, float* ws, int64_t ws_floats,
+                     hipStream_t stream);
 int mi_silu_bwd_f32(const float* x, const float* dy, float* dx, int64_t n, hipStream_t stream);
 
 int mi_logvar_to_sigma_fwd(const void* logvar, void* sigma, int64_t n, hipStream_t stream);
diff --git a/medical_image_generation_amd/_lib.py b/medical_image_generation_amd/_lib.py
--- a/medical_image_generation_amd/_lib.py
+++ b/medical_image_generation_amd/_lib.py
@@ -34,6 +34,7 @@
     "mi_conv_plan_out_dims": [_p, C.POINTER(_i)],
     "mi_conv_pack_weights": [_p, _p, _p],
     "mi_conv_pack_batch_create": [C.POINTER(_p), C.POINTER(_p), C.POINTER(_p), _i],
+    "mi_conv_pack_batch_add_params": [_p, C.POINTER(_p), C.POINTER(_p), C.POINTER(_p), C.POINTER(_i), C.POINTER(_i), _i],
     "mi_conv_pack_batch_run": [_p, _p],
     "mi_conv_pack_batch_destroy": [_p],
     "mi_conv_fwd": [_p, _p, _i, _p, _i, _p, _i, _p, _i, _p, _i, _p, _p],
@@ -55,6 +56,9 @@
     "mi_attn_bwd": [_p, _i, _i, _i, _i, _i, _f, _p, _p, _p, _p, _p, _p, _p, _l, _p],
     "mi_timestep_embedding": [_p, _p, _i, _i, _f, _p],
     "mi_silu_f32": [_p, _p, _l, _p],
+    "mi_embed_mlp_fwd": [_p, _i, _i, _i, _i, _f] + [_p] * 15,
+    "mi_embed_mlp_ws_floats": [_i, _i, _i, _i],
+    "mi_embed_mlp_bwd": [_p, _i, _i, _i, _i] + [_p] * 16 + [_l, _p],
     "mi_silu_bwd_f32": [_p, _p, _p, _l, _p],
     "mi_logvar_to_sigma_fwd": [_p, _p, _l, _p],
     "mi_logvar_to_sigma_bwd": [_p, _p, _p, _p, _l, _p],
@@ -111,11 +115,11 @@
     "mi_l1_eval": [_p, _p, _p, _i, _i, _l, _p],
     "mi_kl_eval": [_p, _p, _p, _i, _i, _l, _p],
 }
-_RET = {"mi_gn_workspace_bytes": _l, "mi_attn_workspace_bytes": _l, "mi_aug_stats_workspace_bytes": _l, "mi_meter_bytes": _l}
-_NOCHECK = {"mi_abi_version", "mi_meter_bytes", "mi_ssim_tiles", "mi_gn_small_supported", "mi_gn_workspace_bytes", "mi_aug_stats_workspace_bytes", "mi_attn_supported", "mi_attn_workspace_bytes", "mi_conv_fwd_stats_chunks"}
+_RET = {"mi_gn_workspace_bytes": _l, "mi_attn_workspace_bytes": _l, "mi_aug_stats_workspace_bytes": _l, "mi_meter_bytes": _l, "mi_embed_mlp_ws_floats": _l}
+_NOCHECK = {"mi_abi_version", "mi_embed_mlp_ws_floats", "mi_meter_bytes", "mi_ssim_tiles", "mi_gn_small_supported", "mi_gn_workspace_bytes", "mi_aug_stats_workspace_bytes", "mi_attn_supported", "mi_attn_workspace_bytes", "mi_conv_fwd_stats_chunks"}
 
 _lib = None
-ABI_VERSION = 12
+ABI_VERSION = 13
 
 
 def exported_symbols() -> list[str]:
diff --git a/medical_image_generation_amd/csrc/api.hip b/medical_image_generation_amd/csrc/api.hip
--- a/medical_image_generation_amd/csrc/api.hip
+++ b/medical_image_generation_amd/csrc/api.hip
@@ -1,3 +1,3 @@
 #include "common.h"
 #include "medimgen_hip.h"
-extern "C" int mi_abi_version(void) { return 12; }
+extern "C" int mi_abi_version(void) { return 13; }
diff --git a/medical_image_generation_amd/csrc/conv.hip b/medical_image_generation_amd/csrc/conv.hip
--- a/medical_image_generation_amd/csrc/conv.hip
+++ b/medical_image_generation_amd/csrc/conv.hip
@@ -2372,7 +2372,7 @@
   __syncthreads();
   for (int r = ty; r < 32; r += 8) {
     const int ci = bi * 32 + r, co = bo * 32 + tx;
-    if (co < g.Co && ci < g.Ci) g.ot[(int64_t)ci * g.Co + co] = f2bf(t[tx][r]);
+    if (g.ot && co < g.Co && ci < g.Ci) g.ot[(int64_t)ci * g.Co + co] = f2bf(t[tx][r]);
   }
 }
 G11Job g11_job(const mi_conv_plan* P, const float* w, int block0) {
@@ -2416,6 +2416,7 @@
   size_t lds_super = 0;
   G11Job* d_g11 = nullptr;
   int ng11 = 0, g11_blocks = 0;
+  std::vector<G11Job> h_g11;
   PackGroup* d_groups = nullptr;
   int2* d_gtaps = nullptr;
   int ngroups = 0;
@@ -2528,6 +2529,7 @@
     B->nsupers = (int)supers.size(); B->lds_super = lds_super;
   }
   if (B->ng11) {
+    B->h_g11 = g11;
     if (hipMalloc((void**)&B->d_g11, sizeof(G11Job) * g11.size()) != hipSuccess ||
         hipMemcpy(B->d_g11, g11.data(), sizeof(G11Job) * g11.size(), hipMemcpyHostToDevice) != hipSuccess) {
       mi_conv_pack_batch_destroy(B);
@@ -2550,6 +2552,26 @@
   if (e == hipSuccess) e = hipMemcpy(B->d_gtaps, gtaps.data(), sizeof(int2) * gtaps.size(), hipMemcpyHostToDevice);
   if (e != hipSuccess) { mi_conv_pack_batch_destroy(B); return (int)e; }
   *out = B;
+  return 0;
+}
+int mi_conv_pack_batch_add_params(mi_pack_batch* B, const float* const* weights, void* const* copies, void* const* transposes,
+                                  const int* rows, const int* cols, int n) {
+  if (!B || !weights || !copies || !transposes || !rows || !cols || n <= 0) return MI_ERR_BAD_ARG;
+  std::vector<G11Job> jobs = B->h_g11;
+  int blocks = B->g11_blocks;
+  for (int i = 0; i < n; ++i) {
+    if (!weights[i] || !copies[i] || rows[i] <= 0 || cols[i] <= 0) return MI_ERR_BAD_ARG;
+    G11Job g;
+    g.w = weights[i]; g.o = (bf16*)copies[i]; g.ot = (bf16*)transposes[i]; g.Co = rows[i]; g.Ci = cols[i]; g.block0 = blocks;
+    g.bx = (cols[i] + 31) / 32;
+    blocks += g.bx * ((rows[i] + 31) / 32);
+    jobs.push_back(g);
+  }
+  G11Job* d = nullptr;
+  if (hipMalloc((void**)&d, sizeof(G11Job) * jobs.size()) != hipSuccess) return (int)hipErrorOutOfMemory;
+  if (hipMemcpy(d, jobs.data(), sizeof(G11Job) * jobs.size(), hipMemcpyHostToDevice) != hipSuccess) { (void)hipFree(d); return (int)hipErrorUnknown; }
+  if (B->d_g11) (void)hipFree(B->d_g11);
+  B->d_g11 = d; B->h_g11.swap(jobs); B->ng11 = (int)B->h_g11.size(); B->g11_blocks = blocks;
   return 0;
 }
 int mi_conv_pack_batch_run(mi_pack_batch* B, hipStream_t st) {
diff --git a/medical_image_generation_amd/csrc/embed.hip b/medical_image_generation_amd/csrc/embed.hip
--- /dev/null
+++ b/medical_image_generation_amd/csrc/embed.hip
@@ -0,0 +1,272 @@
+#include "common.h"
+#include "medimgen_hip.h"
+
+namespace {
+
+constexpr int kThreads = 256;
+constexpr int kWaves = kThreads / MI_WAVE;
+constexpr int kNB = 8;
+constexpr int kRows = 32;
+
+__device__ __forceinline__ float rbf(float v) { return bf2f(f2bf(v)); }
+
+__device__ __forceinline__ void row_dots(const float* __restrict__ wrow, int K, const float* xs, int nn, float acc[kNB]) {
+  const int lane = threadIdx.x & (MI_WAVE - 1);
+#pragma unroll
+  for (int i = 0; i < kNB; ++i) acc[i] = 0.f;
+  for (int k = lane * 4; k < K; k += MI_WAVE * 4) {
+    const float4 w = *reinterpret_cast<const float4*>(wrow + k);
+    const float w0 = rbf(w.x), w1 = rbf(w.y), w2 = rbf(w.z), w3 = rbf(w.w);
+#pragma unroll
+    for (int i = 0; i < kNB; ++i)
+      if (i < nn) {
+        const float4 x = *reinterpret_cast<const float4*>(xs + (size_t)i * K + k);
+        acc[i] = fmaf(w3, x.w, fmaf(w2, x.z, fmaf(w1, x.y, fmaf(w0, x.x, acc[i]))));
+      }
+  }
+#pragma unroll
+  for (int i = 0; i < kNB; ++i)
+    if (i < nn) acc[i] = wave_sum(acc[i]);
+}
+
+__device__ __forceinline__ float sinusoid(int64_t t, int j, int dim, float neg_log_period) {
+  const int half = dim / 2;
+  if (j >= 2 * half) return 0.f;
+  const int k = j < half ? j : j - half;
+  const float freq = (float)exp((double)(neg_log_period * (float)k) / (double)half);
+  const float arg = (float)t * freq;
+  return j < half ? cosf(arg) : sinf(arg);
+}
+
+__global__ void __launch_bounds__(kThreads) k_embed_mlp(const int64_t* __restrict__ t, int N, int C, int E, float neg_log_period,
+                                                        const float* __restrict__ w0, const float* __restrict__ b0,
+                                                        const float* __restrict__ w2, const float* __restrict__ b2,
+                                                        const float* __restrict__ cls, const int64_t* __restrict__ labels,
+                                                        float* __restrict__ t0, float* __restrict__ e1, float* __restrict__ emb) {
+  extern __shared__ float4 smem4[];
+  float* x0 = reinterpret_cast<float*>(smem4);
+  float* s1 = x0 + (size_t)kNB * C;
+  const int wave = threadIdx.x >> 6, lane = threadIdx.x & 63;
+  const int r0 = blockIdx.x * kRows;
+  float acc[kNB];
+  for (int n0 = 0; n0 < N; n0 += kNB) {
+    const int nn = min(kNB, N - n0);
+    for (int i = threadIdx.x; i < nn * C; i += kThreads) {
+      const int n = n0 + i / C, j = i % C;
+      const float v = sinusoid(t[n], j, C, neg_log_period);
+      if (blockIdx.x == 0) t0[(size_t)n * C + j] = v;
+      x0[i] = rbf(v);
+    }
+    __syncthreads();
+    for (int j = wave; j < E; j += kWaves) {
+      row_dots(w0 + (size_t)j * C, C, x0, nn, acc);
+      const float bj = b0[j];
+#pragma unroll
+      for (int i = 0; i < kNB; ++i)
+        if (i < nn && lane == i) {
+          const float h = acc[i] + bj;
+          if (blockIdx.x == 0) e1[(size_t)(n0 + i) * E + j] = h;
+          s1[(size_t)i * E + j] = rbf(silu_f(h));
+        }
+    }
+    __syncthreads();
+    for (int rr = wave; rr < kRows && r0 + rr < E; rr += kWaves) {
+      const int r = r0 + rr;
+      row_dots(w2 + (size_t)r * E, E, s1, nn, acc);
+      const float br = b2[r];
+#pragma unroll
+      for (int i = 0; i < kNB; ++i)
+        if (i < nn && lane == i) {
+          float v = acc[i] + br;
+          if (cls) v += cls[labels[n0 + i] * (int64_t)E + r];
+          emb[(size_t)(n0 + i) * E + r] = v;
+        }
+    }
+    __syncthreads();
+  }
+}
+
+__global__ void __launch_bounds__(kThreads) k_embed_proj(const float* __restrict__ emb, int N, int E, int T, const float* __restrict__ wp,
+                                                         const float* __restrict__ bp, const float* __restrict__ bc,
+                                                         float* __restrict__ temb, float* __restrict__ dtemb) {
+  extern __shared__ float4 smem4[];
+  float* se = reinterpret_cast<float*>(smem4);
+  const int wave = threadIdx.x >> 6, lane = threadIdx.x & 63;
+  const int r0 = blockIdx.x * kRows;
+  float acc[kNB];
+  for (int n0 = 0; n0 < N; n0 += kNB) {
+    const int nn = min(kNB, N - n0);
+    for (int i = threadIdx.x; i < nn * E; i += kThreads) se[i] = rbf(silu_f(emb[(size_t)n0 * E + i]));
+    __syncthreads();
+    for (int rr = wave; rr < kRows && r0 + rr < T; rr += kWaves) {
+      const int r = r0 + rr;
+      row_dots(wp + (size_t)r * E, E, se, nn, acc);
+      const float b1 = bp[r], b2 = bc[r];
+#pragma unroll
+      for (int i = 0; i < kNB; ++i)
+        if (i < nn && lane == i) {
+          temb[(size_t)(n0 + i) * T + r] = (acc[i] + b1) + b2;
+          if (dtemb) dtemb[(size_t)(n0 + i) * T + r] = 0.f;
+        }
+    }
+    __syncthreads();
+  }
+}
+
+struct LinBwd {
+  const float* dy_in;
+  const float* parts;
+  int nparts;
+  const float* pre_y;
+  const float* x_in;
+  int x_silu;
+  const float* w;
+  float *gw, *gb, *gb2;
+  const int64_t* labels;
+  float* gcls;
+  float* part_out;
+  int N, R, K;
+};
+__global__ void __launch_bounds__(kThreads) k_embed_lin_bwd(const LinBwd p) {
+  extern __shared__ float4 smem4[];
+  const int K = p.K, R = p.R, N = p.N;
+  const int KQ = K / 4, RS = kThreads / KQ;
+  float* xs = reinterpret_cast<float*>(smem4);
+  float* dys = xs + (size_t)kNB * K;
+  float* red = dys + kNB * kRows;
+  const int r0 = blockIdx.x * kRows;
+  const int k4 = threadIdx.x % KQ, rsub = threadIdx.x / KQ;
+  for (int n0 = 0; n0 < N; n0 += kNB) {
+    const int nn = min(kNB, N - n0);
+    for (int i = threadIdx.x; i < nn * K; i += kThreads) {
+      const float v = p.x_in[(size_t)n0 * K + i];
+      xs[i] = rbf(p.x_silu ? silu_f(v) : v);
+    }
+    for (int i = threadIdx.x; i < nn * kRows; i += kThreads) {
+      const int n = n0 + i / kRows, rr = i % kRows, r = r0 + rr;
+      float v = 0.f;
+      if (r < R) {
+        if (p.parts) {
+          for (int q = 0; q < p.nparts; ++q) v += p.parts[((size_t)q * N + n) * R + r];
+          v *= silu_grad_f(p.pre_y[(size_t)n * R + r]);
+        } else {
+          v = p.dy_in[(size_t)n * R + r];
+        }
+      }
+      dys[i] = v;
+    }
+    __syncthreads();
+    if (threadIdx.x < kRows && r0 + (int)threadIdx.x < R) {
+      const int rr = threadIdx.x, r = r0 + rr;
+      float s = p.gb[r];
+      for (int i = 0; i < nn; ++i) s += dys[i * kRows + rr];
+      p.gb[r] = s;
+      if (p.gb2) {
+        float s2 = p.gb2[r];
+        for (int i = 0; i < nn; ++i) s2 += dys[i * kRows + rr];
+        p.gb2[r] = s2;
+      }
+      if (p.gcls)
+        for (int i = 0; i < nn; ++i) p.gcls[p.labels[n0 + i] * (int64_t)R + r] += dys[i * kRows + rr];
+    }
+    float4 acc[kNB];
+#pragma unroll
+    for (int i = 0; i < kNB; ++i) acc[i] = make_float4(0.f, 0.f, 0.f, 0.f);
+    if (rsub < RS) {
+      for (int rr = rsub; rr < kRows && r0 + rr < R; rr += RS) {
+        const size_t at = (size_t)(r0 + rr) * K + (size_t)k4 * 4;
+        const float4 wv = *reinterpret_cast<const float4*>(p.w + at);
+        const float w0 = rbf(wv.x), w1 = rbf(wv.y), w2 = rbf(wv.z), w3 = rbf(wv.w);
+        float4 g = make_float4(0.f, 0.f, 0.f, 0.f);
+#pragma unroll
+        for (int i = 0; i < kNB; ++i)
+          if (i < nn) {
+            const float d = rbf(dys[i * kRows + rr]);
+            const float4 x = *reinterpret_cast<const float4*>(xs + (size_t)i * K + k4 * 4);
+            g.x = fmaf(d, x.x, g.x); g.y = fmaf(d, x.y, g.y); g.z = fmaf(d, x.z, g.z); g.w = fmaf(d, x.w, g.w);
+            acc[i].x = fmaf(d, w0, acc[i].x); acc[i].y = fmaf(d, w1, acc[i].y);
+            acc[i].z = fmaf(d, w2, acc[i].z); acc[i].w = fmaf(d, w3, acc[i].w);
+          }
+        float4 cur = *reinterpret_cast<const float4*>(p.gw + at);
+        cur.x += g.x; cur.y += g.y; cur.z += g.z; cur.w += g.w;
+        *reinterpret_cast<float4*>(p.gw + at) = cur;
+      }
+    }
+    if (p.part_out) {
+      if (rsub < RS) {
+#pragma unroll
+        for (int i = 0; i < kNB; ++i)
+          if (i < nn) *reinterpret_cast<float4*>(red + ((size_t)rsub * kNB + i) * K + k4 * 4) = acc[i];
+      }
+      __syncthreads();
+      for (int i = threadIdx.x; i < nn * K; i += kThreads) {
+        const int n = i / K, k = i % K;
+        float s = 0.f;
+        for (int q = 0; q < RS; ++q) s += red[((size_t)q * kNB + n) * K + k];
+        p.part_out[((size_t)blockIdx.x * N + n0 + n) * K + k] = s;
+      }
+    }
+    __syncthreads();
+  }
+}
+
+inline bool aligned16(const void* q) { return (reinterpret_cast<uintptr_t>(q) & 15) == 0; }
+inline bool dims_ok(int N, int C, int E, int T) { return N > 0 && T > 0 && C > 0 && E > 0 && C % 4 == 0 && E % 4 == 0 && C <= 1024 && E <= 1024; }
+inline size_t bwd_lds(int K) { return sizeof(float) * ((size_t)kNB * K + kNB * kRows + (size_t)(kThreads / (K / 4)) * kNB * K); }
+
+}
+
+extern "C" {
+
+int64_t mi_embed_mlp_ws_floats(int N, int C, int E, int T) {
+  if (!dims_ok(N, C, E, T)) return 0;
+  return ((int64_t)ceil_div(T, kRows) + ceil_div(E, kRows)) * N * E;
+}
+
+int mi_embed_mlp_fwd(const int64_t* timesteps, int N, int C, int E, int T, float max_period, const float* w0, const float* b0,
+                     const float* w2, const float* b2, const float* class_weight, const int64_t* labels, const float* w_proj,
+                     const float* b_proj, const float* b_conv1, float* t0, float* e1, float* emb, float* temb_all, float* d_temb_all,
+                     hipStream_t st) {
+  if (!timesteps || !w0 || !b0 || !w2 || !b2 || !w_proj || !b_proj || !b_conv1 || !t0 || !e1 || !emb || !temb_all) return MI_ERR_BAD_ARG;
+  if (!dims_ok(N, C, E, T) || (class_weight && !labels)) return MI_ERR_BAD_ARG;
+  if (!aligned16(w0) || !aligned16(w2) || !aligned16(w_proj)) return MI_ERR_BAD_ARG;
+  const size_t lds1 = sizeof(float) * (size_t)kNB * (C + E), lds2 = sizeof(float) * (size_t)kNB * E;
+  hipLaunchKernelGGL(k_embed_mlp, dim3(ceil_div(E, kRows)), dim3(kThreads), lds1, st, timesteps, N, C, E, -logf(max_period), w0, b0, w2,
+                     b2, class_weight, labels, t0, e1, emb);
+  MI_CHECK_LAUNCH();
+  hipLaunchKernelGGL(k_embed_proj, dim3(ceil_div(T, kRows)), dim3(kThreads), lds2, st, (const float*)emb, N, E, T, w_proj, b_proj, b_conv1,
+                     temb_all, d_temb_all);
+  MI_CHECK_LAUNCH();
+  return 0;
+}
+
+int mi_embed_mlp_bwd(const float* d_temb_all, int N, int C, int E, int T, const float* t0, const float* e1, const float* emb,
+                     const float* w0, const float* w2, const float* w_proj, float* gw0, float* gb0, float* gw2, float* gb2, float* gw_proj,
+                     float* gb_proj, float* gb_conv1, const int64_t* labels, float* g_class, float* ws, int64_t ws_floats, hipStream_t st) {
+  if (!d_temb_all || !t0 || !e1 || !emb || !w0 || !w2 || !w_proj || !gw0 || !gb0 || !gw2 || !gb2 || !gw_proj || !gb_proj || !gb_conv1 || !ws)
+    return MI_ERR_BAD_ARG;
+  if (!dims_ok(N, C, E, T) || (g_class && !labels) || ws_floats < mi_embed_mlp_ws_floats(N, C, E, T)) return MI_ERR_BAD_ARG;
+  for (const void* q : {(const void*)w0, (const void*)w2, (const void*)w_proj, (const void*)gw0, (const void*)gw2, (const void*)gw_proj, (const void*)ws})
+    if (!aligned16(q)) return MI_ERR_BAD_ARG;
+  static const hipError_t attr = hipFuncSetAttribute((const void*)k_embed_lin_bwd, hipFuncAttributeMaxDynamicSharedMemorySize, 96 * 1024);
+  if (attr != hipSuccess) return (int)attr;
+  const int bT = ceil_div(T, kRows), bE = ceil_div(E, kRows);
+  float* part_proj = ws;
+  float* part_2 = ws + (size_t)bT * N * E;
+  LinBwd p;
+  p.dy_in = d_temb_all; p.parts = nullptr; p.nparts = 0; p.pre_y = nullptr; p.x_in = emb; p.x_silu = 1; p.w = w_proj;
+  p.gw = gw_proj; p.gb = gb_proj; p.gb2 = gb_conv1; p.labels = nullptr; p.gcls = nullptr; p.part_out = part_proj; p.N = N; p.R = T; p.K = E;
+  hipLaunchKernelGGL(k_embed_lin_bwd, dim3(bT), dim3(kThreads), bwd_lds(E), st, p);
+  MI_CHECK_LAUNCH();
+  p.dy_in = nullptr; p.parts = part_proj; p.nparts = bT; p.pre_y = emb; p.x_in = e1; p.x_silu = 1; p.w = w2;
+  p.gw = gw2; p.gb = gb2; p.gb2 = nullptr; p.labels = labels; p.gcls = g_class; p.part_out = part_2; p.R = E; p.K = E;
+  hipLaunchKernelGGL(k_embed_lin_bwd, dim3(bE), dim3(kThreads), bwd_lds(E), st, p);
+  MI_CHECK_LAUNCH();
+  p.parts = part_2; p.nparts = bE; p.pre_y = e1; p.x_in = t0; p.x_silu = 0; p.w = w0;
+  p.gw = gw0; p.gb = gb0; p.labels = nullptr; p.gcls = nullptr; p.part_out = nullptr; p.R = E; p.K = C;
+  hipLaunchKernelGGL(k_embed_lin_bwd, dim3(bE), dim3(kThreads), bwd_lds(C), st, p);
+  MI_CHECK_LAUNCH();
+  return 0;
+}
+
+}
diff --git a/medical_image_generation_amd/engine.py b/medical_image_generation_amd/engine.py
--- a/medical_image_generation_amd/engine.py
+++ b/medical_image_generation_amd/engine.py
@@ -14,6 +14,7 @@
 import os as _os
 FLASH_ATTENTION = _os.environ.get("MI_FLASH_ATTENTION", "1") == "1"
 FUSE_GN_STATS = ops.FUSE_GN_STATS
+PARAM_PACK = _os.environ.get("MI_PARAM_PACK", "1") == "1"
 
 
 class ParamArena:
@@ -111,6 +112,7 @@
         self.arena, self.plans = arena, plans
         self.tape = Tape() if grad_enabled else None
         self.packed = set(prepacked)
+        self.wpacked = getattr(prepacked, "params", {})
         self.flops_fwd = 0
         self.flops_bwd = 0
         self.sums = {}
@@ -136,17 +138,34 @@
         return self.arena.gview(name)
 
 
+class PackedKeys(tuple):
+    params = {}
+
+
 class PackBatch:
 
-    def __init__(self, arena: ParamArena, plans: dict):
+    def __init__(self, arena: ParamArena, plans: dict, params=()):
         import ctypes as C
-        self.keys = tuple(plans)
+        self.keys = PackedKeys(plans)
         n = len(self.keys)
         plan_arr = (C.c_void_p * n)(*[plans[k].handle for k in self.keys])
         w_arr = (C.c_void_p * n)(*[arena.view(k[0] + ".weight").data_ptr() for k in self.keys])
         h = C.c_void_p()
         _lib.call_raw("mi_conv_pack_batch_create", C.byref(h), plan_arr, w_arr, n)
         self.handle = h
+        params = [q for q in params if PARAM_PACK]
+        if params:
+            m = len(params)
+            bufs = {}
+            for name, w, want_t in params:
+                assert w.dim() == 2 and w.is_contiguous() and w.dtype == F32
+                r, k = w.shape
+                bufs[name] = (torch.empty((r, k), dtype=BF16, device=w.device), torch.empty((k, r), dtype=BF16, device=w.device) if want_t else None)
+            arr = lambda vals: (C.c_void_p * m)(*vals)
+            _lib.call_raw("mi_conv_pack_batch_add_params", h, arr([q[1].data_ptr() for q in params]), arr([bufs[q[0]][0].data_ptr() for q in params]),
+                          arr([ptr(bufs[q[0]][1]) for q in params]), (C.c_int * m)(*[q[1].shape[0] for q in params]),
+                          (C.c_int * m)(*[q[1].shape[1] for q in params]), m)
+            self.keys.params = bufs
 
     def run(self):
         call("mi_conv_pack_batch_run", self.handle)
@@ -295,6 +314,7 @@
         return fn(ctx, x)
     sub = Ctx(ctx.arena, ctx.plans, grad_enabled=False)
     sub.packed, sub.sums, sub.cat_parts = ctx.packed, ctx.sums, ctx.cat_parts
+    sub.wpacked = ctx.wpacked
     y = fn(sub, x)
     ctx.flops_fwd += sub.flops_fwd
     ctx.flops_bwd += 2 * sub.flops_fwd
@@ -306,6 +326,7 @@
             return
         inner = Ctx(ctx.arena, ctx.plans, grad_enabled=True)
         inner.packed, inner.sums, inner.cat_parts = ctx.packed, ctx.sums, ctx.cat_parts
+        inner.wpacked = ctx.wpacked
         y2 = fn(inner, x)
         it = inner.tape
         tape.move(x, it)
@@ -451,7 +472,7 @@
     return out
 
 
-def _attention_flash(ctx, x, name, st, xn, wqkv, qkv, b, s, c, heads, scale):
+def _attention_flash(ctx, x, name, st, xn, wqkv, wqkv_t, qkv, b, s, c, heads, scale):
     dev = x.device
     d_, h_, w_ = x.shape[1:4]
     y = torch.empty_like(x)
@@ -474,19 +495,20 @@
             ws = torch.empty(max(nws, 16), dtype=torch.uint8, device=dev)
             call("mi_attn_bwd", ptr(qkv), 3 * c, c, heads, b, s, float(scale), ptr(y), ptr(x), ptr(dy), ptr(lse), ptr(dsum), ptr(dqkv),
                  ptr(ws), nws)
-            _attention_param_and_input_grads(ctx, tape, x, name, st, xn, wqkv, dqkv, dy, b, s, c)
-
-        tape.record(bwd)
-    return y
-
-
-def _attention_param_and_input_grads(ctx, tape, x, name, st, xn, wqkv, dqkv, dy, b, s, c):
+            _attention_param_and_input_grads(ctx, tape, x, name, st, xn, wqkv, wqkv_t, dqkv, dy, b, s, c)
+
+        tape.record(bwd)
+    return y
+
+
+def _attention_param_and_input_grads(ctx, tape, x, name, st, xn, wqkv, wqkv_t, dqkv, dy, b, s, c):
     dev = x.device
     pre = name + "." if name else ""
     gw = ctx.arena.span([f"{pre}to_{t}.weight" for t in "qkv"], ctx.arena.grad)
     gb = ctx.arena.span([f"{pre}to_{t}.bias" for t in "qkv"], ctx.arena.grad)
     call("mi_linear_wgrad_bf16", ptr(xn), c, c, ptr(dqkv), 3 * c, 3 * c, b * s, ptr(gw), ptr(gb))
-    wqkv_t = _transpose(wqkv, c, 0, 0, 3 * c, c, 1, 1, dev)[0]
+    if wqkv_t is None:
+        wqkv_t = _transpose(wqkv, c, 0, 0, 3 * c, c, 1, 1, dev)[0]
     dxn = torch.empty(x.shape, dtype=BF16, device=dev)
     _gemm(dqkv, 3 * c, 0, 0, wqkv_t, 3 * c, 0, 0, dxn, c, 0, 0, b * s, c, 3 * c, 1, 1)
     other = tape.take(x)
@@ -504,14 +526,14 @@
     pre = name + "." if name else ""
     st = gn(ctx, x, pre + "norm", groups, eps)
     xn = ops.gn_apply(x, st, False)
-    wqkv = ops.cast_bf16(ctx.arena.span([f"{pre}to_{t}.weight" for t in "qkv"]).view(3 * c, c))
+    wqkv, wqkv_t = ctx.wpacked.get(f"{pre}to_q.weight") or (ops.cast_bf16(ctx.arena.span([f"{pre}to_{t}.weight" for t in "qkv"]).view(3 * c, c)), None)
     bqkv = ctx.arena.span([f"{pre}to_{t}.bias" for t in "qkv"])
     qkv = torch.empty((b * s, 3 * c), dtype=BF16, device=dev)
     _gemm(xn, c, 0, 0, wqkv, c, 0, 0, qkv, 3 * c, 0, 0, b * s, 3 * c, c, 1, 1, bias=bqkv)
     z = b * heads
     sq = s * 3 * c
     if FLASH_ATTENTION and _lib.call_raw("mi_attn_supported", c, heads):
-        return _attention_flash(ctx, x, name, st, xn, wqkv, qkv, b, s, c, heads, scale)
+        return _attention_flash(ctx, x, name, st, xn, wqkv, wqkv_t, qkv, b, s, c, heads, scale)
     sp = (s + 7) // 8 * 8
     scores = torch.empty((z, s, s), dtype=F32, device=dev)
     _gemm((qkv, 0), 3 * c, sq, hd, (qkv, c), 3 * c, sq, hd, scores, s, heads * s * s, s * s, s, s, hd, z, heads, alpha=scale)
@@ -552,7 +574,7 @@
             dot = tr_tokens((dy, 0), c, s * c, hd, hd)
             _gemm(pt, sp, heads * s * sp, s * sp, dot, sp, heads * hd * sp, hd * sp, (dqkv, 2 * c), 3 * c, sq, hd, s, hd, sp, z, heads)
             del pt
-            _attention_param_and_input_grads(ctx, tape, x, name, st, xn, wqkv, dqkv, dy, b, s, c)
+            _attention_param_and_input_grads(ctx, tape, x, name, st, xn, wqkv, wqkv_t, dqkv, dy, b, s, c)
 
         tape.record(bwd)
     return y
diff --git a/medical_image_generation_amd/hipops.py b/medical_image_generation_amd/hipops.py
--- a/medical_image_generation_amd/hipops.py
+++ b/medical_image_generation_amd/hipops.py
@@ -385,6 +385,29 @@
     return out
 
 
+def embed_mlp_fwd(timesteps, c0, w0, b0, w2, b2, w_proj, b_proj, b_conv1, class_weight=None, labels=None, want_grad=True, max_period=10000.0):
+    n, (t, e), dev = timesteps.shape[0], w_proj.shape, timesteps.device
+    assert w0.shape == (e, c0) and w2.shape == (e, e) and all(v.is_contiguous() for v in (w0, w2, w_proj, b0, b2, b_proj, b_conv1))
+    t0, e1, emb = (torch.empty((n, k), dtype=F32, device=dev) for k in (c0, e, e))
+    temb = torch.empty((n, t), dtype=F32, device=dev)
+    d_temb = torch.empty_like(temb) if want_grad else None
+    call("mi_embed_mlp_fwd", ptr(timesteps), n, c0, e, t, float(max_period), ptr(w0), ptr(b0), ptr(w2), ptr(b2), ptr(class_weight),
+         ptr(labels) if class_weight is not None else None, ptr(w_proj), ptr(b_proj), ptr(b_conv1), ptr(t0), ptr(e1), ptr(emb), ptr(temb),
+         ptr(d_temb))
+    return temb, d_temb, (t0, e1, emb)
+
+
+def embed_mlp_bwd(saved, d_temb, w0, w2, w_proj, gw0, gb0, gw2, gb2, gw_proj, gb_proj, gb_conv1, labels=None, g_class=None):
+    t0, e1, emb = saved
+    n, t = d_temb.shape
+    c0, e = t0.shape[1], emb.shape[1]
+    assert d_temb.is_contiguous() and all(v.is_contiguous() for v in (gw0, gb0, gw2, gb2, gw_proj, gb_proj, gb_conv1))
+    nws = _lib.call_raw("mi_embed_mlp_ws_floats", n, c0, e, t)
+    ws = torch.empty(max(nws, 4), dtype=F32, device=d_temb.device)
+    call("mi_embed_mlp_bwd", ptr(d_temb), n, c0, e, t, ptr(t0), ptr(e1), ptr(emb), ptr(w0), ptr(w2), ptr(w_proj), ptr(gw0), ptr(gb0), ptr(gw2),
+         ptr(gb2), ptr(gw_proj), ptr(gb_proj), ptr(gb_conv1), ptr(labels) if g_class is not None else None, ptr(g_class), ptr(ws), nws)
+
+
 def silu_f32(x):
     y = torch.empty_like(x)
     call("mi_silu_f32", ptr(x), ptr(y), x.numel())
diff --git a/medical_image_generation_amd/unet.py b/medical_image_generation_amd/unet.py
--- a/medical_image_generation_amd/unet.py
+++ b/medical_image_generation_amd/unet.py
@@ -12,6 +12,7 @@
 
 F32 = torch.float32
 import os as _os
+EMBED_MLP = _os.environ.get("MI_EMBED_MLP", "1") == "1"
 SKIP_SLOTS = _os.environ.get("MI_SKIP_SLOTS", "1") == "1"
 
 
@@ -148,8 +149,11 @@
         if pb is None or len(pb.keys) != len(self._plans):
             if torch.cuda.is_current_stream_capturing():
                 return () if pb is None else pb.run()
-            pb = self._packb = E.PackBatch(self._arena, self._plans)
+            pb = self._packb = E.PackBatch(self._arena, self._plans, self._pack_params())
         return pb.run()
+
+    def _pack_params(self):
+        return ()
 
     def _apply(self, fn, *args, **kwargs):
         self._arena = None
@@ -351,6 +355,33 @@
             off += cout
         self._temb_total = off
 
+    def _pack_params(self):
+        out = []
+        for name in self._attns:
+            names = [f"{name}.to_{t}.weight" for t in "qkv"]
+            ch = self._arena.shapes[names[0]][1]
+            out.append((names[0], self._arena.span(names).view(3 * ch, ch), True))
+        return out
+
+    def _embed(self, c, timesteps, class_labels):
+        a = c.arena
+        grad = c.tape is not None
+        rn = [r[0] for r in self._resnets]
+        wn, bn, cn = ([r + sfx for r in rn] for sfx in (".time_emb_proj.weight", ".time_emb_proj.bias", ".conv1.conv.bias"))
+        T, E_ = self._temb_total, self.temb_dim
+        cls = c.p("class_embedding.weight") if self.num_class_embeds is not None else None
+        w0, w2, wp = c.p("time_embed.0.weight"), c.p("time_embed.2.weight"), a.span(wn).view(T, E_)
+        temb_all, d_temb_all, saved = ops.embed_mlp_fwd(timesteps, self.block_out_channels[0], w0, c.p("time_embed.0.bias"), w2,
+                                                        c.p("time_embed.2.bias"), wp, a.span(bn), a.span(cn), cls, class_labels, want_grad=grad)
+        if grad:
+            def bwd_emb():
+                ops.embed_mlp_bwd(saved, d_temb_all, w0, w2, wp, c.g("time_embed.0.weight"), c.g("time_embed.0.bias"), c.g("time_embed.2.weight"),
+                                  c.g("time_embed.2.bias"), a.span(wn, a.grad).view(T, E_), a.span(bn, a.grad), a.span(cn, a.grad),
+                                  class_labels, c.g("class_embedding.weight") if cls is not None else None)
+
+            c.tape.record(bwd_emb)
+        return temb_all, d_temb_all
+
     def _resnet(self, c, x, name, temb_all, d_temb_all, out=None, mode=None, stride=None, kernel=None):
         cout = c.p(name + ".conv1.conv.weight").shape[0]
         off = self._temb_off[name]
@@ -372,11 +403,9 @@
     def _heads(self, ch, nhc):
         return ch // nhc if nhc is not None else 1
 
-    def _run(self, c: E.Ctx, x_cl, timesteps, need_dx, class_labels=None, down_res=None, mid_res=None, context=None):
-        ch, L, sd = self.block_out_channels, len(self.block_out_channels), self.spatial_dims
-        self._context = context
+    def _embed_chain(self, c, timesteps, class_labels):
+        ch = self.block_out_channels
         a = c.arena
-        dev = x_cl.device
         grad = c.tape is not None
         t0 = ops.timestep_embedding(timesteps, ch[0])
         e1, bwd1 = E.linear_f32(t0, c.p("time_embed.0.weight"), c.p("time_embed.0.bias"), c.g("time_embed.0.weight"), c.g("time_embed.0.bias"))
@@ -403,7 +432,14 @@
                 bwd1(ops.silu_bwd_f32(e1, d_s1), need_dx=False)
 
             c.tape.record(bwd_emb)
-
+        return temb_all, d_temb_all
+
+    def _run(self, c: E.Ctx, x_cl, timesteps, need_dx, class_labels=None, down_res=None, mid_res=None, context=None):
+        ch, L, sd = self.block_out_channels, len(self.block_out_channels), self.spatial_dims
+        self._context = context
+        dev = x_cl.device
+        grad = c.tape is not None
+        temb_all, d_temb_all = (self._embed if EMBED_MLP else self._embed_chain)(c, timesteps, class_labels)
         k3 = (1,) * (3 - sd) + (3,) * sd
         slots = down_res is None and SKIP_SLOTS
         skips = []
```

After: 99.57 million voxels/s, median of 6. Within noise of the previous version (+0.6%).
